# quitedob/yolo-sod

Hardware: AMD Instinct MI355X
Metric: images/sec @640×640 bs=32, 1→8 MI355X; mAP@0.5:0.95 parity vs CPU ref (higher is better)
Workload: dtype f32

## Files before the change

include/yolosod_hip.h:

```cpp
#ifndef YOLOSOD_HIP_H
#define YOLOSOD_HIP_H
#include <stddef.h>
#include <stdint.h>

#ifdef __cplusplus
extern "C" {
#endif

int yolosod_abi_version(void);
const char* yolosod_last_error(void);
int yolosod_init(int device);

size_t yolosod_se_workspace(int B, int C, int H, int W);
int yolosod_se_forward(const float* x, float* y, int B, int C, int H, int W, const float* fc1_w, const float* fc1_b,
                       const float* fc2_w, const float* fc2_b, int hidden, void* workspace, size_t workspace_bytes,
                       void* stream);

size_t yolosod_cbam_workspace(int B, int C, int H, int W);
int yolosod_cbam_forward(const float* x, float* y, int B, int C, int H, int W, const float* fc0_w,
                         const float* fc2_w, int hidden, const float* sa_w, void* workspace, size_t workspace_bytes,
                         void* stream);

size_t yolosod_ca_workspace(int B, int C, int H, int W);
int yolosod_ca_forward(const float* x, float* y, int B, int C, int H, int W, const float* conv1_w,
// ... 69 lines not shown
                              const float* in_bn_var, float in_bn_eps, const float* pw1_w, const float* dw_w,
                              const float* bn_w, const float* bn_b, const float* bn_mean, const float* bn_var,
                              float bn_eps, const float* pw2_w, const float* out_w, const float* out_bn_w,
                              const float* out_bn_b, const float* out_bn_mean, const float* out_bn_var,
                              float out_bn_eps, void* workspace, size_t workspace_bytes, void* stream);

int yolosod_detect_decode(int nl, const float* const* maps, const int* heights, const int* widths,
                          const float* strides, int B, int nc, int reg_max, float* y, void* stream);

int yolosod_detect_head(int nl, const float* const* box_feat, const float* const* cls_feat, int c2, int c3,
                        const float* const* box_w, const float* const* box_b, const float* const* cls_w,
                        const float* const* cls_b, const int* heights, const int* widths, const float* strides, int B,
                        int nc, int reg_max, float* y, void* stream);

size_t yolosod_nms_workspace(int B, int nc, int A, int multi_label);
size_t yolosod_nms_workspace_v2(int B, int nc, int A, int multi_label, int max_det);
int yolosod_nms(float* pred, int B, int nc, int A, float conf_thres, double iou_thres, const int* classes,
                int n_classes, int agnostic, int multi_label, int max_det, int max_nms, float max_wh, int in_place,
                float* out, int* counts, int* out_index, void* workspace, size_t workspace_bytes, void* stream);
int yolosod_nms_merged(float* pred, int B, int nc, int A, float conf_thres, double iou_thres, const int* classes,
                       int n_classes, int agnostic, int multi_label, int max_det, int max_nms, float max_wh,
                       int in_place, float* out, int* counts, int* out_index, int* n_merged, void* workspace,
                       size_t workspace_bytes, void* stream);

int yolosod_letterbox_ingest(const int64_t* desc, int B, void* out, long out_bstride, int out_h, int out_w,
                             int out_bf16, int pad_value, void* stream);
int yolosod_letterbox_ingest_nv12(const int64_t* desc, int B, void* out, long out_bstride, int out_h, int out_w,
                                  int out_bf16, int pad_value, void* stream);
int yolosod_scale_boxes(float* det, const int* counts, int B, int D, const float* geom, void* stream);
int yolosod_tile_merge(const float* y, int n, int nc, int A, const int32_t* desc, int rows, float* merged, int F,
                       int S, float cut_margin, void* stream);
int yolosod_tta_views(const void* x, int B, int C, int H, int W, int bf16, const int64_t* desc, int V, int max_ph,
                      int max_pw, void* stream);
int yolosod_tta_merge(const float* y, int B, int nc, int A, int src_lo, int n, float* cat, int A_tot, int dst,
                      float scale, int flip, float img_w, float img_h, void* stream);
int yolosod_tile_merge_tta(const float* y, int n, int nc, int A, int src_lo, int n_k, const int32_t* desc, int rows,
                           float* merged, int F, int S, int A_tot, int dst, float scale, int flip, float img_w,
                           float img_h, float cut_margin, void* stream);
int yolosod_match_predictions(const float* det, const int* counts, int B, int D, const float* labels,
                              const int* label_off, const float* iouv, int T, uint8_t* tp, void* stream);
int yolosod_confusion_matrix(const float* det, const int* counts, int B, int D, const float* labels,
                             const int* label_off, int nc, float conf_thr, float iou_thr, int32_t* cm, void* stream);

int yolosod_bias_act(const float* y, long y_bstride, float* out, long out_bstride, const float* bias,
                     const float* res, long res_bstride, int B, int C, long HW, int act, void* stream);

int yolosod_bias_act_dual(const float* y, long y_bstride, float* out, long out_bstride, const float* bias,
                          const float* res, long res_bstride, float* out2, long out2_bstride, int c2lo, int B, int C,
                          long HW, int act, void* stream);

size_t yolosod_conv3x3_prep_bytes(int cin);
int yolosod_conv3x3_prepare(const float* w, int cin, void* prep, size_t prep_bytes, void* stream);
int yolosod_conv3x3_silu(const float* x, float* y, int B, int cin, int H, int W, const float* bias, const void* prep,
                         size_t prep_bytes, void* stream);
size_t yolosod_conv3x3_prep_bytes_ex(int cin, int cout);
int yolosod_conv3x3_prepare_ex(const float* w, int cin, int cout, void* prep, size_t prep_bytes, void* stream);
int yolosod_conv3x3_silu_ex(const float* x, float* y, long y_bstride, const float* res, long res_bstride, int B,
                            int cin, int cout, int H, int W, const float* bias, const void* prep, size_t prep_bytes,
                            void* stream);
int yolosod_conv3x3_silu_xs(const float* x, long x_bstride, float* y, long y_bstride, const float* res, long res_bstride,
                            int B, int cin, int cout, int H, int W, const float* bias, const void* prep,
                            size_t prep_bytes, void* stream);
int yolosod_bottleneck3x3_silu_xs(const float* x, long x_bstride, float* y, long y_bstride, const float* res,
                                  long res_bstride, int B, int H, int W, const float* bias1, const void* prep1,
                                  size_t prep1_bytes, const float* bias2, const void* prep2, size_t prep2_bytes,
                                  void* stream);

int yolosod_conv3x3_head_xs(const float* x, long x_bstride, int B, int H, int W, const float* bias, const void* prep,
                            size_t prep_bytes, const void* head_prep, const float* head_bias, int mode, int nc,
                            float stride, float* y, int A, int a_off, void* stream);
size_t yolosod_detect_head_prep_bytes(int rows);
int yolosod_detect_head_prepare(const float* w, int rows, void* prep, size_t prep_bytes, void* stream);

int yolosod_conv1x1_thin(const float* x, long x_bs, const float* w, const float* bias, float* out, long out_bs,
                         const float* res, long res_bs, float* out2, long out2_bs, int c2lo, int B, int Cin, int Cout,
                         long HW, void* stream);

int yolosod_sppf_pool(float* z, long z_bstride, int B, int C, int H, int W, void* stream);

int yolosod_conv1x1_thin_cat(const float* x, long x_bs, const float* x2, long x2_bs, int k1, const float* w,
                             const float* bias, float* out, long out_bs, float* out2, long out2_bs, int c2lo, int B,
                             int Cin, int Cout, long HW, int up_w, void* stream);

int yolosod_conv1x1_thin_stats(const float* x, long x_bs, const float* w, const float* bias, float* out, long out_bs,
                               int B, int Cin, int Cout, long HW, int parts, float* psum, float* pmax, float* tile_ws,
                               void* stream);

int yolosod_conv1x1(const float* x, long x_bs, const float* w, const float* bias, float* out, long out_bs,
                    const float* res, long res_bs, int B, int Cin, int Cout, long HW, int act, void* stream);

int yolosod_gemm_f32(const float* A, long a_bs, int lda, const float* B, long b_bs, int ldb, int b_kcontig, float* C,
                     long c_bs, int ldc, int M, int N, int K, int batch, const float* bias, int bias_mode, int act,
                     const float* res, void* stream);
int yolosod_layernorm(const float* x, float* y, long rows, int C, const float* w, const float* b, float eps,
                      void* stream);
int yolosod_attention(const float* qkv, float* out, long n_seq, int L, int C, int heads, void* stream);

void yolosod_debug_set_swin_fused(int on);
int yolosod_debug_set_swin_x3(int on);
int yolosod_debug_swin_route(int B, int C, int num_heads, int H, int W, int window, int mlp_hidden);
int yolosod_debug_swin_last_route(void);
int yolosod_debug_set_a2_pool_px(int px);
int yolosod_debug_set_head_x2(int on);
int yolosod_debug_set_a2_x2(int on);
int yolosod_debug_set_a2_fused(int on);
int yolosod_debug_set_a2_pool_wide(int on);
int yolosod_se_gate(const float* x, int B, int C, int H, int W, const float* fc1_w, const float* fc1_b,
                    const float* fc2_w, const float* fc2_b, int hidden, const float* psum, float* gate, void* workspace,
                    size_t workspace_bytes, void* stream);
int yolosod_cbam_gates(const float* x, int B, int C, int H, int W, const float* fc0_w, const float* fc2_w, int hidden,
                       const float* sa_w, const float* psum, const float* pmax, float* ca, float* sa, void* workspace,
                       size_t workspace_bytes, void* stream);
size_t yolosod_conv3x3s2_prep_bytes(int cin, int cout);
int yolosod_conv3x3s2_prepare(const float* w, int cin, int cout, void* prep, size_t prep_bytes, void* stream);
int yolosod_conv3x3s2_silu(const float* x, float* y, int B, int cin, int cout, int H, int W, const float* bias,
                           const float* gc, const float* gp, const void* prep, size_t prep_bytes, void* stream);
int yolosod_conv3x3s2_silu_out(const float* x, float* y, long y_bstride, int B, int cin, int cout, int H, int W,
                               const float* bias, const float* gc, const float* gp, const void* prep,
                               size_t prep_bytes, void* stream);
size_t yolosod_conv1x1x2_prep_bytes(int cin, int cout);
int yolosod_conv1x1x2_prepare(const float* w, int cin, int cout, void* prep, size_t prep_bytes, void* stream);
int yolosod_conv1x1x2_silu(const float* x, long x_bstride, float* y, long y_bstride, float* y2, long y2_bstride,
                           int c2lo, int B, int cin, int cout, int HW, const float* bias, const void* prep,
                           size_t prep_bytes, void* stream);
int yolosod_conv1x1x2_silu_cat(const float* x, long x_bstride, const float* x2, long x2_bstride, int k1, float* y,
                               long y_bstride, float* y2, long y2_bstride, int c2lo, int B, int cin, int cout, int HW,
                               const float* bias, const void* prep, size_t prep_bytes, int up_w, void* stream);
int yolosod_conv1x1x2_silu_stats(const float* x, long x_bstride, float* y, long y_bstride, int B, int cin, int cout,
                                 int HW, const float* bias, const void* prep, size_t prep_bytes, int stats, int parts,
                                 float* psum, float* pmax, float* tile_ws, void* stream);
int yolosod_debug_set_conv1x1x2_form(int form);
int yolosod_debug_conv1x1x2_form(int B, int cout, int H, int W);
int yolosod_debug_set_conv3x3s2_form(int form);
int yolosod_debug_conv3x3s2_form(int B, int cout, int H, int W);
int yolosod_debug_set_conv3x3_form(int form);
int yolosod_debug_conv3x3_form(int B, int cout, int H, int W);
int yolosod_debug_conv3x3_form_ex(int B, int cin, int cout, int H, int W);
int yolosod_debug_bottleneck3x3_fused(int B, int H, int W);
int yolosod_debug_set_bottleneck3x3_fuse(int mode);
int yolosod_debug_conv3x3_head_fused(int B, int H, int W);
int yolosod_debug_set_conv3x3_head_fuse(int mode);
void yolosod_debug_set_gemm_x2(int on);
int yolosod_debug_set_swin_tokln(int on);
int yolosod_debug_split_f16(const float* v, uint32_t* h, uint32_t* l, long npair, void* stream);
int yolosod_split_range_flag(int reset, void* stream);

#include <stdint.h>

int yolosod_se_forward_bf16(const uint16_t* x, uint16_t* y, int B, int C, int H, int W, const float* fc1_w,
                            const float* fc1_b, const float* fc2_w, const float* fc2_b, int hidden, const float* psum,
                            void* workspace, size_t workspace_bytes, void* stream);
int yolosod_cbam_forward_bf16(const uint16_t* x, uint16_t* y, int B, int C, int H, int W, const float* fc0_w,
                              const float* fc2_w, int hidden, const float* sa_w, const float* psum, const float* pmax,
                              void* workspace, size_t workspace_bytes, void* stream);
int yolosod_ca_forward_bf16(const uint16_t* x, uint16_t* y, int B, int C, int H, int W, const float* conv1_w,
                            const float* conv1_b, int mip, const float* bn_w, const float* bn_b, const float* bn_mean,
                            const float* bn_var, float bn_eps, const float* convh_w, const float* convh_b,
                            const float* convw_w, const float* convw_b, const float* yin, void* workspace,
                            size_t workspace_bytes, void* stream);
size_t yolosod_swin_workspace_bf16(int B, int C, int H, int W, int num_heads, int window, int mlp_hidden);
int yolosod_swin_forward_bf16(const uint16_t* x, uint16_t* y, int B, int C, int H, int W, int num_heads, int window,
                              const float* dw_w, const float* ln1_w, const float* ln1_b, float ln1_eps,
                              const uint16_t* in_proj_w, const float* in_proj_b, const uint16_t* out_proj_w,
                              const float* out_proj_b, const float* ln2_w, const float* ln2_b, float ln2_eps,
                              const uint16_t* mlp1_w, const float* mlp1_b, int mlp_hidden, const uint16_t* mlp2_w,
                              const float* mlp2_b, const uint16_t* pw_w, const float* bn_w, const float* bn_b,
                              const float* bn_mean, const float* bn_var, float bn_eps, void* workspace,
                              size_t workspace_bytes, void* stream);
size_t yolosod_a2_workspace_bf16(int B, int C, int H, int W, int num_areas);
int yolosod_a2_forward_bf16(const uint16_t* x, uint16_t* y, int B, int C, int H, int W, int num_areas, int num_heads,
                            const uint16_t* proj_w, const float* proj_b, const float* ln_w, const float* ln_b,
                            float ln_eps, const uint16_t* in_proj_w, const float* in_proj_b, const uint16_t* oproj_w,
                            const float* oproj_b, void* workspace, size_t workspace_bytes, void* stream);
int yolosod_detect_head_levels(int nl, int l0, int l1, const void* const* box_feat, const void* const* cls_feat, int c2,
                               int c3, const float* const* box_w, const float* const* box_b, const float* const* cls_w,
                               const float* const* cls_b, const int* heights, const int* widths, const float* strides,
                               int B, int nc, int reg_max, float* y, int bf16, void* stream);
int yolosod_detect_head_bf16(int nl, const uint16_t* const* box_feat, const uint16_t* const* cls_feat, int c2, int c3,
                             const float* const* box_w, const float* const* box_b, const float* const* cls_w,
                             const float* const* cls_b, const int* heights, const int* widths, const float* strides,
                             int B, int nc, int reg_max, float* y, void* stream);
int yolosod_bias_act_bf16(const uint16_t* y, long y_bstride, uint16_t* out, long out_bstride, const float* bias,
                          const uint16_t* res, long res_bstride, uint16_t* out2, long out2_bstride, int c2lo, int B,
                          int C, long HW, int act, void* stream);
int yolosod_bias_act_stats_bf16(const uint16_t* y, long y_bstride, uint16_t* out, long out_bstride, const float* bias,
                                const uint16_t* res, long res_bstride, int B, int C, long HW, int act, int parts,
                                long seg, float* psum, float* pmax, void* stream);
int yolosod_bias_act_capool_bf16(const uint16_t* y, long y_bstride, uint16_t* out, long out_bstride,
                                 const float* bias, const uint16_t* res, long res_bstride, int B, int C, int H, int W,
                                 int act, float* yin, void* stream);
int yolosod_gemm_bf16(const uint16_t* A, long a_bs, int lda, const uint16_t* B, long b_bs, int ldb, int b_kcontig,
                      uint16_t* C, long c_bs, int ldc, int M, int N, int K, int batch, const float* bias,
                      int bias_mode, int act, const uint16_t* res, void* stream);
int yolosod_attention_bf16(const uint16_t* qkv, uint16_t* out, long n_seq, int L, int C, int heads, void* stream);
int yolosod_debug_gemm_bf16_tile(int M, int N, int batch);
int yolosod_debug_gemm_bf16_last_tile(void);
long yolosod_debug_gemm_bf16_launches(int tile);
int yolosod_debug_swin_bf16_route(int B, int C, int num_heads, int H, int W, int window, int mlp_hidden);
int yolosod_debug_swin_bf16_last_route(void);
int yolosod_debug_attention_bf16_form(int L, int C, int heads);
int yolosod_debug_attention_bf16_last_form(void);

#ifdef __cplusplus
}
#endif
#endif
```

yolo-sod_amd/_hip.py:

```python
from __future__ import annotations

import ctypes
import os
from pathlib import Path

import torch

from .utils.metrics import IOU_THRESHOLDS

LIB_PATH = Path(__file__).resolve().parent / "lib" / "libyolosod_hip.so"

_c_float_p = ctypes.c_void_p
_vp = ctypes.c_void_p
_i = ctypes.c_int
_l = ctypes.c_long
_f = ctypes.c_float
_d = ctypes.c_double
_sz = ctypes.c_size_t

SIGNATURES = {
    "yolosod_abi_version": (_i, []),
    "yolosod_last_error": (ctypes.c_char_p, []),
    "yolosod_se_workspace": (_sz, [_i, _i, _i, _i]),
    "yolosod_se_forward": (_i, [_vp, _vp, _i, _i, _i, _i, _vp, _vp, _vp, _vp, _i, _vp, _sz, _vp]),
    "yolosod_cbam_workspace": (_sz, [_i, _i, _i, _i]),
    "yolosod_cbam_forward": (_i, [_vp, _vp, _i, _i, _i, _i, _vp, _vp, _i, _vp, _vp, _sz, _vp]),
    "yolosod_ca_workspace": (_sz, [_i, _i, _i, _i]),
    "yolosod_ca_forward": (_i, [_vp, _vp, _i, _i, _i, _i, _vp, _vp, _i, _vp, _vp, _vp, _vp, _f, _vp, _vp, _vp,
                                _vp, _vp, _sz, _vp]),
    "yolosod_a2_workspace": (_sz, [_i, _i, _i, _i, _i]),
    "yolosod_a2_forward": (_i, [_vp, _vp, _i, _i, _i, _i, _i, _i, _vp, _vp, _vp, _vp, _f, _vp, _vp, _vp, _vp, _vp,
                                _vp, _vp, _sz, _vp]),
    "yolosod_swin_workspace": (_sz, [_i, _i, _i, _i, _i, _i]),
    "yolosod_swin_workspace_v2": (_sz, [_i, _i, _i, _i, _i, _i, _i]),
    "yolosod_swin_forward": (_i, [_vp, _vp, _i, _i, _i, _i, _i, _i, _vp, _vp, _vp, _f, _vp, _vp, _vp, _vp, _vp, _vp,
                                  _f, _vp, _vp, _i, _vp, _vp, _vp, _vp, _vp, _vp, _vp, _f, _vp, _sz, _vp]),
    "yolosod_detect_decode": (_i, [_i, _vp, _vp, _vp, _vp, _i, _i, _i, _vp, _vp]),
    "yolosod_detect_head": (_i, [_i, _vp, _vp, _i, _i, _vp, _vp, _vp, _vp, _vp, _vp, _vp, _i, _i, _i, _vp, _vp]),
    "yolosod_nms_workspace": (_sz, [_i, _i, _i, _i]),
    "yolosod_nms_workspace_v2": (_sz, [_i, _i, _i, _i, _i]),
    "yolosod_nms": (_i, [_vp, _i, _i, _i, _f, _d, _vp, _i, _i, _i, _i, _i, _f, _i, _vp, _vp, _vp, _vp, _sz, _vp]),
    "yolosod_nms_merged": (_i, [_vp, _i, _i, _i, _f, _d, _vp, _i, _i, _i, _i, _i, _f, _i, _vp, _vp, _vp, _vp, _vp, _sz,
                                _vp]),
    "yolosod_gemm_f32": (_i, [_vp, _l, _i, _vp, _l, _i, _i, _vp, _l, _i, _i, _i, _i, _i, _vp, _i, _i, _vp, _vp]),
    "yolosod_layernorm": (_i, [_vp, _vp, _l, _i, _vp, _vp, _f, _vp]),
    "yolosod_attention": (_i, [_vp, _vp, _l, _i, _i, _i, _vp]),
    "yolosod_bias_act": (_i, [_vp, _l, _vp, _l, _vp, _vp, _l, _i, _i, _l, _i, _vp]),
    "yolosod_upsample2x": (_i, [_vp, _vp, _l, _i, _i, _i, _i, _i, _vp]),
    "yolosod_letterbox_ingest": (_i, [_vp, _i, _vp, _l, _i, _i, _i, _i, _vp]),
    "yolosod_letterbox_ingest_nv12": (_i, [_vp, _i, _vp, _l, _i, _i, _i, _i, _vp]),
    "yolosod_scale_boxes": (_i, [_vp, _vp, _i, _i, _vp, _vp]),
    "yolosod_tile_merge": (_i, [_vp, _i, _i, _i, _vp, _i, _vp, _i, _i, _f, _vp]),
    "yolosod_tile_merge_tta": (_i, [_vp, _i, _i, _i, _i, _i, _vp, _i, _vp, _i, _i, _i, _i, _f, _i, _f, _f, _f, _vp]),
    "yolosod_match_predictions": (_i, [_vp, _vp, _i, _i, _vp, _vp, _vp, _i, _vp, _vp]),
    "yolosod_confusion_matrix": (_i, [_vp, _vp, _i, _i, _vp, _vp, _i, _f, _f, _vp, _vp]),
    "yolosod_tta_views": (_i, [_vp, _i, _i, _i, _i, _i, _vp, _i, _i, _i, _vp]),
    "yolosod_tta_merge": (_i, [_vp, _i, _i, _i, _i, _i, _vp, _i, _i, _f, _i, _f, _f, _vp]),
    "yolosod_stem_workspace": (_sz, [_i, _i, _i, _i]),
    "yolosod_stem_conv": (_i, [_vp, _vp, _vp, _vp, _i, _i, _i, _i, _i, _l, _vp, _vp, _sz, _vp]),
    "yolosod_conv1x1_thin_stats": (_i, [_vp, _l, _vp, _vp, _vp, _l, _i, _i, _i, _l, _i, _vp, _vp, _vp, _vp]),
    "yolosod_conv1x1_thin": (_i, [_vp, _l, _vp, _vp, _vp, _l, _vp, _l, _vp, _l, _i, _i, _i, _i, _l, _vp]),
    "yolosod_bias_act_dual": (_i, [_vp, _l, _vp, _l, _vp, _vp, _l, _vp, _l, _i, _i, _i, _l, _i, _vp]),
    "yolosod_bias_act_capool": (_i, [_vp, ctypes.c_long, _vp, ctypes.c_long, _vp, _vp, ctypes.c_long, _i, _i, _i, _i,
                                     _i, _vp, _vp]),
    "yolosod_ca_forward_pre": (_i, [_vp, _vp, _i, _i, _i, _i, _vp, _vp, _i, _vp, _vp, _vp, _vp, _f, _vp, _vp, _vp, _vp,
                                    _vp, _vp, ctypes.c_size_t, _vp]),
    "yolosod_bias_act_stats": (_i, [_vp, _l, _vp, _l, _vp, _vp, _l, _i, _i, _l, _i, _i, _l, _vp, _vp, _vp]),
    "yolosod_plane_parts": (_i, [_l, ctypes.POINTER(ctypes.c_long)]),
    "yolosod_se_forward_pre": (_i, [_vp, _vp, _i, _i, _i, _i, _vp, _vp, _vp, _vp, _i, _vp, _vp, _sz, _vp]),
    "yolosod_cbam_forward_pre": (_i, [_vp, _vp, _i, _i, _i, _i, _vp, _vp, _i, _vp, _vp, _vp, _vp, _sz, _vp]),
    "yolosod_conv1x1": (_i, [_vp, _l, _vp, _vp, _vp, _l, _vp, _l, _i, _i, _i, _l, _i, _vp]),
    "yolosod_conv3x3_prep_bytes": (_sz, [_i]),
    "yolosod_conv3x3_prepare": (_i, [_vp, _i, _vp, _sz, _vp]),
    "yolosod_conv3x3_silu": (_i, [_vp, _vp, _i, _i, _i, _i, _vp, _vp, _sz, _vp]),
    "yolosod_conv1x1x2_prep_bytes": (_sz, [_i, _i]),
    "yolosod_conv1x1x2_prepare": (_i, [_vp, _i, _i, _vp, _sz, _vp]),
    "yolosod_conv1x1x2_silu": (_i, [_vp, _l, _vp, _l, _vp, _l, _i, _i, _i, _i, _i, _vp, _vp, _sz, _vp]),
    "yolosod_conv1x1x2_silu_cat": (_i, [_vp, _l, _vp, _l, _i, _vp, _l, _vp, _l, _i, _i, _i, _i, _i, _vp, _vp, _sz,
                                        _i, _vp]),
    "yolosod_conv1x1x2_silu_stats": (_i, [_vp, _l, _vp, _l, _i, _i, _i, _i, _vp, _vp, _sz, _i, _i, _vp, _vp, _vp, _vp]),
    "yolosod_sppf_pool": (_i, [_vp, _l, _i, _i, _i, _i, _vp]),
    "yolosod_conv1x1_thin_cat": (_i, [_vp, _l, _vp, _l, _i, _vp, _vp, _vp, _l, _vp, _l, _i, _i, _i, _i, _l, _i, _vp]),
    "yolosod_conv3x3_prep_bytes_ex": (_sz, [_i, _i]),
    "yolosod_conv3x3_prepare_ex": (_i, [_vp, _i, _i, _vp, _sz, _vp]),
    "yolosod_conv3x3_silu_ex": (_i, [_vp, _vp, _l, _vp, _l, _i, _i, _i, _i, _i, _vp, _vp, _sz, _vp]),
    "yolosod_conv3x3_silu_xs": (_i, [_vp, _l, _vp, _l, _vp, _l, _i, _i, _i, _i, _i, _vp, _vp, _sz, _vp]),
    "yolosod_debug_set_swin_fused": (None, [_i]),
    "yolosod_debug_set_swin_x3": (_i, [_i]),
    "yolosod_debug_swin_route": (_i, [_i, _i, _i, _i, _i, _i, _i]),
    "yolosod_debug_swin_last_route": (_i, []),
    "yolosod_debug_set_head_x2": (_i, [_i]),
    "yolosod_debug_set_a2_x2": (_i, [_i]),
    "yolosod_debug_set_gemm_x2": (None, [_i]),
    "yolosod_debug_split_f16": (_i, [_vp, _vp, _vp, _l, _vp]),
    "yolosod_swin_prep_bytes": (_sz, [_i, _i, _i]),
    "yolosod_split_range_flag": (_i, [_i, _vp]),
    "yolosod_swin_prepare": (_i, [_i, _i, _i] + [_vp] * 15 + [_f, _vp, _sz, _vp]),
    "yolosod_swin_forward_prepared": (_i, [_vp, _vp, _i, _i, _i, _i, _i, _i, _vp, _f, _vp, _f, _i, _vp, _vp, _sz,
                                           _vp, _sz, _vp]),
    "yolosod_swin_prepared_workspace": (_sz, [_i, _i, _i, _i, _i, _i, _i]),
    "yolosod_a2_prep_bytes": (_sz, [_i, _i, _i, _i]),
    "yolosod_a2_prepare": (_i, [_i, _vp, _vp, _vp, _vp, _vp, _vp, _sz, _vp]),
    "yolosod_a2_forward_prepared": (_i, [_vp, _vp, _i, _i, _i, _i, _i, _i, _vp, _vp, _vp, _vp, _f, _vp, _vp, _vp,
                                         _vp, _vp, _sz, _vp, _sz, _vp]),
    "yolosod_init": (_i, [_i]),
    "yolosod_debug_set_a2_fused": (_i, [_i]),
    "yolosod_debug_set_a2_pool_wide": (_i, [_i]),
    "yolosod_debug_set_conv3x3_form": (_i, [_i]),
    "yolosod_debug_conv3x3_form": (_i, [_i, _i, _i, _i]),
    "yolosod_debug_conv3x3_form_ex": (_i, [_i, _i, _i, _i, _i]),
    "yolosod_bottleneck3x3_silu_xs": (_i, [_vp, _l, _vp, _l, _vp, _l, _i, _i, _i, _vp, _vp, _sz, _vp, _vp, _sz, _vp]),
    "yolosod_conv3x3_head_xs": (_i, [_vp, _l, _i, _i, _i, _vp, _vp, _sz, _vp, _vp, _i, _i, _f, _vp, _i, _i, _vp]),
    "yolosod_detect_head_prep_bytes": (_sz, [_i]),
    "yolosod_detect_head_prepare": (_i, [_vp, _i, _vp, _sz, _vp]),
    "yolosod_debug_conv3x3_head_fused": (_i, [_i, _i, _i]),
    "yolosod_debug_set_conv3x3_head_fuse": (_i, [_i]),
    "yolosod_debug_bottleneck3x3_fused": (_i, [_i, _i, _i]),
    "yolosod_debug_set_bottleneck3x3_fuse": (_i, [_i]),
    "yolosod_debug_set_conv1x1x2_form": (_i, [_i]),
    "yolosod_debug_conv1x1x2_form": (_i, [_i, _i, _i, _i]),
    "yolosod_debug_set_conv3x3s2_form": (_i, [_i]),
    "yolosod_debug_conv3x3s2_form": (_i, [_i, _i, _i, _i]),
    "yolosod_se_gate": (_i, [_vp, _i, _i, _i, _i, _vp, _vp, _vp, _vp, _i, _vp, _vp, _vp, _sz, _vp]),
    "yolosod_cbam_gates": (_i, [_vp, _i, _i, _i, _i, _vp, _vp, _i, _vp, _vp, _vp, _vp, _vp, _vp, _sz, _vp]),
    "yolosod_conv3x3s2_prep_bytes": (_sz, [_i, _i]),
    "yolosod_conv3x3s2_prepare": (_i, [_vp, _i, _i, _vp, _sz, _vp]),
    "yolosod_conv3x3s2_silu": (_i, [_vp, _vp, _i, _i, _i, _i, _i, _vp, _vp, _vp, _vp, _sz, _vp]),
    "yolosod_conv3x3s2_silu_out": (_i, [_vp, _vp, _l, _i, _i, _i, _i, _i, _vp, _vp, _vp, _vp, _sz, _vp]),
    "yolosod_debug_set_swin_tokln": (_i, [_i]),
    "yolosod_debug_set_a2_pool_px": (_i, [_i]),
    "yolosod_mamba_glu_workspace": (_sz, [_i, _i, _i, _i, _i, _i]),
    "yolosod_mamba_glu_forward": (_i, [_vp, _vp, _i, _i, _i, _i, _i, _i, _vp, _vp, _vp, _vp, _vp, _f, _vp, _vp,
                                       _vp, _vp, _vp, _vp, _f, _vp, _vp, _vp, _vp, _vp, _vp, _f, _vp, _sz, _vp]),
    "yolosod_se_forward_bf16": (_i, [_vp, _vp, _i, _i, _i, _i, _vp, _vp, _vp, _vp, _i, _vp, _vp, _sz, _vp]),
    "yolosod_cbam_forward_bf16": (_i, [_vp, _vp, _i, _i, _i, _i, _vp, _vp, _i, _vp, _vp, _vp, _vp, _sz, _vp]),
    "yolosod_ca_forward_bf16": (_i, [_vp, _vp, _i, _i, _i, _i, _vp, _vp, _i, _vp, _vp, _vp, _vp, _f, _vp, _vp, _vp,
                                     _vp, _vp, _vp, _sz, _vp]),
    "yolosod_bias_act_bf16": (_i, [_vp, _l, _vp, _l, _vp, _vp, _l, _vp, _l, _i, _i, _i, _l, _i, _vp]),
    "yolosod_bias_act_stats_bf16": (_i, [_vp, _l, _vp, _l, _vp, _vp, _l, _i, _i, _l, _i, _i, _l, _vp, _vp, _vp]),
    "yolosod_bias_act_capool_bf16": (_i, [_vp, _l, _vp, _l, _vp, _vp, _l, _i, _i, _i, _i, _i, _vp, _vp]),
    "yolosod_swin_workspace_bf16": (_sz, [_i, _i, _i, _i, _i, _i, _i]),
    "yolosod_swin_forward_bf16": (_i, [_vp, _vp, _i, _i, _i, _i, _i, _i, _vp, _vp, _vp, _f, _vp, _vp, _vp, _vp, _vp,
                                       _vp, _f, _vp, _vp, _i, _vp, _vp, _vp, _vp, _vp, _vp, _vp, _f, _vp, _sz, _vp]),
    "yolosod_a2_workspace_bf16": (_sz, [_i, _i, _i, _i, _i]),
    "yolosod_a2_forward_bf16": (_i, [_vp, _vp, _i, _i, _i, _i, _i, _i, _vp, _vp, _vp, _vp, _f, _vp, _vp, _vp, _vp,
                                     _vp, _sz, _vp]),
    "yolosod_detect_head_bf16": (_i, [_i, _vp, _vp, _i, _i, _vp, _vp, _vp, _vp, _vp, _vp, _vp, _i, _i, _i, _vp,
                                      _vp]),
    "yolosod_detect_head_levels": (_i, [_i, _i, _i, _vp, _vp, _i, _i, _vp, _vp, _vp, _vp, _vp, _vp, _vp, _i, _i,
                                        _i, _vp, _i, _vp]),
    "yolosod_gemm_bf16": (_i, [_vp, _l, _i, _vp, _l, _i, _i, _vp, _l, _i, _i, _i, _i, _i, _vp, _i, _i, _vp, _vp]),
    "yolosod_attention_bf16": (_i, [_vp, _vp, _l, _i, _i, _i, _vp]),
    "yolosod_debug_gemm_bf16_tile": (_i, [_i, _i, _i]),
    "yolosod_debug_gemm_bf16_last_tile": (_i, []),
    "yolosod_debug_gemm_bf16_launches": (_l, [_i]),
    "yolosod_debug_swin_bf16_route": (_i, [_i, _i, _i, _i, _i, _i, _i]),
    "yolosod_debug_swin_bf16_last_route": (_i, []),
    "yolosod_debug_attention_bf16_form": (_i, [_i, _i, _i]),
    "yolosod_debug_attention_bf16_last_form": (_i, []),
}

_LIB = None
# ... 141 lines not shown
def _c(t: torch.Tensor) -> torch.Tensor:
    return t.detach().float().contiguous()


class PlaneStats:

    __slots__ = ("psum", "pmax", "parts", "shape")

    def __init__(self, psum, pmax, parts, shape):
        self.psum, self.pmax, self.parts, self.shape = psum, pmax, parts, tuple(shape)


_PARTS = {}


def plane_parts(HW: int):
    if HW not in _PARTS:
        seg = ctypes.c_long(0)
        parts = load_library().yolosod_plane_parts(int(HW), ctypes.byref(seg))
        _PARTS[HW] = (int(parts), int(seg.value))
    return _PARTS[HW]


def _pre_stats(x, need_max):
    st = getattr(x, "_ys_plane_stats", None)
    if st is None or st.shape != tuple(x.shape) or (need_max and st.pmax is None):
        return None
    return st


def _t(t, name):
    if not isinstance(t, torch.Tensor):
        raise TypeError(f"{name}: expected a tensor")
    if t.device.type != "cuda":
        raise RuntimeError(f"{name}: HIP kernel requires a GPU tensor (got device {t.device}); no CPU fallback")
    return t


def se_forward(x, fc1_w, fc1_b, fc2_w, fc2_b):
    bf = _act_dtype(_t(x, "x"))
    hid = fc1_w.shape[0]
    pre = _pre_stats(x, False)
    return _launch(("se", tuple(x.shape), hid) + ((2,) if bf else ()), x.device, ops().se_fwd, x, fc1_w, fc1_b,
                   fc2_w, fc2_b, None if pre is None else pre.psum)


def cbam_forward(x, fc0_w, fc2_w, sa_w):
    bf = _act_dtype(_t(x, "x"))
    hid = fc0_w.shape[0]
    pre = _pre_stats(x, True)
    return _launch(("cbam", tuple(x.shape), hid) + ((2,) if bf else ()), x.device, ops().cbam_fwd, x, fc0_w, fc2_w,
                   sa_w, None if pre is None else pre.psum, None if pre is None else pre.pmax)


def se_gate(x, fc1_w, fc1_b, fc2_w, fc2_b):
    lib = load_library()
    B, C, H, W = x.shape
    hid = int(fc1_w.shape[0])
    pre = _pre_stats(x, False)
    gate = torch.empty((B, C), dtype=torch.float32, device=x.device)
    ws = torch.empty(int(lib.yolosod_se_workspace(B, C, H, W)), dtype=torch.uint8, device=x.device)
    _check(_launch(("se_gate", tuple(x.shape), hid), x.device, lib.yolosod_se_gate, _dev(x, "x"), B, C, H, W,
                   _dev(fc1_w, "fc1_w"), _dev(fc1_b, "fc1_b"), _dev(fc2_w, "fc2_w"), _dev(fc2_b, "fc2_b"), hid,
                   None if pre is None else _dev(pre.psum, "psum"), gate.data_ptr(), ws.data_ptr(), ws.numel(),
                   _stream(x.device)), "se_gate")
    return gate


def cbam_gates(x, fc0_w, fc2_w, sa_w):
    lib = load_library()
    B, C, H, W = x.shape
    hid = int(fc0_w.shape[0])
    pre = _pre_stats(x, True)
    ca = torch.empty((B, C), dtype=torch.float32, device=x.device)
    sa = torch.empty((B, H, W), dtype=torch.float32, device=x.device)
    ws = torch.empty(int(lib.yolosod_cbam_workspace(B, C, H, W)), dtype=torch.uint8, device=x.device)
    _check(_launch(("cbam_gate", tuple(x.shape), hid), x.device, lib.yolosod_cbam_gates, _dev(x, "x"), B, C, H, W,
                   _dev(fc0_w, "fc0_w"), _dev(fc2_w, "fc2_w"), hid, _dev(sa_w, "sa_w"),
                   None if pre is None else _dev(pre.psum, "psum"), None if pre is None else _dev(pre.pmax, "pmax"),
                   ca.data_ptr(), sa.data_ptr(), ws.data_ptr(), ws.numel(), _stream(x.device)), "cbam_gates")
    return ca, sa


def ca_forward(x, conv1_w, conv1_b, bn_w, bn_b, bn_mean, bn_var, bn_eps, convh_w, convh_b, convw_w, convw_b):
    bf = _act_dtype(_t(x, "x"))
    mip = conv1_w.shape[0]
    pre = getattr(x, "_ys_ca_pool", None)
    yin = pre[0] if pre is not None and pre[1] == tuple(x.shape) else None
    return _launch(("ca", tuple(x.shape), mip) + ((2,) if bf else ()), x.device, ops().ca_fwd, x, conv1_w, conv1_b,
                   bn_w, bn_b, bn_mean, bn_var, float(bn_eps), convh_w, convh_b, convw_w, convw_b, yin)


def a2_prep_bytes(C, num_heads, num_areas, W) -> int:
    return int(load_library().yolosod_a2_prep_bytes(int(C), int(num_heads), int(num_areas), int(W)))


def a2_prepare(x, num_areas, num_heads, proj_w, ln_w, ln_b, in_w, in_b):
    return ops().a2_prep(x, int(num_areas), int(num_heads), proj_w, ln_w, ln_b, in_w, in_b)


def a2_forward(x, num_areas, num_heads, proj_w, proj_b, ln_w, ln_b, ln_eps, in_w, in_b, mo_w, mo_b, op_w, op_b,
               prep=None):
    bf = _act_dtype(_t(x, "x"))
    B, C, H, W = x.shape
    if num_areas * W > 320:
        raise RuntimeError(f"A2_Attn: sequence length {num_areas * W} > 320 unsupported")
    if bf and (C // num_heads not in (32, 64, 128) or C % 64):
        raise RuntimeError(f"A2_Attn (bf16): C={C} with head dim {C // num_heads} unsupported")
    use_prep = prep is not None and not bf and mo_w is None and a2_prep_bytes(C, num_heads, num_areas, W) > 0

    def run():
        return ops().a2_fwd(x, int(num_areas), int(num_heads), proj_w, proj_b, ln_w, ln_b, float(ln_eps), in_w, in_b,
                            mo_w, mo_b, op_w, op_b, prep() if use_prep else None)

    return _launch(("a2", tuple(x.shape), (num_areas, num_heads)) + ((2,) if bf else ()), x.device, run)


def swin_forward(x, num_heads, window, dw_w, ln1_w, ln1_b, ln1_eps, in_w, in_b, out_w, out_b, ln2_w, ln2_b,
                 ln2_eps, m1_w, m1_b, m2_w, m2_b, pw_w, bn_w, bn_b, bn_mean, bn_var, bn_eps, prep=None):
    bf = _act_dtype(_t(x, "x"))
    B, C, H, W = x.shape
    hid = m1_w.shape[0]
    wh = H if (H <= window and W <= window) else min(window, H)
    ww = W if (H <= window and W <= window) else min(window, W)
    if wh * ww > 320:
        raise RuntimeError(f"SwinBlock: window of {wh}x{ww} tokens unsupported")
    if C % num_heads or (C // num_heads) not in ((32, 64, 128) if bf else (8, 16, 32, 64, 128)):
        raise RuntimeError(f"SwinBlock: head dim {C}/{num_heads} unsupported")
    key = ("swin", tuple(x.shape), (num_heads, window, hid)) + ((2,) if bf else ())
    if (prep is not None and not bf and wh == 7 and ww == 7 and C * H * W < (1 << 30)
            and swin_prep_bytes(C, num_heads, hid) > 0):
        return _launch(key, x.device, lambda: ops().swin_fwd_prepared(x, prep(), int(num_heads), int(window), dw_w,
                                                                      float(ln1_eps), out_b, float(ln2_eps), int(hid),
                                                                      m2_b))
    return _launch(key, x.device, ops().swin_fwd, x, int(num_heads), int(window), dw_w, ln1_w, ln1_b, float(ln1_eps),
                   in_w, in_b, out_w, out_b, ln2_w, ln2_b, float(ln2_eps), m1_w, m1_b, m2_w, m2_b, pw_w, bn_w, bn_b,
                   bn_mean, bn_var, float(bn_eps))


def split_range_flag(reset: bool = True, device=None) -> bool:
    dev = torch.device("cuda", torch.cuda.current_device()) if device is None else torch.device(device)
    with torch.cuda.device(dev):
        rc = load_library().yolosod_split_range_flag(int(bool(reset)), _stream(dev))
    if rc < 0:
        _check(rc, "split_range_flag")
    return rc == 1


_split_convs_off = 0


def split_convs_enabled() -> bool:
    return _split_convs_off == 0


class exact_fp32_matrix:

    _SWITCHES = ("yolosod_debug_set_swin_x3", "yolosod_debug_set_head_x2", "yolosod_debug_set_a2_x2")

    def __enter__(self):
        global _split_convs_off
        lib = load_library()
        self._prev = [int(getattr(lib, f)(0)) for f in self._SWITCHES]
        _split_convs_off += 1
        return self

# ... 211 lines not shown
            fn = lib.yolosod_bias_act_capool_bf16 if bf else lib.yolosod_bias_act_capool
            _check(_launch(key("capool"), y.device, fn, y.data_ptr(), yb, out.data_ptr(), ob,
                           bp, rp, rb, B, C, H, W, int(act), yin.data_ptr(), _stream(y.device)), "bias_act_capool")
            out._ys_ca_pool = (yin, tuple(out.shape))
            return out
    if stats is not None:
        parts, seg = plane_parts(HW)
        psum = torch.empty(B * C * parts, dtype=torch.float32, device=y.device)
        pmax = torch.empty_like(psum) if stats == "summax" else None
        fn = lib.yolosod_bias_act_stats_bf16 if bf else lib.yolosod_bias_act_stats
        _check(_launch(key(stats), y.device, fn, y.data_ptr(), yb, out.data_ptr(), ob, bp,
                       rp, rb, B, C, HW, int(act), parts, seg, psum.data_ptr(),
                       None if pmax is None else pmax.data_ptr(), _stream(y.device)), "bias_act_stats")
        out._ys_plane_stats = PlaneStats(psum, pmax, parts, out.shape)
        return out
    if bf:
        _check(_launch(key(None), y.device, lib.yolosod_bias_act_bf16, y.data_ptr(), yb,
                       out.data_ptr(), ob, bp, rp, rb, None, 0, 0, B, C, HW, int(act), _stream(y.device)),
               "bias_act_bf16")
        return out
    _check(_launch(key(None), y.device, lib.yolosod_bias_act, y.data_ptr(), yb, out.data_ptr(),
                   ob, bp, rp, rb, B, C, HW, int(act), _stream(y.device)), "bias_act")
    return out


STEM_TILE_ROWS = 8


def stem_ok(x, conv) -> bool:
    if not isinstance(x, torch.Tensor) or x.dim() != 4 or x.device.type != "cuda" or x.dtype != torch.float32:
        return False
    B, Cin, H, W = x.shape
    if (conv.bias is None or Cin != 3 or conv.in_channels != 3 or conv.kernel_size != (3, 3) or conv.stride != (2, 2)
            or conv.padding != (1, 1) or conv.dilation != (1, 1) or conv.groups != 1
            or conv.padding_mode != "zeros" or conv.weight.dtype != torch.float32 or conv.weight.device != x.device):
        return False
    Cout = conv.out_channels
    if Cout % 2 or Cout > 64 or B == 0 or H % 2 or W % 2 or (W // 2) % 4:
        return False
    if not x.is_contiguous() or x.data_ptr() % 16:
        return False
    parts, seg = plane_parts((H // 2) * (W // 2))
    return parts == 1 or STEM_TILE_ROWS * (W // 2) <= seg


def stem_conv(x, weight, bias):
    B, _, H, W = _t(x, "x").shape
    Cout = int(weight.shape[0])
    out, psum = _launch(("stem", tuple(x.shape), (Cout, "sum")), x.device, ops().stem_fwd, x, weight, bias)
    out._ys_plane_stats = PlaneStats(psum, None, plane_parts((H // 2) * (W // 2))[0], out.shape)
    return out


def upsample2x_into(x, out) -> bool:
    B, C, h, w = x.shape
    if (x.device.type != "cuda" or out.device != x.device or out.dtype != x.dtype or x.dtype not in (torch.float32, _BF16)
            or not x.is_contiguous() or tuple(out.shape) != (B, C, 2 * h, 2 * w) or out.stride(3) != 1
            or out.stride(2) != 2 * w or out.stride(1) != 4 * h * w):
        return False
    eb = x.element_size()
    if (w % 4 or x.data_ptr() % 16 or out.data_ptr() % 16 or (out.stride(0) * eb) % 16 or (4 * h * w * eb) % 16
            or B == 0):
        return False
    _check(_launch(("upsample2x", tuple(x.shape), None), x.device, load_library().yolosod_upsample2x, x.data_ptr(),
                   out.data_ptr(), out.stride(0), B, C, h, w, eb, _stream(x.device)), "upsample2x")
    return True


THIN1X1_COUT = (64, 128)
THIN1X1_CIN = (64, 96, 128, 192, 256)


def conv1x1_thin_ok(x, cout) -> bool:
    if isinstance(x, CatView):
        B, Cin, H, W = x.shape
        return (x.device.type == "cuda" and x.dtype == torch.float32 and cout in THIN1X1_COUT and Cin in THIN1X1_CIN
                and (H * W) % 64 == 0 and all(_imgs_contig(t) for t in x.parts) and (not x.up0 or W % 4 == 0))
    B, Cin, H, W = x.shape
    return (x.device.type == "cuda" and x.dtype == torch.float32 and cout in THIN1X1_COUT and Cin in THIN1X1_CIN
            and (H * W) % 64 == 0 and x.stride(3) == 1 and x.stride(2) == W and x.stride(1) == H * W
            and x.stride(0) % 4 == 0 and x.data_ptr() % 16 == 0)


def conv1x1_thin(x, w, bias, out=None, res=None, out2=None, c2lo=0, stats=None):
    lib = load_library()
    B, Cin, H, W = x.shape
    Cout = w.shape[0]
    HW = H * W
    if out is None:
        out = torch.empty((B, Cout, H, W), dtype=torch.float32, device=x.device)

    def bstride(t, name, C):
        if t.device.type != "cuda" or t.dtype != torch.float32:
            raise RuntimeError(f"conv1x1_thin: {name} must be a float32 GPU tensor")
        if tuple(t.shape) != (B, C, H, W) or t.stride(3) != 1 or t.stride(2) != W or t.stride(1) != HW:
            raise RuntimeError(f"conv1x1_thin: {name} must be [B,{C},H,W] with contiguous channels")
        return t.stride(0)

    if isinstance(x, CatView):
        if res is not None or stats is not None:
            raise RuntimeError("conv1x1_thin: a CatView input takes no res / stats")
        x0, x1 = x.parts
        k1 = int(x0.shape[1])
        ob = bstride(out, "out", Cout)
        o2 = bstride(out2, "out2", Cout - c2lo) if out2 is not None else 0
        if x.up0:
            if not _imgs_contig(x0) or W % 4:
                raise RuntimeError("conv1x1_thin: an upsampled CatView part needs contiguous images and W % 4 == 0")
            xb0 = x0.stride(0)
        else:
            xb0 = bstride(x0, "x", k1)
        _check(_launch(("conv1x1_thin", tuple(x.shape), (Cout, False, out2 is not None, "cat")), x.device,
                       lib.yolosod_conv1x1_thin_cat, x0.data_ptr(), xb0, x1.data_ptr(),
                       bstride(x1, "x2", Cin - k1), k1, _dev(w.contiguous(), "weight"), _dev(bias, "bias"),
                       out.data_ptr(), ob, None if out2 is None else out2.data_ptr(), o2, int(c2lo), B, Cin, Cout, HW,
                       W if x.up0 else 0, _stream(x.device)), "conv1x1_thin_cat")
        return out
    xb = bstride(x, "x", Cin)
    ob = bstride(out, "out", Cout)
    rb = bstride(res, "res", Cout) if res is not None else 0
    o2 = bstride(out2, "out2", Cout - c2lo) if out2 is not None else 0
    if stats in ("sum", "summax") and res is None and out2 is None:
        parts, _ = plane_parts(HW)
        psum = torch.empty(B * Cout * parts, dtype=torch.float32, device=x.device)
        pmax = torch.empty_like(psum) if stats == "summax" else None
        tws = torch.empty(2 * B * Cout * (HW // 64), dtype=torch.float32, device=x.device)
        _check(_launch(("conv1x1_thin", tuple(x.shape), (Cout, stats)), x.device, lib.yolosod_conv1x1_thin_stats, x.data_ptr(), xb, _dev(w.contiguous(), "weight"), _dev(bias, "bias"),
                                              out.data_ptr(), ob, B, Cin, Cout, HW, parts, psum.data_ptr(),
                                              None if pmax is None else pmax.data_ptr(), tws.data_ptr(), _stream(x.device)),
               "conv1x1_thin_stats")
        out._ys_plane_stats = PlaneStats(psum, pmax, parts, out.shape)
        return out
    if stats is not None:
        raise RuntimeError(f"conv1x1_thin: stats={stats!r} needs res=None and out2=None")
    _check(_launch(("conv1x1_thin", tuple(x.shape), (Cout, res is not None, out2 is not None)), x.device, lib.yolosod_conv1x1_thin, x.data_ptr(), xb, _dev(w.contiguous(), "weight"), _dev(bias, "bias"),
                                    out.data_ptr(), ob, None if res is None else res.data_ptr(), rb,
                                    None if out2 is None else out2.data_ptr(), o2, int(c2lo), B, Cin, Cout, HW,
                                    _stream(x.device)), "conv1x1_thin")
    return out


def conv1x1(x, w, bias, act, out=None, res=None):
    lib = load_library()
    B, Cin, H, W = x.shape
    Cout = w.shape[0]
    HW = H * W
    if out is None:
        out = torch.empty((B, Cout, H, W), dtype=torch.float32, device=x.device)

    def bstride(t, name, C):
        if t.device.type != "cuda" or t.dtype != torch.float32:
            raise RuntimeError(f"conv1x1: {name} must be a float32 GPU tensor")
        if tuple(t.shape) != (B, C, H, W) or t.stride(3) != 1 or t.stride(2) != W or t.stride(1) != HW:
            raise RuntimeError(f"conv1x1: {name} must be [B,{C},H,W] with contiguous channels")
        return t.stride(0)

    xb = bstride(x, "x", Cin)
    ob = bstride(out, "out", Cout)
    rb = bstride(res, "res", Cout) if res is not None else 0
    _check(_launch(("conv1x1", tuple(x.shape), Cout), x.device, lib.yolosod_conv1x1, x.data_ptr(), xb, _dev(w, "weight"), None if bias is None else _dev(bias, "bias"),
                               out.data_ptr(), ob, None if res is None else res.data_ptr(), rb, B, Cin, Cout, HW,
                               int(act), _stream(x.device)), "conv1x1")
    return out


def conv3x3_ok(x, conv) -> bool:
    return (x.device.type == "cuda" and x.dtype == torch.float32 and x.dim() == 4 and _imgs_contig(x)
            and conv.kernel_size == (3, 3) and conv.stride == (1, 1) and conv.padding == (1, 1)
            and conv.dilation == (1, 1) and conv.groups == 1 and x.shape[1] == conv.in_channels
            and int(load_library().yolosod_conv3x3_prep_bytes_ex(int(conv.in_channels), int(conv.out_channels))) > 0)


def _split_prepare(name, bytes_fn, prepare_fn, w):
# ... 41 lines not shown
                                           0 if res is None else res.stride(0), B, Cin, cout, H, W, _dev(b, "bias"),
                                           blk.data_ptr(), blk.numel(), _stream(x.device))

    _check(_launch((op, tuple(x.shape), cout if res is None else (cout, "res")), x.device, run), "conv3x3")
    return y


def conv3x3_head_fused(B, H, W) -> bool:
    return bool(load_library().yolosod_debug_conv3x3_head_fused(int(B), int(H), int(W)))


def detect_head_prepare(w, rows):
    lib = load_library()
    nbytes = int(lib.yolosod_detect_head_prep_bytes(int(rows)))
    wc = w.detach().float().reshape(w.shape[0], -1).contiguous()
    if nbytes == 0 or tuple(wc.shape) != (rows, 64):
        raise RuntimeError(f"detect_head_prepare: weight {tuple(w.shape)} unsupported ([64 | 1..16, 64])")
    blk = torch.empty(nbytes, dtype=torch.uint8, device=w.device)
    _check(_launch(("head_prep", (rows, 64), None), w.device, lib.yolosod_detect_head_prepare, _dev(wc, "weight"),
                   int(rows), blk.data_ptr(), nbytes, _stream(w.device)), "detect_head_prepare")
    return blk


def conv3x3_head(x, bias, prep, head_prep, head_bias, mode, nc, stride, y, a_off):
    lib = load_library()
    B, Cin, H, W = x.shape
    if Cin != 64:
        raise RuntimeError(f"conv3x3_head: {Cin} channels (64 only)")
    if (y.dtype != torch.float32 or y.device != x.device or not y.is_contiguous() or y.dim() != 3 or y.shape[0] != B
            or y.shape[1] != 4 + nc):
        raise RuntimeError(f"conv3x3_head: y {tuple(y.shape)} is not a contiguous fp32 [{B}, {4 + nc}, A] tensor")
    b = bias.detach().float().contiguous()
    hb = head_bias.detach().float().contiguous()
    if hb.numel() != (64 if mode == 1 else nc):
        raise RuntimeError(f"conv3x3_head: head bias of {hb.numel()} values")

    def run():
        blk, hblk = prep(), head_prep()
        _img_view(x, (B, 64, H, W), "conv3x3_head: x")
        return lib.yolosod_conv3x3_head_xs(x.data_ptr(), x.stride(0), B, H, W, _dev(b, "bias"), blk.data_ptr(),
                                           blk.numel(), hblk.data_ptr(), _dev(hb, "head bias"), int(mode), int(nc),
                                           float(stride), y.data_ptr(), int(y.shape[2]), int(a_off), _stream(x.device))

    _check(_launch(("conv3x3", tuple(x.shape), (64, "head", int(mode))), x.device, run), "conv3x3_head")
    return y


def bottleneck3x3_fused(B, H, W) -> bool:
    return bool(load_library().yolosod_debug_bottleneck3x3_fused(int(B), int(H), int(W)))


def bottleneck3x3_silu(x, bias1, prep1, bias2, prep2, out=None, res=None, op="bottleneck3x3"):
    lib = load_library()
    B, C, H, W = x.shape
    if C != 32:
        raise RuntimeError(f"bottleneck3x3: {C} channels (32 only)")
    if out is None:
        y = torch.empty((B, 32, H, W), dtype=torch.float32, device=x.device)
    else:
        _img_view(out, (B, 32, H, W), "bottleneck3x3: out")
        y = out
    if res is not None:
        _img_view(res, (B, 32, H, W), "bottleneck3x3: res")
    b1 = bias1.detach().float().contiguous()
    b2 = bias2.detach().float().contiguous()

    def run():
        blk1, blk2 = prep1(), prep2()
        _img_view(x, (B, 32, H, W), "bottleneck3x3: x")
        return lib.yolosod_bottleneck3x3_silu_xs(x.data_ptr(), x.stride(0), y.data_ptr(), y.stride(0),
                                                 None if res is None else res.data_ptr(),
                                                 0 if res is None else res.stride(0), B, H, W, _dev(b1, "bias1"),
                                                 blk1.data_ptr(), blk1.numel(), _dev(b2, "bias2"), blk2.data_ptr(),
                                                 blk2.numel(), _stream(x.device))

    _check(_launch((op, tuple(x.shape), 32 if res is None else (32, "res")), x.device, run), "bottleneck3x3")
    return y


class CatView:

    def __init__(self, parts, up0=False):
        a, b = parts
        sp = (2 * a.shape[2], 2 * a.shape[3]) if up0 else tuple(a.shape[2:])
        if a.shape[0] != b.shape[0] or sp != tuple(b.shape[2:]) or a.dtype != b.dtype or a.device != b.device:
            raise ValueError("CatView: parts must agree in batch, spatial size, dtype and device")
        self.parts = (a, b)
        self.up0 = bool(up0)
        self.shape = torch.Size((a.shape[0], a.shape[1] + b.shape[1], b.shape[2], b.shape[3]))
        self.device, self.dtype = a.device, a.dtype

    def dim(self):
        return 4

    def materialize(self):
        a, b = self.parts
        if self.up0:
            a = torch.nn.functional.interpolate(a, scale_factor=2, mode="nearest")
        return torch.cat((a, b), 1)


def sppf_pool(z, c):
    B, C4, H, W = z.shape
    if (C4 != 4 * c or z.dtype != torch.float32 or z.device.type != "cuda"
            or z.stride()[1:] != (H * W, W, 1)):
        raise RuntimeError("sppf_pool: z must be a [B, 4c, H, W] fp32 GPU tensor with contiguous images")
    lib = load_library()
    _check(_launch(("sppf_pool", (B, c, H, W), None), z.device, lib.yolosod_sppf_pool, z.data_ptr(), z.stride(0), B,
                   int(c), H, W, _stream(z.device)), "sppf_pool")
    return z


def _imgs_contig(t) -> bool:
    B, C, H, W = t.shape
    return t.stride()[1:] == (H * W, W, 1) and t.stride(0) % 4 == 0 and t.data_ptr() % 16 == 0


def conv1x1x2_ok(x, conv) -> bool:
    if isinstance(x, CatView):
        if not (all(_imgs_contig(t) for t in x.parts) and x.parts[0].shape[1] % 128 == 0):
            return False
    elif not (x.dim() == 4 and _imgs_contig(x)):
        return False
    return (x.device.type == "cuda" and x.dtype == torch.float32
            and conv.kernel_size == (1, 1) and conv.stride == (1, 1) and conv.padding == (0, 0) and conv.groups == 1
            and x.shape[1] == conv.in_channels and (x.shape[2] * x.shape[3]) % 4 == 0
            and int(load_library().yolosod_conv1x1x2_prep_bytes(int(conv.in_channels), int(conv.out_channels))) > 0)


def conv1x1x2_prepare(w):
    lib = load_library()
    return _split_prepare("conv1x1x2", lib.yolosod_conv1x1x2_prep_bytes, lib.yolosod_conv1x1x2_prepare,
                          w.reshape(int(w.shape[0]), int(w.shape[1])))


def conv1x1x2_silu(x, bias, prep, cout, out=None, out2=None, c2lo=0, op="conv1x1x2", stats=None):
    lib = load_library()
    B, Cin, H, W = x.shape
    if stats is not None and (stats not in ("sum", "summax", "capool") or out2 is not None or isinstance(x, CatView)):
        raise RuntimeError(f"conv1x1x2: stats={stats!r} takes one input tensor, no out2")
    if out is None:
        y = torch.empty((B, cout, H, W), dtype=torch.float32, device=x.device)
    else:
        _img_view(out, (B, cout, H, W), "conv1x1x2: out")
        y = out
    if out2 is not None:
        _img_view(out2, (B, cout - c2lo, H, W), "conv1x1x2: out2")
    b = bias.detach().float().contiguous()
    if stats in ("sum", "summax"):
        HW = H * W
        parts, _ = plane_parts(HW)
        psum = torch.empty(B * cout * parts, dtype=torch.float32, device=x.device)
        pmax = torch.empty_like(psum) if stats == "summax" else None
        tws = torch.empty(2 * B * cout * ((HW + 63) // 64), dtype=torch.float32, device=x.device)

        def run_stats():
            blk = prep()
            return lib.yolosod_conv1x1x2_silu_stats(x.data_ptr(), x.stride(0), y.data_ptr(), y.stride(0), B, Cin, cout,
                                                    HW, _dev(b, "bias"), blk.data_ptr(), blk.numel(),
                                                    2 if stats == "summax" else 1, parts, psum.data_ptr(),
                                                    None if pmax is None else pmax.data_ptr(), tws.data_ptr(),
                                                    _stream(x.device))

        _check(_launch(("conv1x1x2_stats", tuple(x.shape), (cout, stats)), x.device, run_stats), "conv1x1x2_stats")
        y._ys_plane_stats = PlaneStats(psum, pmax, parts, y.shape)
        return y

    x0, x1 = x.parts if isinstance(x, CatView) else (x, None)

    def run():
        blk = prep()
        return lib.yolosod_conv1x1x2_silu_cat(x0.data_ptr(), x0.stride(0), None if x1 is None else x1.data_ptr(),
                                              0 if x1 is None else x1.stride(0), int(x0.shape[1]), y.data_ptr(),
                                              y.stride(0), None if out2 is None else out2.data_ptr(),
                                              0 if out2 is None else out2.stride(0), int(c2lo), B, Cin, cout, H * W,
                                              _dev(b, "bias"), blk.data_ptr(), blk.numel(),
                                              W if x1 is not None and x.up0 else 0, _stream(x.device))

    extra = (cout, out2 is not None) + (("cat",) if x1 is not None else ())
    if stats == "capool":
        op, extra = "conv1x1x2_stats", (cout, stats)
    _check(_launch((op, tuple(x.shape), extra), x.device, run), "conv1x1x2")
    return y


def conv3x3s2_ok(x, conv) -> bool:
    return (x.device.type == "cuda" and x.dtype == torch.float32 and x.is_contiguous() and x.dim() == 4
            and conv.kernel_size == (3, 3) and conv.stride == (2, 2) and conv.padding == (1, 1)
            and conv.dilation == (1, 1) and conv.groups == 1
            and (conv.out_channels == 64 or (conv.out_channels % 128 == 0 and conv.out_channels <= 512))
            and conv.in_channels % 32 == 0 and x.shape[1] == conv.in_channels and ((x.shape[3] + 1) // 2) % 4 == 0
            and x.numel() * 4 < 2 ** 32
            and int(load_library().yolosod_conv3x3s2_prep_bytes(int(conv.in_channels), int(conv.out_channels))) > 0)


def conv3x3s2_prepare(w):
    lib = load_library()
    return _split_prepare("conv3x3s2", lib.yolosod_conv3x3s2_prep_bytes, lib.yolosod_conv3x3s2_prepare, w)


def conv3x3s2_silu(x, bias, prep, cout, gate_c=None, gate_p=None, key=None, out=None):
    lib = load_library()
    B, Cin, H, W = x.shape
    Ho, Wo = (H + 1) // 2, (W + 1) // 2
    if out is None:
        y = torch.empty((B, cout, Ho, Wo), dtype=torch.float32, device=x.device)
    else:
        y = out
        if (tuple(y.shape) != (B, cout, Ho, Wo) or y.dtype != torch.float32 or y.device != x.device
                or y.stride()[1:] != (Ho * Wo, Wo, 1) or y.data_ptr() % 16 or y.stride(0) % 4):
            raise RuntimeError(f"conv3x3s2: out {tuple(y.shape)} / {y.stride()} is not a [{B}, {cout}, {Ho}, {Wo}] "
                               "fp32 view with contiguous 16-byte aligned images")
    b = bias.detach().float().contiguous()
    gc = None if gate_c is None else gate_c.float().contiguous()
    gp = None if gate_p is None else gate_p.float().contiguous()
    if gc is not None and (tuple(gc.shape) != (B, Cin) or gc.data_ptr() % 16):
        raise RuntimeError(f"conv3x3s2: channel gate {tuple(gc.shape)} (16-byte aligned [{B}, {Cin}] expected)")
    if gp is not None and gp.numel() != B * H * W:
        raise RuntimeError(f"conv3x3s2: spatial gate of {gp.numel()} values ({B * H * W} expected)")

    def run():
        blk = prep()
        return lib.yolosod_conv3x3s2_silu_out(_dev(x, "x"), y.data_ptr(), y.stride(0), B, Cin, cout, H, W,
                                              _dev(b, "bias"), None if gc is None else _dev(gc, "gate_c"),
                                              None if gp is None else _dev(gp, "gate_p"), blk.data_ptr(), blk.numel(),
                                              _stream(x.device))

    if key is None:
        key = ("conv3x3s2", tuple(x.shape), (cout, gc is not None, gp is not None))
    _check(_launch(key, x.device, run), "conv3x3s2")
    return y


INGEST_MAX_DIM = 16384


def letterbox_ingest(images, out_shape, geoms, dtype=torch.float32, out=None, pad_value=114):
    lib = load_library()
    B = len(images)
    out_h, out_w = int(out_shape[0]), int(out_shape[1])
    if B < 1 or len(geoms) != B:
        raise RuntimeError(f"letterbox_ingest: {B} frames with {len(geoms)} geometries")
    if dtype not in (torch.float32, _BF16):
        raise RuntimeError(f"letterbox_ingest: output dtype must be float32 or bfloat16, got {dtype}")
    if out_w % 4 or not (0 < out_h <= INGEST_MAX_DIM and 0 < out_w <= INGEST_MAX_DIM):
        raise RuntimeError(f"letterbox_ingest: canvas {out_h}x{out_w} unsupported (width % 4 == 0, <= {INGEST_MAX_DIM})")
    rows = []
    dev = None
    for i, (t, g) in enumerate(zip(images, geoms)):
        if not isinstance(t, torch.Tensor):
            raise TypeError(f"letterbox_ingest: frame {i}: expected a tensor")
        if t.dtype != torch.uint8:
            raise RuntimeError(f"letterbox_ingest: frame {i}: expected uint8, got {t.dtype}")
        if t.dim() != 3 or t.shape[2] != 3:
            raise RuntimeError(f"letterbox_ingest: frame {i}: expected [h, w, 3] (BGR), got {tuple(t.shape)}")
        h, w = int(t.shape[0]), int(t.shape[1])
        if not (0 < h <= INGEST_MAX_DIM and 0 < w <= INGEST_MAX_DIM):
            raise RuntimeError(f"letterbox_ingest: frame {i}: {h}x{w} outside 1..{INGEST_MAX_DIM}")
        if t.stride(2) != 1:
            raise RuntimeError(f"letterbox_ingest: frame {i}: channel stride {t.stride(2)} (1 expected)")
        if w > 1 and t.stride(1) != 3:
            raise RuntimeError(f"letterbox_ingest: frame {i}: pixel stride {t.stride(1)} (3 expected)")
        pitch = int(t.stride(0)) if h > 1 else 3 * w
        if pitch < 3 * w:
# ... 538 lines not shown
```

yolo-sod_amd/csrc/channel_attention.hip:

```cpp
#include "common.h"
#include <stdlib.h>
#include <math.h>

namespace ys {

constexpr int kMaxParts = 64;

struct PartPlan {
  int parts;
  long seg;
};
static PartPlan part_plan(long HW) {
  long p = HW / 8192;
  if (p > kMaxParts) p = kMaxParts;
  if (p < 1) p = 1;
  long seg = (HW + p - 1) / p;
  if ((HW & 3) == 0) seg = (seg + 3) & ~3L;
  p = (HW + seg - 1) / seg;
  return {(int)p, seg};
}

template <bool WITH_MAX, class T>
__global__ __launch_bounds__(256) void plane_part_stats_kernel(const T* __restrict__ x, long HW, int parts,
                                                               long seg, float* __restrict__ psum,
// ... 669 lines not shown
template <class T>
static int cbam_forward_impl(const T* x, T* y, int B, int C, int H, int W, const float* fc0_w, const float* fc2_w,
                             int hidden, const float* sa_w, const float* psum_pre, const float* pmax_pre,
                             void* workspace, size_t workspace_bytes, void* stream, float* ca_out = nullptr,
                             float* sa_out = nullptr) {
  YS_CHECK_ARG(x && (y || (ca_out && sa_out)) && fc0_w && fc2_w && sa_w, "cbam: null pointer");
  YS_CHECK_ARG(B >= 0 && C > 0 && C <= 16384 && H > 0 && W > 0, "cbam: bad shape");
  YS_CHECK_ARG(hidden > 0 && hidden <= 64, "cbam: hidden=%d unsupported (1..64)", hidden);
  if (B == 0) return 0;
  const long HW = (long)H * W;
  const int V = (HW % 4 == 0) ? 4 : 1;
  const long pxb = (HW + 256 * V - 1) / (256 * V);
  const int G = (C + kCbamGroup - 1) / kCbamGroup;
  Carver cv(workspace, workspace_bytes);
  float* psum = cv.take<float>((size_t)B * C * part_plan((long)H * W).parts);
  float* pmax = cv.take<float>((size_t)B * C * part_plan((long)H * W).parts);
  float* ca = cv.take<float>((size_t)B * C);
  float* mpart = cv.take<float>((size_t)B * G * 2 * HW);
  float* sa = cv.take<float>((size_t)B * HW);
  YS_CHECK_ARG(sa, "cbam: workspace too small (%zu)", workspace_bytes);
  if (!y) {
    ca = ca_out;
    sa = sa_out;
  }
  hipStream_t st = (hipStream_t)stream;
  const PartPlan pp = part_plan(HW);
  const size_t lds = sizeof(float) * (3 * (size_t)C + 128);
  const bool fused = V == 4 && lds <= 64 * 1024;
  YS_CHECK_ARG(lds <= 64 * 1024, "cbam: C=%d too large for the gate kernel", C);
  const float* ps = psum_pre ? psum_pre : psum;
  const float* pm = pmax_pre ? pmax_pre : pmax;
  if (!psum_pre)
    hipLaunchKernelGGL((plane_part_stats_kernel<true, T>), dim3((unsigned)(B * C * pp.parts)), dim3(256), 0, st, x, HW,
                       pp.parts, pp.seg, psum, pmax);
  dim3 gs((unsigned)pxb, G, B);
  if (fused) {
    hipLaunchKernelGGL((cbam_pixel_stats_kernel<4, T, true>), gs, dim3(256), lds, st, x, ca, C, kCbamGroup, HW, mpart,
                       ps, pm, pp.parts, 1.0f / (float)HW, fc0_w, fc2_w, hidden);
  } else {
    hipLaunchKernelGGL((channel_gate_kernel<true>), dim3(B), dim3(256), lds, st, ps, pm, pp.parts, C, 1.0f / (float)HW,
                       fc0_w, nullptr, fc2_w, nullptr, hidden, ca);
    if (V == 4)
      hipLaunchKernelGGL((cbam_pixel_stats_kernel<4, T, false>), gs, dim3(256), 0, st, x, ca, C, kCbamGroup, HW, mpart,
                         nullptr, nullptr, 0, 0.f, nullptr, nullptr, 0);
    else
      hipLaunchKernelGGL((cbam_pixel_stats_kernel<1, T, false>), gs, dim3(256), 0, st, x, ca, C, kCbamGroup, HW, mpart,
                         nullptr, nullptr, 0, 0.f, nullptr, nullptr, 0);
  }
  hipLaunchKernelGGL(cbam_sa_kernel, dim3((W + kSaTW - 1) / kSaTW, (H + kSaTH - 1) / kSaTH, B), dim3(256), 0, st, mpart, G, C, H, W, sa_w,
                     sa);
  if (y) {
    dim3 ga((unsigned)pxb, (C + 7) / 8, B);
    if (V == 4)
      hipLaunchKernelGGL((cbam_apply_kernel<4, T>), ga, dim3(256), 0, st, x, y, ca, sa, C, HW);
    else
      hipLaunchKernelGGL((cbam_apply_kernel<1, T>), ga, dim3(256), 0, st, x, y, ca, sa, C, HW);
  }
  YS_CHECK_LAUNCH("cbam");
  return 0;
}

YS_EXPORT int yolosod_cbam_forward(const float* x, float* y, int B, int C, int H, int W, const float* fc0_w,
                                   const float* fc2_w, int hidden, const float* sa_w, void* workspace,
                                   size_t workspace_bytes, void* stream) {
  return cbam_forward_impl(x, y, B, C, H, W, fc0_w, fc2_w, hidden, sa_w, (const float*)nullptr, nullptr, workspace,
                           workspace_bytes, stream);
}

YS_EXPORT int yolosod_cbam_forward_pre(const float* x, float* y, int B, int C, int H, int W, const float* fc0_w,
                                       const float* fc2_w, int hidden, const float* sa_w, const float* psum,
                                       const float* pmax, void* workspace, size_t workspace_bytes, void* stream) {
  YS_CHECK_ARG(psum && pmax, "cbam_pre: null partials");
  return cbam_forward_impl(x, y, B, C, H, W, fc0_w, fc2_w, hidden, sa_w, psum, pmax, workspace, workspace_bytes,
                           stream);
}

YS_EXPORT int yolosod_cbam_gates(const float* x, int B, int C, int H, int W, const float* fc0_w, const float* fc2_w,
                                 int hidden, const float* sa_w, const float* psum, const float* pmax, float* ca,
                                 float* sa, void* workspace, size_t workspace_bytes, void* stream) {
  YS_CHECK_ARG((psum == nullptr) == (pmax == nullptr), "cbam_gates: give both partials or neither");
  YS_CHECK_ARG(ca && sa, "cbam_gates: null output");
  return cbam_forward_impl<float>(x, nullptr, B, C, H, W, fc0_w, fc2_w, hidden, sa_w, psum, pmax, workspace,
                                  workspace_bytes, stream, ca, sa);
}

YS_EXPORT int yolosod_cbam_forward_bf16(const bf16_t* x, bf16_t* y, int B, int C, int H, int W, const float* fc0_w,
                                        const float* fc2_w, int hidden, const float* sa_w, const float* psum,
                                        const float* pmax, void* workspace, size_t workspace_bytes, void* stream) {
  YS_CHECK_ARG((psum == nullptr) == (pmax == nullptr), "cbam_bf16: give both partials or neither");
  return cbam_forward_impl(x, y, B, C, H, W, fc0_w, fc2_w, hidden, sa_w, psum, pmax, workspace, workspace_bytes,
                           stream);
}

YS_EXPORT size_t yolosod_ca_workspace(int B, int C, int H, int W) {
  Sizer s;
  s.take<float>((size_t)B * C * (H + W));
  s.take<float>((size_t)B * C * (H + W));
  return s.off;
}

template <class T>
static int ca_forward_impl(const T* x, T* y, int B, int C, int H, int W, const float* conv1_w, const float* conv1_b,
                           int mip, const float* bn_w, const float* bn_b, const float* bn_mean, const float* bn_var,
                           float bn_eps, const float* convh_w, const float* convh_b, const float* convw_w,
                           const float* convw_b, const float* yin_pre, void* workspace, size_t workspace_bytes,
                           void* stream) {
  YS_CHECK_ARG(x && y && conv1_w && conv1_b && bn_w && bn_b && bn_mean && bn_var && convh_w && convh_b && convw_w &&
                   convw_b,
               "ca: null pointer");
  YS_CHECK_ARG(B >= 0 && C > 0 && H > 0 && W > 0 && W <= 1024, "ca: bad shape (W <= 1024 supported)");
  YS_CHECK_ARG(mip > 0 && mip <= 64, "ca: mip=%d unsupported (1..64)", mip);
  const size_t gate_lds = ca_gate_lds_bytes(C, mip);
  YS_CHECK_ARG(gate_lds <= 64 * 1024, "ca: C=%d mip=%d exceed the gate kernel's LDS budget", C, mip);
  if (B == 0) return 0;
  Carver cv(workspace, workspace_bytes);
  float* yin = cv.take<float>((size_t)B * C * (H + W));
  float* gate = cv.take<float>((size_t)B * C * (H + W));
  YS_CHECK_ARG(gate, "ca: workspace too small (%zu)", workspace_bytes);
  hipStream_t st = (hipStream_t)stream;
  const long HW = (long)H * W;
  int RB = 8192 / W;
  if (RB < 1) RB = 1;
  if (RB > H) RB = H;
  const size_t pool_lds = sizeof(float) * (size_t)RB * W;
  const int V = (W % 4 == 0) ? 4 : 1;
  const int VA = (sizeof(T) == 2 && W % 8 == 0) ? 8 : V;
  const unsigned apply_y = (unsigned)((HW + 256 * VA - 1) / (256 * VA));
  if (!yin_pre)
    hipLaunchKernelGGL((ca_pool_kernel<T>), dim3(B * C), dim3(256), pool_lds, st, x, H, W, RB, yin);
  hipLaunchKernelGGL(ca_gate_kernel, dim3((H + W + 15) / 16, B), dim3(256), gate_lds, st, yin_pre ? yin_pre : yin, C,
                     H, W, mip, conv1_w, conv1_b, bn_w, bn_b, bn_mean, bn_var, bn_eps, convh_w, convh_b, convw_w,
                     convw_b, gate);
  if (VA == 8)
    hipLaunchKernelGGL((ca_apply_kernel<8, T>), dim3(B * C, apply_y), dim3(256), 0, st, x, y, gate, H, W);
  else if (V == 4)
    hipLaunchKernelGGL((ca_apply_kernel<4, T>), dim3(B * C, apply_y), dim3(256), 0, st, x, y, gate, H, W);
  else
    hipLaunchKernelGGL((ca_apply_kernel<1, T>), dim3(B * C, apply_y), dim3(256), 0, st, x, y, gate, H, W);
  YS_CHECK_LAUNCH("ca");
  return 0;
}

YS_EXPORT int yolosod_ca_forward(const float* x, float* y, int B, int C, int H, int W, const float* conv1_w,
                                 const float* conv1_b, int mip, const float* bn_w, const float* bn_b,
                                 const float* bn_mean, const float* bn_var, float bn_eps, const float* convh_w,
                                 const float* convh_b, const float* convw_w, const float* convw_b, void* workspace,
                                 size_t workspace_bytes, void* stream) {
  return ca_forward_impl(x, y, B, C, H, W, conv1_w, conv1_b, mip, bn_w, bn_b, bn_mean, bn_var, bn_eps, convh_w,
                         convh_b, convw_w, convw_b, (const float*)nullptr, workspace, workspace_bytes, stream);
}

YS_EXPORT int yolosod_ca_forward_pre(const float* x, float* y, int B, int C, int H, int W, const float* conv1_w,
                                     const float* conv1_b, int mip, const float* bn_w, const float* bn_b,
                                     const float* bn_mean, const float* bn_var, float bn_eps, const float* convh_w,
                                     const float* convh_b, const float* convw_w, const float* convw_b,
                                     const float* yin, void* workspace, size_t workspace_bytes, void* stream) {
  YS_CHECK_ARG(yin, "ca_pre: null pooled means");
  return ca_forward_impl(x, y, B, C, H, W, conv1_w, conv1_b, mip, bn_w, bn_b, bn_mean, bn_var, bn_eps, convh_w,
                         convh_b, convw_w, convw_b, yin, workspace, workspace_bytes, stream);
}

YS_EXPORT int yolosod_ca_forward_bf16(const bf16_t* x, bf16_t* y, int B, int C, int H, int W, const float* conv1_w,
                                      const float* conv1_b, int mip, const float* bn_w, const float* bn_b,
                                      const float* bn_mean, const float* bn_var, float bn_eps, const float* convh_w,
                                      const float* convh_b, const float* convw_w, const float* convw_b,
                                      const float* yin, void* workspace, size_t workspace_bytes, void* stream) {
// ... 4 lines not shown
```

yolo-sod_amd/csrc/conv1x1x2.hip:

```cpp
#include "split_conv.h"

namespace ys {
namespace c1 {

constexpr float WSC = SPLIT_WSC;
constexpr int KS = 128;
constexpr int PS = KS + 8;
constexpr int NT = 256;

struct Args {
  const float* x;
  long xbs;
  const h16_t* wp;
  const float* bias;
  float* y;
  long ybs;
  float* y2;
  long y2bs;
  int c2lo, cin, cout, HW, ntile;
  unsigned* range_flag;
  const unsigned* prep_flag;
  const float* x2;
  long x2bs;
  int k1;
  int up_w;
};

#include "conv1x1x2_kernel.h"
#define YS_C1_STATS_FORMS
#include "conv1x1x2_kernel.h"
#undef YS_C1_STATS_FORMS

}
}

using namespace ys;

static int c1_pad(int cin) { return (cin + c1::KS - 1) / c1::KS * c1::KS; }
static size_t c1_halves(int cin, int cout) { return (size_t)2 * cout * c1_pad(cin); }

static int g_c1_form = 0;
YS_EXPORT int yolosod_debug_set_conv1x1x2_form(int form) {
  const int old = g_c1_form;
  if (form >= 0 && form < 12 && (form & 3) != 3) g_c1_form = form;
  return old;
}

static int c1_form(int B, int cout, int HW) {
  if (cout == 64) return 1 + 4 * 1;
  const int fgrp = g_c1_form & 3, fbuf = g_c1_form >> 2;
  const bool g256 = fgrp ? fgrp == 2
                         : cout == 512 && HW <= 400 && (long)B * ((HW + 63) / 64) * (cout / 128) > 2L * cu_count();
  return (g256 && cout % 256 == 0 ? 2 : 1) + 4 * (fbuf ? fbuf : 1);
}

YS_EXPORT int yolosod_debug_conv1x1x2_form(int B, int cout, int H, int W) {
  if (B <= 0 || H <= 0 || W <= 0 || ((long)H * W) % 4 || cout <= 0 || (cout != 64 && cout % 128) || cout > 1024)
    return 0;
  return c1_form(B, cout, H * W);
}

template <int CPW, bool DB>
static void c1_launch(bool dual, unsigned nwg, hipStream_t st, const c1::Args& a) {
  if (dual) hipLaunchKernelGGL((c1::conv1x1_x2_kernel<true, 64, CPW, DB>), dim3(nwg), dim3(c1::NT), 0, st, a);
  else hipLaunchKernelGGL((c1::conv1x1_x2_kernel<false, 64, CPW, DB>), dim3(nwg), dim3(c1::NT), 0, st, a);
}

YS_EXPORT size_t yolosod_conv1x1x2_prep_bytes(int cin, int cout) {
  if (cin <= 0 || cin % 32 || cin > 4096 || cout <= 0 || (cout != 64 && cout % 128) || cout > 1024) return 0;
  return split_prep_bytes(c1_halves(cin, cout));
}

YS_EXPORT int yolosod_conv1x1x2_prepare(const float* w, int cin, int cout, void* prep, size_t prep_bytes,
                                        void* stream) {
  YS_CHECK_ARG(yolosod_conv1x1x2_prep_bytes(cin, cout) > 0, "conv1x1x2_prepare: (cin=%d, cout=%d) unsupported", cin,
               cout);
  return split_prepare<1>("conv1x1x2_prepare", w, cin, c1_pad(cin), cout, prep, prep_bytes, stream);
}

YS_EXPORT int yolosod_conv1x1x2_silu_cat(const float* x, long x_bstride, const float* x2, long x2_bstride, int k1,
                                         float* y, long y_bstride, float* y2, long y2_bstride, int c2lo, int B, int cin,
                                         int cout, int HW, const float* bias, const void* prep, size_t prep_bytes,
                                         int up_w, void* stream) {
  YS_CHECK_ARG(x && y && bias && prep, "conv1x1x2: null pointer");
  if (!x2) k1 = cin;
  YS_CHECK_ARG(up_w == 0 || (x2 && up_w > 0 && up_w % 2 == 0 && HW % up_w == 0 && (HW / up_w) % 2 == 0),
               "conv1x1x2: an upsampled first part needs a second part and even H, W (W=%d, HW=%d)", up_w, HW);
  YS_CHECK_ARG(k1 > 0 && k1 <= cin && (!x2 || (k1 % c1::KS == 0 && k1 < cin && x2_bstride >= (long)(cin - k1) * HW)),
               "conv1x1x2: concat split k1=%d (Cin %d) must be a multiple of %d", k1, cin, c1::KS);
  YS_CHECK_ARG(B >= 0 && HW > 0 && HW % 4 == 0 && yolosod_conv1x1x2_prep_bytes(cin, cout) > 0, "conv1x1x2: bad shape");
  YS_CHECK_ARG(x_bstride >= (long)k1 * (up_w ? HW / 4 : HW) && y_bstride >= (long)cout * HW,
               "conv1x1x2: batch strides too small");
  YS_CHECK_ARG((long)c1_pad(cin) * HW * 4 < (1L << 32), "conv1x1x2: image too large for 32-bit buffer offsets");
  YS_CHECK_ARG((((uintptr_t)y | (uintptr_t)(y2 ? y2 : y)) & 15) == 0 && y_bstride % 4 == 0 && y2_bstride % 4 == 0,
               "conv1x1x2: outputs must be 16-byte aligned");
  YS_CHECK_ARG(!y2 || (c2lo >= 0 && c2lo < cout && y2_bstride >= (long)(cout - c2lo) * HW), "conv1x1x2: c2lo=%d",
               c2lo);
  if (B == 0) return 0;
  SplitPrep sp;
  YS_CHECK_ARG(split_prep_carve(prep, prep_bytes, c1_halves(cin, cout), &sp),
               "conv1x1x2: prepared block too small");
  constexpr int NPx = 64;
  const int ntile = (HW + NPx - 1) / NPx;
  c1::Args a{x, x_bstride, sp.wp, bias, y, y_bstride, y2, y2_bstride, c2lo, cin, cout, HW, ntile, range_flag_dev(),
             sp.flag, x2, x2_bstride, k1, up_w};
  const int form = c1_form(B, cout, HW);
  const bool g256 = (form & 3) == 2, db = (form >> 2) == 2;
  const long nwg = (long)B * ntile * (cout == 64 ? 1 : cout / (g256 ? 256 : 128));
  YS_CHECK_ARG(nwg < (1L << 31), "conv1x1x2: too many tiles");
  hipStream_t st = (hipStream_t)stream;
  if (cout == 64) c1_launch<1, false>(y2 != nullptr, (unsigned)nwg, st, a);
  else if (g256 && db) c1_launch<4, true>(y2 != nullptr, (unsigned)nwg, st, a);
  else if (g256) c1_launch<4, false>(y2 != nullptr, (unsigned)nwg, st, a);
  else if (db) c1_launch<2, true>(y2 != nullptr, (unsigned)nwg, st, a);
  else c1_launch<2, false>(y2 != nullptr, (unsigned)nwg, st, a);
  YS_CHECK_LAUNCH("conv1x1x2");
  return 0;
}

YS_EXPORT int yolosod_conv1x1x2_silu(const float* x, long x_bstride, float* y, long y_bstride, float* y2,
                                     long y2_bstride, int c2lo, int B, int cin, int cout, int HW, const float* bias,
                                     const void* prep, size_t prep_bytes, void* stream) {
  return yolosod_conv1x1x2_silu_cat(x, x_bstride, nullptr, 0, cin, y, y_bstride, y2, y2_bstride, c2lo, B, cin, cout, HW,
                                    bias, prep, prep_bytes, 0, stream);
}

template <int CPW>
static void c1_launch_stats(int stats, unsigned nwg, hipStream_t st, const c1::Args& a) {
  if (stats == 2)
    hipLaunchKernelGGL((c1::conv1x1_x2s_kernel<CPW, 2>), dim3(nwg), dim3(c1::NT), 0, st, a);
  else
    hipLaunchKernelGGL((c1::conv1x1_x2s_kernel<CPW, 1>), dim3(nwg), dim3(c1::NT), 0, st, a);
}

YS_EXPORT int yolosod_conv1x1x2_silu_stats(const float* x, long x_bstride, float* y, long y_bstride, int B, int cin,
                                           int cout, int HW, const float* bias, const void* prep, size_t prep_bytes,
                                           int stats, int parts, float* psum, float* pmax, float* tile_ws,
                                           void* stream) {
  YS_CHECK_ARG(x && y && bias && prep && psum && tile_ws, "conv1x1x2_stats: null pointer");
  YS_CHECK_ARG((stats == 1 || stats == 2) && (stats == 1 || pmax) && parts >= 1, "conv1x1x2_stats: stats=%d parts=%d",
               stats, parts);
  YS_CHECK_ARG(B >= 0 && HW > 0 && HW % 4 == 0 && cout % 128 == 0 && yolosod_conv1x1x2_prep_bytes(cin, cout) > 0,
               "conv1x1x2_stats: bad shape");
  YS_CHECK_ARG(x_bstride >= (long)cin * HW && y_bstride >= (long)cout * HW, "conv1x1x2_stats: batch strides too small");
  YS_CHECK_ARG((long)c1_pad(cin) * HW * 4 < (1L << 32), "conv1x1x2_stats: image too large for 32-bit buffer offsets");
  YS_CHECK_ARG(((uintptr_t)y & 15) == 0 && y_bstride % 4 == 0, "conv1x1x2_stats: output must be 16-byte aligned");
  if (B == 0) return 0;
  SplitPrep sp;
  YS_CHECK_ARG(split_prep_carve(prep, prep_bytes, c1_halves(cin, cout), &sp),
               "conv1x1x2_stats: prepared block too small");
  const int ntile = (HW + 63) / 64;
  float* tsum = tile_ws;
  float* tmax = tile_ws + (long)B * cout * ntile;
  c1::Args a{x, x_bstride, sp.wp, bias, y, y_bstride, tsum, tmax - tsum, 0, cin, cout, HW, ntile, range_flag_dev(),
             sp.flag, nullptr, 0, cin, 0};
  const bool g256 = (c1_form(B, cout, HW) & 3) == 2;
  const long nwg = (long)B * ntile * (cout / (g256 ? 256 : 128));
  YS_CHECK_ARG(nwg < (1L << 31), "conv1x1x2_stats: too many tiles");
  hipStream_t st = (hipStream_t)stream;
  if (g256) c1_launch_stats<4>(stats, (unsigned)nwg, st, a);
  else c1_launch_stats<2>(stats, (unsigned)nwg, st, a);
  thin_stats_reduce_launch(tsum, stats == 2 ? tmax : nullptr, (long)B * cout, ntile, parts, psum,
                           stats == 2 ? pmax : nullptr, st);
  YS_CHECK_LAUNCH("conv1x1x2_stats");
  return 0;
}
```

yolo-sod_amd/csrc/conv1x1x2_kernel.h:

```cpp

#ifdef YS_C1_STATS_FORMS
template <int CPW, int STATS>
__global__ __launch_bounds__(NT, 2) void conv1x1_x2s_kernel(Args p) {
  constexpr bool DUAL = false, DB = false;
  constexpr int NP = 64;
  static_assert(STATS == 1 || STATS == 2, "STATS");
#else
template <bool DUAL, int NP, int CPW = 2, bool DB = false>
__global__ __launch_bounds__(NT, 2) void conv1x1_x2_kernel(Args p) {
  constexpr int STATS = 0;
#endif
  constexpr int PL = NP * PS;
  constexpr int NITEM = (KS / 4) * NP;
  constexpr int NIT = NITEM / NT;
  constexpr int NPB = NP / 16;
  static_assert(NITEM % NT == 0, "items");
  __shared__ __attribute__((aligned(16))) h16_t Pl[(DB ? 4 : 2) * PL];
  const int tid = threadIdx.x, lane = tid & 63, wid = __builtin_amdgcn_readfirstlane(tid >> 6);
  const int l15 = lane & 15, g = lane >> 4;
  const int ngrp = p.cout / (64 * CPW);
  const int grp = blockIdx.x % ngrp, tile = (blockIdx.x / ngrp) % p.ntile, b = blockIdx.x / (ngrp * p.ntile);
  const int HW = p.HW, p0 = tile * NP, nst = (p.cin + KS - 1) / KS, nks = nst * (KS / 32);
  float rng = 0.f;

  auto rsrc = [&](const void* base, unsigned bytes) {
    const unsigned long long a = (unsigned long long)base;
    return __builtin_amdgcn_make_buffer_rsrc(
        (void*)(((unsigned long long)__builtin_amdgcn_readfirstlane((unsigned)(a >> 32)) << 32) |
                (unsigned)__builtin_amdgcn_readfirstlane((unsigned)a)),
        (short)0, __builtin_amdgcn_readfirstlane(bytes), 0x00020000);
  };
  const float* xb1 = p.x + (long)b * p.xbs;
  const float* xb2 = p.x2 ? p.x2 + (long)b * p.x2bs : xb1;
  const int HW1 = p.up_w ? HW >> 2 : HW;
  const unsigned nb1 = (unsigned)((long)p.k1 * HW1 * 4), nb2 = (unsigned)((long)(p.cin - p.k1) * HW * 4);
  const __amdgpu_buffer_rsrc_t rw = rsrc(p.wp, (unsigned)((long)nks * (p.cout >> 4) * 2 * 1024));

  static_assert(NT % NP == 0, "a thread stages one pixel");
  const int q0 = tid / NP;
  const int pc = min(p0 + tid % NP, HW - 1);
  int pc1 = pc;
  if (p.up_w) {
    const int yy = pc / p.up_w, xx = pc - yy * p.up_w;
    pc1 = (yy >> 1) * (p.up_w >> 1) + (xx >> 1);
  }
  f32x4 sv[NIT];
  auto load_part = [&](int st, int k0, int k1, bool live) __attribute__((always_inline)) {
    const bool second = KS * st >= p.k1;
    const int chs = second ? HW : HW1;
    const unsigned sx = (unsigned)((second ? KS * st - p.k1 : KS * st) * chs * 4);
    const unsigned vo = (unsigned)((4 * q0 * chs + (second ? pc : pc1)) * 4);
    const __amdgpu_buffer_rsrc_t r = rsrc(second ? xb2 : xb1, live ? (second ? nb2 : nb1) : 0u);
#pragma unroll
    for (int k = 0; k < 4 * NIT; ++k)
      if (k >= k0 && k < k1)
        sv[k >> 2][k & 3] = __builtin_bit_cast(
            float, __builtin_amdgcn_raw_buffer_load_b32(
                       r, vo + sx + (unsigned)((4 * (NT / NP) * (k >> 2) + (k & 3)) * chs * 4), 0, 0));
  };
  const int cb0 = grp * 4 * CPW + CPW * wid;
  auto wfrag = [&](int s, int u, int pl) __attribute__((always_inline)) {
    const int st = __builtin_amdgcn_readfirstlane((s * (p.cout >> 4) * 2) * 1024);
    return __builtin_bit_cast(f16x8_t, __builtin_amdgcn_raw_buffer_load_b128(
                                           rw, (unsigned)((((cb0 + u) * 2 + pl) * 64 + lane) * 16), st, 0));
  };
  f32x4 acc[CPW][NPB];
#pragma unroll
  for (int u = 0; u < CPW; ++u)
#pragma unroll
    for (int k = 0; k < NPB; ++k) acc[u][k] = f32x4{0.f, 0.f, 0.f, 0.f};
  float bo[CPW];
#pragma unroll
  for (int u = 0; u < CPW; ++u) bo[u] = p.bias[16 * (cb0 + u) + l15];

  auto stage_store = [&](h16_t* pl) __attribute__((always_inline)) {
#pragma unroll
    for (int i = 0; i < NIT; ++i) {
      const int e = tid + NT * i, quad = e / NP, px = e - quad * NP;
      uint2 hh, ll;
      split4x(sv[i], hh, ll);
      rng = range_acc(rng, sv[i]);
      h16_t* d = pl + px * PS + 4 * quad;
      *reinterpret_cast<uint2*>(d) = hh;
      *reinterpret_cast<uint2*>(d + PL) = ll;
    }
  };
  load_part(0, 0, 4 * NIT, true);
  if (DB) {
    stage_store(Pl);
    __syncthreads();
  }
  for (int st = 0; st < nst; ++st) {
    const h16_t* cur = DB ? Pl + (st & 1) * 2 * PL : Pl;
    if (!DB) {
      __syncthreads();
      stage_store(Pl);
      __syncthreads();
    }
    const bool nlive = st + 1 < nst;
    const int stn = nlive ? st + 1 : st;
    f16x8_t wa[CPW][2], wn[CPW][2];
#pragma unroll
    for (int u = 0; u < CPW; ++u) {
      wa[u][0] = wfrag(4 * st, u, 0);
      wa[u][1] = wfrag(4 * st, u, 1);
    }
    __builtin_amdgcn_sched_barrier(0);
#pragma unroll
    for (int kk = 0; kk < KS / 32; ++kk) {
      const int sn = kk + 1 < KS / 32 ? 4 * st + kk + 1 : 4 * st + kk;
#pragma unroll
      for (int u = 0; u < CPW; ++u) {
        wn[u][0] = wfrag(sn, u, 0);
        wn[u][1] = wfrag(sn, u, 1);
      }
      load_part(stn, NIT * kk, NIT * kk + NIT, nlive);
      __builtin_amdgcn_sched_barrier(0);
#pragma unroll
      for (int k = 0; k < NPB; ++k) {
        const h16_t* src = cur + (16 * k + l15) * PS + 32 * kk + 8 * g;
        const f16x8_t xh = *reinterpret_cast<const f16x8_t*>(src);
        const f16x8_t xl = *reinterpret_cast<const f16x8_t*>(src + PL);
#pragma unroll
        for (int u = 0; u < CPW; ++u) {
          f32x4 c = __builtin_amdgcn_mfma_f32_16x16x32_f16(xh, wa[u][1], acc[u][k], 0, 0, 0);
          c = __builtin_amdgcn_mfma_f32_16x16x32_f16(xl, wa[u][0], c, 0, 0, 0);
          acc[u][k] = __builtin_amdgcn_mfma_f32_16x16x32_f16(xh, wa[u][0], c, 0, 0, 0);
        }
      }
#pragma unroll
      for (int u = 0; u < CPW; ++u) {
        wa[u][0] = wn[u][0];
        wa[u][1] = wn[u][1];
      }
    }
    if (DB && nlive) {
      stage_store(Pl + ((st + 1) & 1) * 2 * PL);
      __syncthreads();
    }
  }
  float* yb = p.y + (long)b * p.ybs;
#pragma unroll
  for (int u = 0; u < CPW; ++u) {
    const int o = 16 * (cb0 + u) + l15;
    float ts = 0.f, tm = -INFINITY;
#pragma unroll
    for (int k = 0; k < NPB; ++k) {
      const int px = p0 + 16 * k + 4 * g;
      f32x4 v;
#pragma unroll
      for (int j = 0; j < 4; ++j) v[j] = silu_fast_(acc[u][k][j] * (1.0f / WSC) + bo[u]);
      if (px < HW) {
        __builtin_nontemporal_store(v, reinterpret_cast<f32x4*>(yb + (long)o * HW + px));
        if (DUAL && o >= p.c2lo)
          __builtin_nontemporal_store(
              v, reinterpret_cast<f32x4*>(p.y2 + (long)b * p.y2bs + (long)(o - p.c2lo) * HW + px));
        if (STATS) {
          ts += (v[0] + v[1]) + (v[2] + v[3]);
          if (STATS == 2) tm = nmax_(tm, nmax4_(v[0], v[1], v[2], v[3]));
        }
      }
    }
// ... 18 lines not shown
```

yolo-sod_amd/csrc/conv_epilogue.hip:

```cpp
#include "common.h"
#include <math.h>

namespace ys {


template <int ACT, bool RES, bool DUAL = false, class T = float>
__global__ __launch_bounds__(256) void bias_act_kernel(const T* __restrict__ y, T* __restrict__ out,
                                                       const float* __restrict__ bias, const T* __restrict__ res,
                                                       int C, long HW4, long y_bs4, long o_bs4, long r_bs4,
                                                       long total4, int rev, T* __restrict__ out2 = nullptr,
                                                       int c2lo = 0, long o2_bs4 = 0) {
  for (long i0 = (long)blockIdx.x * 256 + threadIdx.x; i0 < total4; i0 += (long)gridDim.x * 256) {
    const long i = rev ? total4 - 1 - i0 : i0;
    const long b = i / ((long)C * HW4);
    const long rem = i - b * (long)C * HW4;
    const int c = (int)(rem / HW4);
    const float bc = bias[c];
    f32x4 v = ld4(y + 4 * (b * y_bs4 + rem));
    v += bc;
    if (ACT == 1) {
      v.x = silu_st<T>(v.x); v.y = silu_st<T>(v.y); v.z = silu_st<T>(v.z); v.w = silu_st<T>(v.w);
    }
    if (RES) v += ld4(res + 4 * (b * r_bs4 + rem));
    st4(out + 4 * (b * o_bs4 + rem), v);
// ... 121 lines not shown
  }
  __syncthreads();
  if (tid == 0) {
    psum[bx] = (ss[0] + ss[1]) + (ss[2] + ss[3]);
    if (MAX) pmax[bx] = nmax4_(sm[0], sm[1], sm[2], sm[3]);
  }
}

template <int ACT, bool RES, class T = float>
__global__ __launch_bounds__(256) void bias_act_capool_kernel(const T* __restrict__ y, T* __restrict__ out,
                                                              const float* __restrict__ bias,
                                                              const T* __restrict__ res, int C, int H, int W,
                                                              int RB, long y_bs, long o_bs, long r_bs,
                                                              float* __restrict__ yin) {
  extern __shared__ __attribute__((aligned(16))) float band[];
  const long plane = blockIdx.x;
  const long b = plane / C;
  const int c = (int)(plane - b * C);
  const long HW = (long)H * W;
  const T* yp = y + b * y_bs + (long)c * HW;
  T* op = out + b * o_bs + (long)c * HW;
  const T* rp = RES ? res + b * r_bs + (long)c * HW : nullptr;
  float* o = yin + plane * (long)(H + W);
  const float bc = bias[c];
  const int tid = threadIdx.x;
  const int W4 = W >> 2, NG = 256 / W4;
  const int cq = tid % W4, rg = tid / W4;
  f32x4* band4 = reinterpret_cast<f32x4*>(band);
  f32x4 col = f32x4{0.f, 0.f, 0.f, 0.f};
  const float invW = 1.0f / (float)W;
  for (int h0 = 0; h0 < H; h0 += RB) {
    const int rb = (H - h0 < RB) ? H - h0 : RB;
    const int n4 = rb * W4;
    const long base = (long)h0 * W;
    f32x4 v[8], r[8];
#pragma unroll
    for (int u = 0; u < 8; ++u) {
      const int i = tid + 256 * u < n4 ? tid + 256 * u : n4 - 1;
      v[u] = ld4(yp + base + 4 * i);
      if (RES) r[u] = ld4(rp + base + 4 * i);
    }
#pragma unroll
    for (int u = 0; u < 8; ++u) {
      f32x4 t = v[u] + bc;
      if (ACT == 1) {
        t.x = silu_st<T>(t.x); t.y = silu_st<T>(t.y); t.z = silu_st<T>(t.z); t.w = silu_st<T>(t.w);
      }
      if (RES) t += r[u];
      v[u] = t;
    }
#pragma unroll
    for (int u = 0; u < 8; ++u) {
      const int i = tid + 256 * u;
      if (i < n4) {
        f32x4 t = v[u];
        st4(op + base + 4 * i, t);
        if (sizeof(T) == 2) t = round_bf16(t);
        band4[i] = t;
      }
    }
    __syncthreads();
    for (int rr = tid >> 2; rr < rb; rr += 64) {
      f32x4 s4 = f32x4{0.f, 0.f, 0.f, 0.f};
      for (int q = tid & 3; q < W4; q += 4) s4 += band4[rr * W4 + q];
      const float sm = quad_sum((s4.x + s4.y) + (s4.z + s4.w));
      if ((tid & 3) == 0) o[h0 + rr] = sm * invW;
    }
    if (rg < NG)
      for (int rr = rg; rr < rb; rr += NG) col += band4[rr * W4 + cq];
    __syncthreads();
  }
  float* cpart = band + (long)RB * W;
  if (rg < NG) reinterpret_cast<f32x4*>(cpart)[rg * W4 + cq] = col;
  __syncthreads();
  const float invH = 1.0f / (float)H;
  for (int w = tid; w < W; w += 256) {
    float s = 0.f;
    for (int g = 0; g < NG; ++g) s += cpart[g * W + w];
    o[H + w] = s * invH;
  }
}


template <int M, int K, bool RES, bool DUAL, bool STATS = false, bool UP = false>
__global__ __launch_bounds__(256, 2) void conv1x1_thin_kernel(const float* __restrict__ x, long x_bs,
                                                              const float* __restrict__ w,
                                                              const float* __restrict__ bias, float* __restrict__ out,
                                                              long o_bs, const float* __restrict__ res, long r_bs,
                                                              float* __restrict__ out2, long o2_bs, int c2lo, int HW,
                                                              int ntile, int rev, float* __restrict__ tsum = nullptr,
                                                              float* __restrict__ tmax = nullptr,
                                                              const float* __restrict__ x2 = nullptr, long x2_bs = 0,
                                                              int k1 = K, int up_w = 0) {
  constexpr int RB = M / 64;
  constexpr int KQ = K / 4;
  constexpr int XS = 68;
  __shared__ __attribute__((aligned(16))) float xs[K * XS];
  const int tid = threadIdx.x, lane = tid & 63, wid = tid >> 6;
  const int l15 = lane & 15, g = lane >> 4;
  const int b = rev ? gridDim.y - 1 - blockIdx.y : blockIdx.y;
  const float* xb = x + (long)b * x_bs;
  const float* xb2 = x2 ? x2 + (long)b * x2_bs - (long)k1 * HW : xb;
  float4 a[RB][KQ / 4];
#pragma unroll
  for (int rb = 0; rb < RB; ++rb) {
    const float* wr = w + (long)(wid * (M / 4) + rb * 16 + l15) * K + g * KQ;
#pragma unroll
    for (int t = 0; t < KQ / 4; ++t) a[rb][t] = *reinterpret_cast<const float4*>(wr + 4 * t);
  }
  float bv[RB][4];
#pragma unroll
  for (int rb = 0; rb < RB; ++rb)
#pragma unroll
    for (int r = 0; r < 4; ++r) bv[rb][r] = bias[wid * (M / 4) + rb * 16 + 4 * g + r];
  for (int tile = blockIdx.x; tile < ntile; tile += gridDim.x) {
    const int p0 = tile * 64;
    __syncthreads();
    if (UP) {
      const int pp = p0 + 4 * (tid & 15), yy = pp / up_w, xx = pp - yy * up_w;
      const float* xu = xb + (yy >> 1) * (up_w >> 1) + (xx >> 1);
      const int hw1 = HW >> 2;
#pragma unroll 4
      for (int e = tid; e < k1 * 16; e += 256) {
        const int row = e >> 4, c4 = e & 15;
        const float2 s2 = *reinterpret_cast<const float2*>(xu + (long)row * hw1);
        *reinterpret_cast<float4*>(xs + row * XS + 4 * c4) = make_float4(s2.x, s2.x, s2.y, s2.y);
      }
#pragma unroll 4
      for (int e = k1 * 16 + tid; e < K * 16; e += 256) {
        const int row = e >> 4, c4 = e & 15;
        *reinterpret_cast<float4*>(xs + row * XS + 4 * c4) =
            *reinterpret_cast<const float4*>(xb2 + (long)row * HW + p0 + 4 * c4);
      }
    } else {
#pragma unroll 4
      for (int e = tid; e < K * 16; e += 256) {
        const int row = e >> 4, c4 = e & 15;
        *reinterpret_cast<float4*>(xs + row * XS + 4 * c4) =
            *reinterpret_cast<const float4*>((row < k1 ? xb : xb2) + (long)row * HW + p0 + 4 * c4);
      }
    }
    __syncthreads();
    f32x4 acc[RB][4];
#pragma unroll
    for (int rb = 0; rb < RB; ++rb)
#pragma unroll
      for (int pb = 0; pb < 4; ++pb) acc[rb][pb] = f32x4{0.f, 0.f, 0.f, 0.f};
#pragma unroll
    for (int t4 = 0; t4 < KQ / 4; ++t4)
#pragma unroll
      for (int c = 0; c < 4; ++c) {
        const float* xr = xs + (g * KQ + 4 * t4 + c) * XS + l15;
        float bx[4];
#pragma unroll
        for (int pb = 0; pb < 4; ++pb) bx[pb] = xr[16 * pb];
#pragma unroll
        for (int rb = 0; rb < RB; ++rb) {
          const float av = c == 0 ? a[rb][t4].x : c == 1 ? a[rb][t4].y : c == 2 ? a[rb][t4].z : a[rb][t4].w;
#pragma unroll
          for (int pb = 0; pb < 4; ++pb) acc[rb][pb] = __builtin_amdgcn_mfma_f32_16x16x4f32(av, bx[pb], acc[rb][pb], 0, 0, 0);
        }
      }
#pragma unroll
    for (int rb = 0; rb < RB; ++rb)
#pragma unroll
      for (int r = 0; r < 4; ++r) {
        const int row = wid * (M / 4) + rb * 16 + 4 * g + r;
        float ts = 0.f, tm = -INFINITY;
#pragma unroll
        for (int pb = 0; pb < 4; ++pb) {
          const int p = p0 + pb * 16 + l15;
          float v = siluf_(acc[rb][pb][r] + bv[rb][r]);
          if (RES) v += res[(long)b * r_bs + (long)row * HW + p];
          out[(long)b * o_bs + (long)row * HW + p] = v;
          if (DUAL && row >= c2lo) out2[(long)b * o2_bs + (long)(row - c2lo) * HW + p] = v;
          if (STATS) {
            ts += v;
            tm = nmax_(tm, v);
          }
        }
        if (STATS) {
#pragma unroll
          for (int o = 1; o < 16; o <<= 1) {
            ts += __shfl_xor(ts, o, 64);
            tm = nmax_(tm, __shfl_xor(tm, o, 64));
          }
          if (l15 == 0) {
            const long ti = ((long)b * M + row) * ntile + tile;
            tsum[ti] = ts;
            tmax[ti] = tm;
          }
        }
      }
  }
}

__global__ __launch_bounds__(256) void thin_stats_reduce_kernel(const float* __restrict__ tsum,
                                                                const float* __restrict__ tmax, long planes, int ntile,
                                                                int parts, float* __restrict__ psum,
                                                                float* __restrict__ pmax) {
  const long plane = (long)blockIdx.x * 4 + (threadIdx.x >> 6);
  const int lane = threadIdx.x & 63;
  if (plane >= planes) return;
  float s = 0.f, m = -INFINITY;
  for (int t = lane; t < ntile; t += 64) {
    s += tsum[plane * ntile + t];
    if (tmax) m = nmax_(m, tmax[plane * ntile + t]);
  }
  s = wave_sum(s);
  m = wave_nmax(m);
  for (int k = lane; k < parts; k += 64) {
    psum[plane * parts + k] = k == 0 ? s : 0.f;
    if (pmax) pmax[plane * parts + k] = k == 0 ? m : -INFINITY;
  }
}

void thin_stats_reduce_launch(const float* tsum, const float* tmax, long planes, int ntile, int parts, float* psum,
                              float* pmax, hipStream_t st) {
  hipLaunchKernelGGL(thin_stats_reduce_kernel, dim3((unsigned)((planes + 3) / 4)), dim3(256), 0, st, tsum, tmax, planes,
                     ntile, parts, psum, pmax);
}

template <class E>
__global__ __launch_bounds__(256) void upsample2x_kernel(const E* __restrict__ x, E* __restrict__ out, long ob, int C,
                                                         int h, int w, long quads) {
  const int wq = w >> 2;
  for (long q = (long)blockIdx.x * 256 + threadIdx.x; q < quads; q += (long)gridDim.x * 256) {
    const long row = q / wq;
    const int j = (int)(q - row * wq) * 4;
    const long plane = row / h;
    const int i = (int)(row - plane * h);
    const int b = (int)(plane / C), c = (int)(plane - (long)b * C);
    E* o = out + (long)b * ob + ((long)c * 2 * h + 2 * i) * (2L * w) + 2 * j;
    if (sizeof(E) == 4) {
      const uint4 v = *reinterpret_cast<const uint4*>(x + row * w + j);
      const uint4 lo = make_uint4(v.x, v.x, v.y, v.y), hi = make_uint4(v.z, v.z, v.w, v.w);
      uint4* o0 = reinterpret_cast<uint4*>(o);
      uint4* o1 = reinterpret_cast<uint4*>(o + 2L * w);
      o0[0] = lo; o0[1] = hi; o1[0] = lo; o1[1] = hi;
    } else {
      const uint2 v = *reinterpret_cast<const uint2*>(x + row * w + j);
      const uint32_t e0 = v.x & 0xffffu, e1 = v.x >> 16, e2 = v.y & 0xffffu, e3 = v.y >> 16;
      const uint4 d = make_uint4(e0 | (e0 << 16), e1 | (e1 << 16), e2 | (e2 << 16), e3 | (e3 << 16));
      *reinterpret_cast<uint4*>(o) = d;
      *reinterpret_cast<uint4*>(o + 2L * w) = d;
    }
  }
}

}

using namespace ys;

YS_EXPORT int yolosod_upsample2x(const void* x, void* out, long out_bstride, int B, int C, int h, int w, int elem_bytes,
                                 void* stream) {
  YS_CHECK_ARG(x && out, "upsample2x: null pointer");
  YS_CHECK_ARG(B >= 0 && C > 0 && h > 0 && w > 0 && (elem_bytes == 4 || elem_bytes == 2), "upsample2x: bad shape");
  YS_CHECK_ARG(w % 4 == 0 && ((uintptr_t)x & 15) == 0 && ((uintptr_t)out & 15) == 0 &&
                   (out_bstride * elem_bytes) % 16 == 0 && (4L * h * w * elem_bytes) % 16 == 0 &&
                   out_bstride >= 4L * C * h * w,
               "upsample2x: w %% 4, 16-byte alignment and a batch stride >= C*4*h*w required");
  if (B == 0) return 0;
  const long quads = (long)B * C * h * (w / 4);
  const unsigned grid = (unsigned)((quads + 255) / 256 < 8192 ? (quads + 255) / 256 : 8192);
  hipStream_t st = (hipStream_t)stream;
  if (elem_bytes == 4)
    hipLaunchKernelGGL(upsample2x_kernel<uint32_t>, dim3(grid), dim3(256), 0, st, (const uint32_t*)x, (uint32_t*)out,
                       out_bstride, C, h, w, quads);
  else
    hipLaunchKernelGGL(upsample2x_kernel<uint16_t>, dim3(grid), dim3(256), 0, st, (const uint16_t*)x, (uint16_t*)out,
                       out_bstride, C, h, w, quads);
  YS_CHECK_LAUNCH("upsample2x");
  return 0;
}

template <class T>
static int bias_act_stats_impl(const T* y, long y_bstride, T* out, long out_bstride, const float* bias, const T* res,
                               long res_bstride, int B, int C, long HW, int act, int parts, long seg, float* psum,
// ... 121 lines not shown
#undef YS_BAC
  YS_CHECK_LAUNCH("bias_act_capool");
  return 0;
}

YS_EXPORT int yolosod_bias_act_stats(const float* y, long y_bstride, float* out, long out_bstride, const float* bias,
                                     const float* res, long res_bstride, int B, int C, long HW, int act, int parts,
                                     long seg, float* psum, float* pmax, void* stream) {
  return bias_act_stats_impl(y, y_bstride, out, out_bstride, bias, res, res_bstride, B, C, HW, act, parts, seg, psum,
                             pmax, stream);
}

YS_EXPORT int yolosod_bias_act(const float* y, long y_bstride, float* out, long out_bstride, const float* bias,
                               const float* res, long res_bstride, int B, int C, long HW, int act, void* stream) {
  return bias_act_impl(y, y_bstride, out, out_bstride, bias, res, res_bstride, (float*)nullptr, 0L, 0, B, C, HW, act,
                       stream);
}

YS_EXPORT int yolosod_bias_act_dual(const float* y, long y_bstride, float* out, long out_bstride, const float* bias,
                                    const float* res, long res_bstride, float* out2, long out2_bstride, int c2lo,
                                    int B, int C, long HW, int act, void* stream) {
  YS_CHECK_ARG(out2, "bias_act_dual: null pointer");
  return bias_act_impl(y, y_bstride, out, out_bstride, bias, res, res_bstride, out2, out2_bstride, c2lo, B, C, HW, act,
                       stream);
}

YS_EXPORT int yolosod_bias_act_capool(const float* y, long y_bstride, float* out, long out_bstride, const float* bias,
                                      const float* res, long res_bstride, int B, int C, int H, int W, int act,
                                      float* yin, void* stream) {
  return bias_act_capool_impl(y, y_bstride, out, out_bstride, bias, res, res_bstride, B, C, H, W, act, yin, stream);
}

YS_EXPORT int yolosod_bias_act_bf16(const bf16_t* y, long y_bstride, bf16_t* out, long out_bstride, const float* bias,
                                    const bf16_t* res, long res_bstride, bf16_t* out2, long out2_bstride, int c2lo,
                                    int B, int C, long HW, int act, void* stream) {
  return bias_act_impl(y, y_bstride, out, out_bstride, bias, res, res_bstride, out2, out2_bstride, c2lo, B, C, HW, act,
                       stream);
}
YS_EXPORT int yolosod_bias_act_stats_bf16(const bf16_t* y, long y_bstride, bf16_t* out, long out_bstride,
                                          const float* bias, const bf16_t* res, long res_bstride, int B, int C,
                                          long HW, int act, int parts, long seg, float* psum, float* pmax,
                                          void* stream) {
  return bias_act_stats_impl(y, y_bstride, out, out_bstride, bias, res, res_bstride, B, C, HW, act, parts, seg, psum,
                             pmax, stream);
}
YS_EXPORT int yolosod_bias_act_capool_bf16(const bf16_t* y, long y_bstride, bf16_t* out, long out_bstride,
                                           const float* bias, const bf16_t* res, long res_bstride, int B, int C, int H,
                                           int W, int act, float* yin, void* stream) {
  return bias_act_capool_impl(y, y_bstride, out, out_bstride, bias, res, res_bstride, B, C, H, W, act, yin, stream);
}

YS_EXPORT int yolosod_conv1x1_thin(const float* x, long x_bs, const float* w, const float* bias, float* out, long out_bs,
                                   const float* res, long res_bs, float* out2, long out2_bs, int c2lo, int B, int Cin,
                                   int Cout, long HW, void* stream) {
  YS_CHECK_ARG(x && w && bias && out, "conv1x1_thin: null pointer");
  YS_CHECK_ARG(HW % 64 == 0 && HW < (1L << 30), "conv1x1_thin: HW=%ld must be a multiple of 64", HW);
  YS_CHECK_ARG(Cout == 64 || Cout == 128, "conv1x1_thin: Cout=%d unsupported", Cout);
  YS_CHECK_ARG(x_bs % 4 == 0 && out_bs % 4 == 0 && (!res || res_bs % 4 == 0) && (!out2 || out2_bs % 4 == 0),
               "conv1x1_thin: batch strides must be multiples of 4");
  YS_CHECK_ARG((((uintptr_t)x | (uintptr_t)w | (uintptr_t)out) & 15) == 0, "conv1x1_thin: pointers must be 16-byte aligned");
  YS_CHECK_ARG(!out2 || (c2lo >= 0 && c2lo < Cout), "conv1x1_thin: c2lo=%d", c2lo);
  if (B == 0) return 0;
  const int ntile = (int)(HW / 64);
  const int gx = ntile < 4 ? ntile : (ntile + 3) / 4;
  hipStream_t st = (hipStream_t)stream;
  const dim3 grid((unsigned)gx, (unsigned)B);
  bool ok = false;
#define YS_THIN(M_, K_)                                                                                            \
  if (Cout == M_ && Cin == K_) {                                                                                   \
    ok = true;                                                                                                     \
    if (res && out2) hipLaunchKernelGGL((conv1x1_thin_kernel<M_, K_, true, true>), grid, dim3(256), 0, st, x, x_bs, w, bias, out, out_bs, res, res_bs, out2, out2_bs, c2lo, (int)HW, ntile, mall_reverse()); \
    else if (res) hipLaunchKernelGGL((conv1x1_thin_kernel<M_, K_, true, false>), grid, dim3(256), 0, st, x, x_bs, w, bias, out, out_bs, res, res_bs, out2, out2_bs, c2lo, (int)HW, ntile, mall_reverse()); \
    else if (out2) hipLaunchKernelGGL((conv1x1_thin_kernel<M_, K_, false, true>), grid, dim3(256), 0, st, x, x_bs, w, bias, out, out_bs, res, res_bs, out2, out2_bs, c2lo, (int)HW, ntile, mall_reverse()); \
    else hipLaunchKernelGGL((conv1x1_thin_kernel<M_, K_, false, false>), grid, dim3(256), 0, st, x, x_bs, w, bias, out, out_bs, res, res_bs, out2, out2_bs, c2lo, (int)HW, ntile, mall_reverse()); \
  }
  YS_THIN(64, 64) YS_THIN(64, 96) YS_THIN(64, 128) YS_THIN(64, 192) YS_THIN(64, 256)
  YS_THIN(128, 64) YS_THIN(128, 96) YS_THIN(128, 128) YS_THIN(128, 192) YS_THIN(128, 256)
#undef YS_THIN
  YS_CHECK_ARG(ok, "conv1x1_thin: Cin=%d unsupported", Cin);
  YS_CHECK_LAUNCH("conv1x1_thin");
  return 0;
}

YS_EXPORT int yolosod_conv1x1_thin_cat(const float* x, long x_bs, const float* x2, long x2_bs, int k1, const float* w,
                                       const float* bias, float* out, long out_bs, float* out2, long out2_bs, int c2lo,
                                       int B, int Cin, int Cout, long HW, int up_w, void* stream) {
  YS_CHECK_ARG(x && x2 && w && bias && out, "conv1x1_thin_cat: null pointer");
  YS_CHECK_ARG(k1 > 0 && k1 < Cin, "conv1x1_thin_cat: k1=%d (Cin %d)", k1, Cin);
  YS_CHECK_ARG(HW % 64 == 0 && HW < (1L << 30), "conv1x1_thin_cat: HW=%ld must be a multiple of 64", HW);
  YS_CHECK_ARG(Cout == 64 || Cout == 128, "conv1x1_thin_cat: Cout=%d unsupported", Cout);
  YS_CHECK_ARG(x_bs % 4 == 0 && x2_bs % 4 == 0 && out_bs % 4 == 0 && (!out2 || out2_bs % 4 == 0),
               "conv1x1_thin_cat: batch strides must be multiples of 4");
  YS_CHECK_ARG((((uintptr_t)x | (uintptr_t)x2 | (uintptr_t)w | (uintptr_t)out) & 15) == 0,
               "conv1x1_thin_cat: pointers must be 16-byte aligned");
  YS_CHECK_ARG(!out2 || (c2lo >= 0 && c2lo < Cout), "conv1x1_thin_cat: c2lo=%d", c2lo);
  YS_CHECK_ARG(up_w == 0 || (up_w > 0 && up_w % 4 == 0 && HW % up_w == 0 && (HW / up_w) % 2 == 0 &&
                             x_bs >= (long)k1 * (HW / 4)),
               "conv1x1_thin_cat: upsampled part needs W %% 4 == 0 and an even H (W=%d, HW=%ld)", up_w, HW);
  if (B == 0) return 0;
  const int ntile = (int)(HW / 64);
  const int gx = ntile < 4 ? ntile : (ntile + 3) / 4;
  hipStream_t st = (hipStream_t)stream;
  const dim3 grid((unsigned)gx, (unsigned)B);
  bool ok = false;
#define YS_THINC(M_, K_)                                                                                          \
  if (Cout == M_ && Cin == K_) {                                                                                  \
    ok = true;                                                                                                    \
    if (out2 && up_w) hipLaunchKernelGGL((conv1x1_thin_kernel<M_, K_, false, true, false, true>), grid, dim3(256), 0, st, x, x_bs, w, \
                                 bias, out, out_bs, nullptr, 0L, out2, out2_bs, c2lo, (int)HW, ntile, mall_reverse(), \
                                 nullptr, nullptr, x2, x2_bs, k1, up_w);                                           \
    else if (up_w) hipLaunchKernelGGL((conv1x1_thin_kernel<M_, K_, false, false, false, true>), grid, dim3(256), 0, st, x, x_bs, w, bias, \
                            out, out_bs, nullptr, 0L, nullptr, 0L, 0, (int)HW, ntile, mall_reverse(), nullptr, nullptr, \
                            x2, x2_bs, k1, up_w);                                                                  \
    else if (out2) hipLaunchKernelGGL((conv1x1_thin_kernel<M_, K_, false, true>), grid, dim3(256), 0, st, x, x_bs, w, \
                                 bias, out, out_bs, nullptr, 0L, out2, out2_bs, c2lo, (int)HW, ntile, mall_reverse(), \
                                 nullptr, nullptr, x2, x2_bs, k1);                                                 \
    else hipLaunchKernelGGL((conv1x1_thin_kernel<M_, K_, false, false>), grid, dim3(256), 0, st, x, x_bs, w, bias,  \
                            out, out_bs, nullptr, 0L, nullptr, 0L, 0, (int)HW, ntile, mall_reverse(), nullptr, nullptr, \
                            x2, x2_bs, k1);                                                                        \
  }
  YS_THINC(64, 64) YS_THINC(64, 96) YS_THINC(64, 128) YS_THINC(64, 192) YS_THINC(64, 256)
  YS_THINC(128, 64) YS_THINC(128, 96) YS_THINC(128, 128) YS_THINC(128, 192) YS_THINC(128, 256)
#undef YS_THINC
  YS_CHECK_ARG(ok, "conv1x1_thin_cat: Cin=%d unsupported", Cin);
  YS_CHECK_LAUNCH("conv1x1_thin_cat");
  return 0;
}

YS_EXPORT int yolosod_conv1x1_thin_stats(const float* x, long x_bs, const float* w, const float* bias, float* out,
                                         long out_bs, int B, int Cin, int Cout, long HW, int parts, float* psum,
                                         float* pmax, float* tile_ws, void* stream) {
  YS_CHECK_ARG(x && w && bias && out && psum && tile_ws, "conv1x1_thin_stats: null pointer");
  YS_CHECK_ARG(HW % 64 == 0 && HW < (1L << 30), "conv1x1_thin_stats: HW=%ld must be a multiple of 64", HW);
  YS_CHECK_ARG(Cout == 64 || Cout == 128, "conv1x1_thin_stats: Cout=%d unsupported", Cout);
  YS_CHECK_ARG(parts >= 1, "conv1x1_thin_stats: parts=%d", parts);
  YS_CHECK_ARG(x_bs % 4 == 0 && out_bs % 4 == 0, "conv1x1_thin_stats: batch strides must be multiples of 4");
  YS_CHECK_ARG((((uintptr_t)x | (uintptr_t)w | (uintptr_t)out) & 15) == 0,
               "conv1x1_thin_stats: pointers must be 16-byte aligned");
  if (B == 0) return 0;
  const int ntile = (int)(HW / 64);
  const int gx = ntile < 4 ? ntile : (ntile + 3) / 4;
  hipStream_t st = (hipStream_t)stream;
  const dim3 grid((unsigned)gx, (unsigned)B);
  float* tsum = tile_ws;
  float* tmax = tile_ws + (long)B * Cout * ntile;
  bool ok = false;
#define YS_THINS(M_, K_)                                                                                          \
  if (Cout == M_ && Cin == K_) {                                                                                  \
    ok = true;                                                                                                    \
    hipLaunchKernelGGL((conv1x1_thin_kernel<M_, K_, false, false, true>), grid, dim3(256), 0, st, x, x_bs, w, bias, \
                       out, out_bs, nullptr, 0L, nullptr, 0L, 0, (int)HW, ntile, mall_reverse(), tsum, tmax);                   \
  }
  YS_THINS(64, 64) YS_THINS(64, 96) YS_THINS(64, 128) YS_THINS(64, 192) YS_THINS(64, 256)
  YS_THINS(128, 64) YS_THINS(128, 96) YS_THINS(128, 128) YS_THINS(128, 192) YS_THINS(128, 256)
#undef YS_THINS
  YS_CHECK_ARG(ok, "conv1x1_thin_stats: Cin=%d unsupported", Cin);
  const long planes = (long)B * Cout;
  hipLaunchKernelGGL(thin_stats_reduce_kernel, dim3((unsigned)((planes + 3) / 4)), dim3(256), 0, st, tsum, tmax, planes,
                     ntile, parts, psum, pmax);
  YS_CHECK_LAUNCH("conv1x1_thin_stats");
  return 0;
}
```

yolo-sod_amd/nn/modules.py:

```python
from __future__ import annotations

import contextlib
import math
import os
from collections.abc import Sequence

import torch
import torch.nn as nn
import torch.nn.functional as F

from .. import _hip

__all__ = (
    "Conv", "DWConv", "Concat", "Bottleneck", "C2f", "SPPF", "DFL", "SE", "SE_Block", "CBAM_Block",
    "ChannelAttention", "SpatialAttention", "CA_Block", "h_sigmoid", "A2_Attn", "WindowAttention", "SwinBlock",
    "Conv1x1BN", "GLUBlock", "MambaBlock", "Detect",
)


def autopad(k, p=None, d=1):
    if d > 1:
        k = d * (k - 1) + 1 if isinstance(k, int) else [d * (x - 1) + 1 for x in k]
    if p is None:
        p = k // 2 if isinstance(k, int) else [x // 2 for x in k]
# ... 29 lines not shown
    if isinstance(v, (tuple, list)):
        for t in v:
            d = _cuda_device(t)
            if d is not None:
                return d
    return None


def _record_stream(v, stream):
    if isinstance(v, torch.Tensor):
        if v.is_cuda:
            v.record_stream(stream)
    elif isinstance(v, (tuple, list)):
        for t in v:
            _record_stream(t, stream)


def _f32(mod: nn.Module, tag: str, *ts):
    if all(t.dtype == torch.float32 and t.is_contiguous() for t in ts):
        return tuple(t.detach() for t in ts)
    return _cached(mod, tag, ts, lambda: tuple(t.detach().float().contiguous() for t in ts))


def _as(mod: nn.Module, tag: str, dtype, *ts):
    if all(t.dtype == dtype and t.is_contiguous() for t in ts):
        return tuple(t.detach() for t in ts)
    return _cached(mod, tag, ts, lambda: tuple(t.detach().to(dtype).contiguous() for t in ts))


def _act_code(act):
    if isinstance(act, nn.SiLU):
        return 1
    if isinstance(act, nn.Identity):
        return 0
    return None


THIN1X1 = os.environ.get("YOLOSOD_THIN1X1", "1") == "1"
CONV3X3 = os.environ.get("YOLOSOD_CONV3X3", "1")
S2_NECK = os.environ.get("YOLOSOD_S2_NECK", "1") != "0"
S1_BACKBONE_DEFAULT, S2_BACKBONE_DEFAULT = "1", "10"
S2_BACKBONE_LAYERS = (7, 10)


def _backbone_switch(value: str, layers=()):
    v = value.strip()
    if v in ("0", "1"):
        return v == "1"
    try:
        picked = frozenset(int(t) for t in v.split(","))
    except ValueError:
        picked = frozenset()
    if not picked or not picked <= frozenset(layers):
        raise ValueError(f"backbone switch {value!r}: expected 0, 1"
                         + (f" or layers out of {tuple(layers)}" if layers else ""))
    return True if picked == frozenset(layers) else picked


S2_BACKBONE = _backbone_switch(os.environ.get("YOLOSOD_S2_BACKBONE", S2_BACKBONE_DEFAULT), S2_BACKBONE_LAYERS)
S1_BACKBONE = _backbone_switch(os.environ.get("YOLOSOD_S1_BACKBONE", S1_BACKBONE_DEFAULT))
S1_NECK = os.environ.get("YOLOSOD_S1_NECK", "1") != "0"
N1_NECK = os.environ.get("YOLOSOD_N1_NECK", "1") != "0"
N1_BACKBONE_DEFAULT = "8,11,13"
N1_BACKBONE_LAYERS = (6, 8, 11, 13)
N1_BACKBONE = _backbone_switch(os.environ.get("YOLOSOD_N1_BACKBONE", N1_BACKBONE_DEFAULT), N1_BACKBONE_LAYERS)
N1_STATS_DEFAULT = "17,22,31"
N1_STATS_LAYERS = (17, 22, 31)
N1_STATS = _backbone_switch(os.environ.get("YOLOSOD_N1_STATS", N1_STATS_DEFAULT), N1_STATS_LAYERS)
C2F_SLICES = os.environ.get("YOLOSOD_C2F_SLICES", "1") != "0"
SPPF_HIP = os.environ.get("YOLOSOD_SPPF_HIP", "1") != "0"
STEM_HIP = os.environ.get("YOLOSOD_STEM_HIP", "1") != "0"


def _onoff_switch(name: str, value: str) -> bool:
    v = value.strip()
    if v not in ("0", "1"):
        raise ValueError(f"{name}={value!r}: expected 0 or 1")
    return v == "1"


BOTTLENECK_FUSE = _onoff_switch("YOLOSOD_BOTTLENECK_FUSE", os.environ.get("YOLOSOD_BOTTLENECK_FUSE", "1"))
HEAD_FUSE_DEFAULT = "1"
HEAD_FUSE = _onoff_switch("YOLOSOD_HEAD_FUSE", os.environ.get("YOLOSOD_HEAD_FUSE", HEAD_FUSE_DEFAULT))


def _s2_on(s2, layer=None):
    if not s2:
        return False
    if s2 != "backbone":
        return S2_NECK
    if layer is None or isinstance(S2_BACKBONE, bool):
        return S2_BACKBONE
    return layer in S2_BACKBONE


def _s1_on(s1) -> bool:
    return bool(s1) and (S1_BACKBONE if s1 == "backbone" else S1_NECK)


def _n1_on(n1, layer=None):
    if not n1:
        return False
    if n1 != "backbone":
        return N1_NECK
    if layer is None or isinstance(N1_BACKBONE, bool):
        return bool(N1_BACKBONE)
    return layer in N1_BACKBONE


def _n1_stats_on(stats_layer) -> bool:
    if stats_layer is None:
        return False
    if isinstance(N1_STATS, bool):
        return N1_STATS
    return stats_layer in N1_STATS


def _n1_run(conv, x, out, out2, c2lo, n1, stats=None):
    prep = _prep(conv, "c1prep", _hip.conv1x1x2_prepare)
    return _hip.conv1x1x2_silu(x, conv.bias, prep, conv.out_channels, out=out, out2=out2, c2lo=c2lo,
                               op="conv1x1x2_backbone" if n1 == "backbone" else "conv1x1x2", stats=stats)


def conv_epilogue(conv: nn.Conv2d, act_code, x, out=None, res=None, stats=None, out2=None, c2lo=0, tower=False,
                  s2=False, s1=False, n1=False, layer=None, stats_layer=None):
    if x.device.type != "cuda" or conv.bias is None or act_code is None or x.dtype not in (torch.float32,
                                                                                           torch.bfloat16):
        return None
    split = _hip.split_convs_enabled()
    if isinstance(x, _hip.CatView):
        if act_code == 1 and res is None and stats is None and conv.kernel_size == (1, 1):
            if split and _n1_on(n1, layer) and _hip.conv1x1x2_ok(x, conv) and (
                    out is None or _hip._imgs_contig(out)) and (out2 is None or _hip._imgs_contig(out2)):
                return _n1_run(conv, x, out, out2, c2lo, n1)
            if (THIN1X1 and conv.out_channels == 64 and conv.stride == (1, 1) and conv.groups == 1
                    and conv.padding == (0, 0) and _hip.conv1x1_thin_ok(x, conv.out_channels)
                    and (out is None or out.data_ptr() % 16 == 0)):
                return _hip.conv1x1_thin(x, conv.weight.detach().reshape(conv.out_channels, -1), conv.bias.detach(),
                                         out=out, out2=out2, c2lo=c2lo)
        x = x.materialize()
    if (split and act_code == 1 and out is None and res is None and stats is None and out2 is None and CONV3X3 != "0"
            and (CONV3X3 == "all" or tower) and _hip.conv3x3_ok(x, conv)):
        prep = _prep(conv, "c3prep", _hip.conv3x3_prepare)
        return _hip.conv3x3_silu(x, conv.bias, prep, conv.out_channels)
    if (split and _n1_on(n1, layer) and act_code == 1 and res is None
            and (stats is None or (n1 is True and out2 is None and stats in ("sum", "summax", "capool")
                                   and _n1_stats_on(stats_layer)))
            and _hip.conv1x1x2_ok(x, conv) and (out is None or _hip._imgs_contig(out))
            and (out2 is None or _hip._imgs_contig(out2))):
        return _n1_run(conv, x, out, out2, c2lo, n1, stats)
    if (split and _s1_on(s1) and act_code == 1 and stats is None and out2 is None and _hip.conv3x3_ok(x, conv)
            and x.shape[3] % 4 == 0 and (res is None or _hip._imgs_contig(res))):
        prep = _prep(conv, "c3prep", _hip.conv3x3_prepare)
        return _hip.conv3x3_silu(x, conv.bias, prep, conv.out_channels, out=out, res=res,
                                 op="conv3x3_backbone" if s1 == "backbone" else "conv3x3")
    if (split and _s2_on(s2, layer) and act_code == 1 and res is None and stats is None and out2 is None
            and _hip.conv3x3s2_ok(x, conv)):
        prep = _prep(conv, "c3s2prep", _hip.conv3x3s2_prepare)
        key = ("conv3x3s2_backbone", tuple(x.shape), (conv.out_channels, False, False)) if s2 == "backbone" else None
        return _hip.conv3x3s2_silu(x, conv.bias, prep, conv.out_channels, key=key, out=out)
    if (THIN1X1 and act_code == 1 and (stats is None or (stats in ("sum", "summax") and res is None and out2 is None))
            and conv.out_channels == 64 and conv.kernel_size == (1, 1) and conv.stride == (1, 1)
            and conv.groups == 1 and conv.padding == (0, 0) and _hip.conv1x1_thin_ok(x, conv.out_channels)
            and (out is None or out.data_ptr() % 16 == 0) and (res is None or res.data_ptr() % 16 == 0)):
        return _hip.conv1x1_thin(x, conv.weight.detach().reshape(conv.out_channels, -1), conv.bias.detach(),
                                 out=out, res=res, out2=out2, c2lo=c2lo, stats=stats)
    y = F.conv2d(x, conv.weight, None, conv.stride, conv.padding, conv.dilation, conv.groups)
    if (y.shape[2] * y.shape[3]) % 4 or y.dtype != x.dtype:
        y = y + conv.bias.view(1, -1, 1, 1)
        y = F.silu(y) if act_code == 1 else y
        if res is not None:
            y = y + res
        if out2 is not None:
            out2.copy_(y[:, c2lo:])
        if out is not None:
            out.copy_(y)
            return out
        return y
    (bias,) = _f32(conv, "bias", conv.bias)
    return _hip.bias_act(y, bias, act_code, out=out, res=res, stats=stats, out2=out2, c2lo=c2lo)


def catview_route(cv, c0, c1, H, W, dtype) -> bool:
    conv = cv.conv
    if (dtype != torch.float32 or not cv.is_fused() or conv.bias is None or _act_code(cv.act) != 1
            or cv.emit_stats is not None or conv.kernel_size != (1, 1) or conv.stride != (1, 1) or conv.groups != 1
            or conv.padding != (0, 0) or conv.in_channels != c0 + c1):
        return False
    if cv.n1 and N1_NECK and _hip.split_convs_enabled() and c0 % 128 == 0 and c1 % 32 == 0 and (H * W) % 4 == 0 and int(
            _hip.load_library().yolosod_conv1x1x2_prep_bytes(c0 + c1, conv.out_channels)) > 0:
        return True
    return (THIN1X1 and conv.out_channels == 64 and c0 + c1 in _hip.THIN1X1_CIN and (H * W) % 64 == 0
            and c0 % 4 == 0 and c1 % 4 == 0)


class Conv(nn.Module):

    default_act = nn.SiLU()
    emit_stats = None
    tower = False
    s2 = False
    s2_backbone = False
    layer = None
    s1 = False
    s1_backbone = False
    n1 = False
    n1_backbone = False
    n1_layer = None
    n1_stats_layer = None
    stem = False

    def __init__(self, c1, c2, k=1, s=1, p=None, g=1, d=1, act=True):
        super().__init__()
        self.conv = nn.Conv2d(c1, c2, k, s, autopad(k, p, d), groups=g, dilation=d, bias=False)
        self.bn = nn.BatchNorm2d(c2)
        self.act = self.default_act if act is True else act if isinstance(act, nn.Module) else nn.Identity()

    def forward(self, x):
        return self.act(self.bn(self.conv(x)))

    def gated_ok(self, x) -> bool:
        return (not hasattr(self, "bn") and self.conv.bias is not None and isinstance(self.act, nn.SiLU)
                and _hip.split_convs_enabled() and _hip.conv3x3s2_ok(x, self.conv))

    def forward_gated(self, x, gate_c, gate_p, key):
        cv = self.conv
        prep = _prep(cv, "c3s2prep", _hip.conv3x3s2_prepare)
        return _hip.conv3x3s2_silu(x, cv.bias, prep, cv.out_channels, gate_c, gate_p, key=key)

    def forward_fuse(self, x, out=None, res=None, out2=None, c2lo=0):
        if (self.stem and STEM_HIP and self.emit_stats == "sum" and out is None and res is None and out2 is None
                and isinstance(self.act, nn.SiLU) and _hip.stem_ok(x, self.conv)):
            return _hip.stem_conv(x, self.conv.weight.detach(), self.conv.bias.detach())
        y = conv_epilogue(self.conv, _act_code(self.act), x, out, res, self.emit_stats, out2, c2lo, self.tower,
                          "backbone" if self.s2_backbone else self.s2, self.s1_mark(),
                          "backbone" if self.n1_backbone else self.n1,
                          self.n1_layer if self.n1_backbone else self.layer, self.n1_stats_layer)
        if y is not None:
            return y
        if isinstance(x, _hip.CatView):
            x = x.materialize()
        y = self.act(self.conv(x))
        if res is not None:
            y = y + res
        if out2 is not None:
            out2.copy_(y[:, c2lo:])
        if out is not None:
            out.copy_(y)
            return out
        return y

    def is_fused(self):
        return not hasattr(self, "bn")

    def s1_mark(self):
        return "backbone" if self.s1_backbone else self.s1


class DWConv(Conv):

    def __init__(self, c1, c2, k=1, s=1, d=1, act=True):
        super().__init__(c1, c2, k, s, g=math.gcd(c1, c2), d=d, act=act)


class Concat(nn.Module):
    def __init__(self, dimension=1):
        super().__init__()
        self.d = dimension

    def forward(self, x):
        return torch.cat(x, self.d)


class Bottleneck(nn.Module):
    def __init__(self, c1, c2, shortcut=True, g=1, k=(3, 3), e=0.5):
        super().__init__()
        c_ = int(c2 * e)
        self.cv1 = Conv(c1, c_, k[0], 1)
        self.cv2 = Conv(c_, c2, k[1], 1, g=g)
        self.add = shortcut and c1 == c2

    def _one_launch(self, x, out, out2) -> bool:
        if not (BOTTLENECK_FUSE and out2 is None and x.device.type == "cuda" and x.dtype == torch.float32
                and _hip.split_convs_enabled() and x.dim() == 4 and x.shape[1] == 32 and x.shape[3] % 4 == 0):
            return False
        for cv in (self.cv1, self.cv2):
            c = cv.conv
            if not (cv.is_fused() and c.bias is not None and _act_code(cv.act) == 1 and cv.emit_stats is None
                    and _s1_on(cv.s1_mark()) and c.in_channels == 32 and c.out_channels == 32
                    and _hip.conv3x3_ok(x, c)):
                return False
        if not _hip._imgs_contig(x) or (out is not None and not _hip._imgs_contig(out)):
            return False
        return _hip.bottleneck3x3_fused(x.shape[0], x.shape[2], x.shape[3])

    def forward(self, x, out=None, out2=None):
        if self._one_launch(x, out, out2):
            c1, c2 = self.cv1.conv, self.cv2.conv
            prep1 = _prep(c1, "c3prep", _hip.conv3x3_prepare)
            prep2 = _prep(c2, "c3prep", _hip.conv3x3_prepare)
            backbone = self.cv2.s1_mark() == "backbone"
            return _hip.bottleneck3x3_silu(x, c1.bias, prep1, c2.bias, prep2, out=out, res=x if self.add else None,
                                           op="bottleneck3x3_backbone" if backbone else "bottleneck3x3")
        if self.cv2.is_fused():
            return self.cv2.forward_fuse(self.cv1(x), out=out, res=x if self.add else None, out2=out2)
        y = x + self.cv2(self.cv1(x)) if self.add else self.cv2(self.cv1(x))
        if out2 is not None:
            out2.copy_(y)
        if out is not None:
            out.copy_(y)
            return out
        return y

# ... 558 lines not shown
```

yolo-sod_amd/nn/tasks.py:

```python
from __future__ import annotations

import ast
import contextlib
import copy
import hashlib
import math
import os
import re
from pathlib import Path

import numpy as np
import torch
import torch.nn as nn
import yaml

from .. import _hip
from . import modules as M

CFG_DIR = Path(__file__).resolve().parent.parent / "cfg"

_STREAMS_ENV = os.environ.get("YOLOSOD_STREAMS")
STREAMS = int(_STREAMS_ENV) if _STREAMS_ENV is not None else 1
SIDE_STREAMS = max(1, int(os.environ.get("YOLOSOD_SIDE_STREAMS", "2")))
GATE_FUSE = os.environ.get("YOLOSOD_GATE_FUSE", "1") != "0"
# ... 103 lines not shown
            ch = []
        ch.append(c2)
    return nn.Sequential(*layers), sorted(save)


def initialize_weights(model: nn.Module) -> None:
    for m in model.modules():
        t = type(m)
        if t is nn.BatchNorm2d:
            m.eps = 1e-3
            m.momentum = 0.03
        elif t in {nn.Hardswish, nn.LeakyReLU, nn.ReLU, nn.ReLU6, nn.SiLU}:
            m.inplace = True


def state_dict_sha256(model: nn.Module) -> str:
    h = hashlib.sha256()
    for k, v in model.state_dict().items():
        h.update(k.encode())
        h.update(v.detach().cpu().contiguous().numpy().tobytes())
    return h.hexdigest()


class BaseModel(nn.Module):
    def forward(self, x, *args, **kwargs):
        return self.predict(x, *args, **kwargs)

    def predict(self, x, profile=False, visualize=False, augment=False, embed=None):
        if augment:
            return self._predict_augment(x)
        return self._predict_once(x)

    def _predict_augment(self, x):
        raise NotImplementedError(f"{type(self).__name__} does not support augment=True")

    def _predict_once(self, x):
        if x.device.type == "cuda" and getattr(self, "_fused", False):
            return self._predict_once_planned(x)
        y = []
        for m in self.model:
            if m.f != -1:
                x = y[m.f] if isinstance(m.f, int) else [x if j == -1 else y[j] for j in m.f]
            x = m(x)
            y.append(x if m.i in self.save else None)
        return x

    def _concat_producers(self):
        plan = getattr(self, "_cplan", None)
        if plan is not None:
            return plan
        plan = {}
        for c, m in enumerate(self.model):
            if not isinstance(m, M.Concat) or m.d != 1 or not isinstance(m.f, (list, tuple)) or -1 not in m.f:
                continue
            p = c - 1
            prod = self.model[p]
            if p in self.save or sum(1 for j in m.f if j in (-1, p)) != 1:
                continue
            if (isinstance(prod, M.Conv) and prod.is_fused() and prod.emit_stats is None) or (
                    isinstance(prod, nn.Upsample) and prod.mode == "nearest" and prod.size is None
                    and prod.scale_factor in (2, 2.0, (2, 2), (2.0, 2.0))):
                plan[p] = c
        self._cplan = plan
        return plan

    def _gate_consumers(self):
        plan = getattr(self, "_gplan", None)
        if plan is not None:
            return plan
        plan = {}
        det = self.model[-1]
        busy = set(self._concat_producers()) | (set(det.f) if isinstance(det, M.Detect) and isinstance(
            det.f, (list, tuple)) else set())
        for k in range(len(self.model) - 1):
            m, nxt = self.model[k], self.model[k + 1]
            if (isinstance(m, (M.SE, M.CBAM_Block)) and k not in self.save and k + 1 not in busy
                    and isinstance(nxt, M.Conv)
                    and not isinstance(nxt, M.DWConv) and nxt.f == -1 and nxt.conv.kernel_size == (3, 3)
                    and nxt.conv.stride == (2, 2) and nxt.conv.groups == 1 and nxt.conv.out_channels in (64, 128)):
                plan[k] = nxt
        self._gplan = plan
        return plan

    def _predict_once_planned(self, x):
        plan = self._concat_producers()
        det = self.model[-1]
        towers = lvl = main = side = None
        img_hw = tuple(x.shape[2:])
        streams = STREAMS
        if _STREAMS_ENV is None and x.dtype == torch.bfloat16:
            streams = 2
        if (streams > 0 and isinstance(det, M.Detect) and isinstance(det.f, (list, tuple)) and len(set(det.f)) == len(det.f)
                and det._fused_ok([x])):
            lvl = {j: k for k, j in enumerate(det.f)}
            towers = {}
            ready = []
            last_mafn = max((k for k, mm in enumerate(self.model)
                             if isinstance(mm, (M.SE, M.CBAM_Block, M.CA_Block, M.A2_Attn, M.SwinBlock))), default=-1)
            main = torch.cuda.current_stream(x.device)
            side = getattr(self, "_side_streams", None)
            if side is None or len(side) != SIDE_STREAMS or side[0].device != x.device:
                side = self._side_streams = [torch.cuda.Stream(device=x.device) for _ in range(SIDE_STREAMS)]
            rr = 0
            head_y = None
            lvl_in = {}
            head_hw = [_level_hw(img_hw, float(s)) for s in det.stride]
        y = []
        pend = {}
        cvpend = {}
        elided = 0
        gplan = self._gate_consumers() if GATE_FUSE else {}
        gated = None
        for m in self.model:
            if gated is not None:
                xg, gc, gp, key = gated
                gated = None
                x = m.forward_gated(xg, gc, gp, key)
                y.append(x if m.i in self.save else None)
                continue
            inp = x
            if m.f != -1:
                inp = y[m.f] if isinstance(m.f, int) else [x if j == -1 else y[j] for j in m.f]
            cons = gplan.get(m.i)
            if cons is not None and isinstance(inp, torch.Tensor) and cons.gated_ok(inp):
                if isinstance(m, M.SE):
                    gc, gp = m.gate(inp), None
                    key = ("se_conv", tuple(inp.shape), (cons.conv.out_channels, m.fc1.out_channels))
                else:
                    gc, gp = m.gates(inp)
                    key = ("cbam_conv", tuple(inp.shape),
                           (cons.conv.out_channels, m.channel_attention.fc[0].out_channels))
                gated = (inp, gc, gp, key)
                x = None
                y.append(None)
                continue
            c = plan.get(m.i)
            if c is not None and isinstance(inp, torch.Tensor) and inp.dim() == 4:
                cat = self.model[c]
                B, _, H, W = inp.shape
                if isinstance(m, nn.Upsample):
                    H, W = 2 * H, 2 * W
                    cp = inp.shape[1]
                else:
                    cv = m.conv
                    cp = cv.out_channels
                    H, W = ((n + 2 * p - d * (k - 1) - 1) // s + 1 for n, p, d, k, s in
                            zip((H, W), cv.padding, cv.dilation, cv.kernel_size, cv.stride))
                srcs = [None if j == -1 else y[j] for j in cat.f]
                chans = [cp if s is None else s.shape[1] for s in srcs]
                nxt = self.model[c + 1] if c + 1 < len(self.model) else None
                if (CATVIEW and len(srcs) == 2 and c not in self.save and isinstance(nxt, M.C2f) and nxt.f == -1
                        and all(s is None or (s.shape[0], s.shape[2], s.shape[3]) == (B, H, W) for s in srcs)
                        and M.catview_route(nxt.cv1, chans[0], chans[1], H, W, inp.dtype)):
                    up0 = False
                    if isinstance(m, nn.Upsample):
                        if (UPVIEW and cat.f[0] == -1 and inp.dtype == torch.float32 and inp.is_contiguous()
                                and inp.data_ptr() % 16 == 0 and W % 4 == 0):
                            x, up0 = inp, True
                        else:
                            x = torch.empty((B, cp, H, W), dtype=inp.dtype, device=inp.device)
                            if not (UPSAMPLE_HIP and _hip.upsample2x_into(inp, x)):
                                x = m(inp)
                    else:
                        x = m(inp)
                    cvpend[c] = (up0,)
                    y.append(None)
                    continue
                if all(s is None or (s.shape[0], s.shape[2], s.shape[3]) == (B, H, W) for s in srcs):
                    buf = torch.empty((B, sum(chans), H, W), dtype=inp.dtype, device=inp.device)
                    offs = [sum(chans[:i]) for i in range(len(chans))]
                    k = [j for j in cat.f].index(-1)
                    out = buf[:, offs[k]:offs[k] + cp]
                    if isinstance(m, nn.Upsample):
                        h, w = inp.shape[2], inp.shape[3]
                        if not (UPSAMPLE_HIP and _hip.upsample2x_into(inp, out)):
                            out.view(B, cp, h, 2, w, 2).copy_(inp[:, :, :, None, :, None].expand(B, cp, h, 2, w, 2))
                    else:
                        m.forward_fuse(inp, out=out)
                    pend[c] = (buf, offs, chans)
                    x = out
                    y.append(None)
                    continue
            cvp = cvpend.pop(m.i, None)
            if cvp is not None:
                x = _hip.CatView([x if j == -1 else y[j] for j in m.f], up0=cvp[0])
                elided += 1
            elif m.i in pend:
                buf, offs, chans = pend.pop(m.i)
                elided += 1
                for j, o, n in zip(m.f, offs, chans):
                    if j != -1:
                        buf[:, o:o + n].copy_(y[j])
                x = buf
            elif m is det and towers is not None and len(towers) == det.nl:
                feats = [towers[k] for k in range(det.nl)]
                for sd in side:
                    main.wait_stream(sd)
                if head_y is None:
                    x = det.forward_towers(feats)
                else:
                    ins = [lvl_in[k] for k in range(det.nl)]
                    if [tuple(t.shape[2:]) for t in ins] == head_hw:
                        x = det.forward_levels(head_y, feats, ins)
                    else:
                        x = det.forward_towers([f if f is not None else det.tower_features(k, ins[k])
                                                for k, f in enumerate(feats)])
            else:
                x = m(inp)
            if towers is not None and m is not det:
                if m.i in lvl:
                    ready.append((lvl[m.i], x))
                if ready and (streams != 2 or m.i >= last_mafn):
                    for k, xk in ready:
                        lvl_in[k] = xk
                        if (None not in head_hw and tuple(xk.shape[2:]) == head_hw[k]
                                and det.head_fuse_level(k, xk)):
                            if head_y is None:
                                head_off = [sum(h * w for h, w in head_hw[:j]) for j in range(det.nl + 1)]
                                head_y = torch.empty((xk.shape[0], 4 + det.nc, head_off[-1]), dtype=torch.float32,
                                                     device=xk.device)
                            for mode in (1, 2):
                                sd = side[rr % len(side)]
                                rr += 1
                                sd.wait_stream(main)
                                xk.record_stream(sd)
                                head_y.record_stream(sd)
                                with torch.cuda.stream(sd):
                                    det.tower_into(head_y, k, mode, xk, head_off[k])
                            towers[k] = None
                            continue
                        feats = []
                        for tower in (det.cv2[k], det.cv3[k]):
                            sd = side[rr % len(side)]
                            rr += 1
                            sd.wait_stream(main)
                            xk.record_stream(sd)
                            with torch.cuda.stream(sd):
                                f = tower[:-1](xk).contiguous()
                            f.record_stream(main)
                            feats.append(f)
                        towers[k] = tuple(feats)
                    ready = []
            y.append(x if m.i in self.save else None)
        self._last_elided = elided
        return x

    def is_fused(self, thresh=10):
        bn = tuple(v for k, v in nn.__dict__.items() if "Norm" in k)
        return sum(isinstance(v, bn) for v in self.modules()) < thresh

    def fuse(self, verbose=False):
        if not self.is_fused():
            for m in self.model.modules():
                if isinstance(m, M.Conv) and hasattr(m, "bn"):
                    m.conv = _fuse_conv_and_bn(m.conv, m.bn)
                    delattr(m, "bn")
                    m.forward = m.forward_fuse
        self._fused = True
        self._cplan = None
        return self


def _level_hw(img_hw, stride):
    h, w = img_hw
    n = int(round(math.log2(stride))) if stride >= 1 else -1
    if n < 0 or 2.0 ** n != stride:
        return None
    for _ in range(n):
        h, w = (h + 1) // 2, (w + 1) // 2
    return h, w


def _fuse_conv_and_bn(conv: nn.Conv2d, bn: nn.BatchNorm2d) -> nn.Conv2d:
    fused = nn.Conv2d(conv.in_channels, conv.out_channels, kernel_size=conv.kernel_size, stride=conv.stride,
                      padding=conv.padding, dilation=conv.dilation, groups=conv.groups,
                      bias=True).requires_grad_(False).to(conv.weight.device)
    with torch.no_grad():
        w, b = M.fold_conv_bn(conv, bn)
        fused.weight.copy_(w)
        fused.bias.copy_(b)
    return fused


def probe_manifest_path(yaml_file) -> Path:
    return CFG_DIR / (Path(yaml_file).stem + ".probe.npz")


class DetectionModel(BaseModel):

    def __init__(self, cfg="yolov12-sod-fusion-v5-simple.yaml", ch=3, nc=None, verbose=False, registry=None,
                 probe_stats: bool = True):
        super().__init__()
        self.yaml = cfg if isinstance(cfg, dict) else yaml_model_load(cfg)
        ch = self.yaml["ch"] = self.yaml.get("ch", ch)
        if nc and nc != self.yaml["nc"]:
            self.yaml["nc"] = nc
        self.model, self.save = parse_model(copy.deepcopy(self.yaml), ch=ch, verbose=verbose, registry=registry)
        self.names = {i: f"{i}" for i in range(self.yaml["nc"])}
        self.inplace = self.yaml.get("inplace", True)

        for i, m in enumerate(self.model):
            if i and m.f == -1 and isinstance(m, (M.SE, M.CBAM_Block, M.CA_Block)):
                prod = self.model[i - 1]
                conv = prod if isinstance(prod, M.Conv) else getattr(prod, "cv2", None)
                if isinstance(conv, M.Conv):
                    conv.emit_stats = ("summax" if isinstance(m, M.CBAM_Block) else
                                       "capool" if isinstance(m, M.CA_Block) else "sum")

        m0 = self.model[0]
        if (isinstance(m0, M.Conv) and not isinstance(m0, M.DWConv) and m0.emit_stats == "sum"
                and m0.conv.in_channels == 3 and m0.conv.kernel_size == (3, 3) and m0.conv.stride == (2, 2)
                and m0.conv.groups == 1):
            m0.stem = True

        n_backbone = len(self.yaml.get("backbone", []))
        for i, m in enumerate(self.model):
            if (isinstance(m, M.Conv) and not isinstance(m, M.DWConv)
                    and m.conv.kernel_size == (3, 3) and m.conv.stride == (2, 2) and m.conv.groups == 1):
                if i >= n_backbone:
                    m.s2 = True
                elif i and m.f == -1 and not isinstance(self.model[i - 1], (M.SE, M.CBAM_Block)):
                    m.s2_backbone = True
                    m.layer = i
            if isinstance(m, M.C2f):
                for bt in m.m:
                    for cv in (bt.cv1, bt.cv2):
                        if cv.conv.kernel_size == (3, 3) and cv.conv.stride == (1, 1) and cv.conv.groups == 1:
                            if i >= n_backbone:
                                cv.s1 = True
                            else:
                                cv.s1_backbone = True
            if i >= n_backbone:
                for cv in ([m] if isinstance(m, M.Conv) and not isinstance(m, M.DWConv) else
                           [m.cv1, m.cv2] if isinstance(m, M.C2f) else []):
                    if cv.conv.kernel_size == (1, 1) and cv.conv.groups == 1 and cv.conv.out_channels % 128 == 0:
                        cv.n1 = True
                        if cv.emit_stats is not None:
                            cv.n1_stats_layer = i
            elif isinstance(m, (M.C2f, M.SPPF)):
                for cv in (m.cv1, m.cv2):
                    if cv.conv.kernel_size == (1, 1) and cv.conv.groups == 1 and cv.conv.out_channels % 128 == 0:
                        cv.n1_backbone = True
# ... 92 lines not shown
```

yolo-sod_amd/perf.py:

```python
from __future__ import annotations

import os

F32 = 4

PEAK_HBM_GBS = 8000.0
PEAK_FP32_MFMA_TFLOPS = 157.3
PEAK_BF16_MFMA_TFLOPS = 2516.6


def elem_size(key) -> int:
    return key[3] if len(key) > 3 else F32


def peak_tflops(key) -> float:
    return PEAK_BF16_MFMA_TFLOPS if elem_size(key) == 2 else PEAK_FP32_MFMA_TFLOPS


def _on(name: str) -> bool:
    return os.environ.get(name, "1") != "0"


def method_peak_tflops(key) -> float:
    if elem_size(key) == 4:
        op = key[0]
        split = ((op == "swin" and key[1][1] in (64, 256) and _on("YOLOSOD_SWIN_X3"))
                 or (op == "a2" and _on("YOLOSOD_A2_X2")) or (op == "head" and _on("YOLOSOD_HEAD_X2"))
                 or op in FUSED_CONV)
        if split:
            return PEAK_BF16_MFMA_TFLOPS / 3
    return peak_tflops(key)


FUSED_CONV = {"se_conv": "se", "cbam_conv": "cbam"}
GATE_ONLY = {"se_gate": "se_conv", "cbam_gate": "cbam_conv"}
PATH_OPS = frozenset({"se", "cbam", "ca", "a2", "swin", "mamba", "decode", "head", "nms", *FUSED_CONV})


def swin_geom(H, W, ws=7):
    if H <= ws and W <= ws:
        return H, W, H, W
    wh, ww = min(ws, H), min(ws, W)
    return wh, ww, H + (wh - H % wh) % wh, W + (ww - W % ww) % ww


def op_cost(key):
    b, f = _op_cost(key[:3], elem_size(key))
    return b, f


def _op_cost(key, E):
    op, shape, extra = key
    if op in FUSED_CONV:
        B, C, H, W = shape
        cout, hid = extra
        Ho, Wo = (H + 1) // 2, (W + 1) // 2
        act = B * C * H * W * E + B * cout * Ho * Wo * E + (B * H * W * F32 if op == "cbam_conv" else 0)
        w = (cout * C * 9 + cout + 2 * C * hid + C + hid + (98 if op == "cbam_conv" else 0)) * F32
        flops = 2 * B * Ho * Wo * cout * C * 9 + B * C * H * W * (1 if op == "se_conv" else 2)
        return act + w, flops
    if op in ("se", "cbam", "ca"):
        B, C, H, W = shape
        hid = extra
        act = 2 * B * C * H * W * E
        w = (2 * C * hid + C + hid) * F32
        flops = B * C * H * W * (2 if op == "se" else 6)
        return act + w, flops
    if op == "a2":
        B, C, H, W = shape
        A, heads = extra
        L = A * W
        act = 2 * B * C * H * W * E
        w = (2 * (C * C + C) + 4 * C * C + 4 * C + 2 * C) * F32
        conv = 2 * 2 * C * C * H * W
        mha = 2 * L * C * 3 * C + 2 * L * C * C + 2 * 2 * L * L * C
        return act + w, B * (conv + mha)
    if op == "swin":
        B, C, H, W = shape
        heads, ws, hid = extra
        wh, ww, Hp, Wp = swin_geom(H, W, ws)
        L = wh * ww
        tok_p = Hp * Wp
        act = 2 * B * C * H * W * E
        w = (9 * C + 4 * C * C + 3 * C + C + 2 * C * hid + hid + C + C * C + 6 * C) * F32
        dense = tok_p * (2 * C * 3 * C + 2 * C * C + 2 * 2 * C * hid) + H * W * 2 * C * C
        attn = tok_p * 2 * 2 * L * C
        dw = H * W * 2 * 9 * C
        return act + w, B * (dense + attn + dw)
    if op == "mamba":
        B, C, H, W = shape
        ch, r = extra
        hd = 2 * ch
        hw, hwh = H * W, (H // r) * (W // r)
        act = 2 * B * C * hw * E
        w = (ch * C + 2 * hd * ch + 9 * hd + ch * hd + C * ch + 4 * (ch + hd + C)) * F32
        flops = 2 * ch * C * hw + hwh * (2 * 2 * hd * ch + 2 * 9 * hd + 2 * ch * hd + 2 * C * ch)
        return act + w, B * flops
    if op == "decode":
        B, A = shape
        nc = extra
        return B * A * ((64 + nc) + (4 + nc)) * F32, B * A * (64 * 4 + nc * 4)
    if op == "head":
        B, A = shape
        nc, c2, c3 = extra
        return (B * A * ((c2 + c3) * E + (4 + nc) * F32) + (64 * c2 + nc * c3 + 64 + nc) * F32,
                B * A * (2 * (64 * c2 + nc * c3) + 64 * 4 + nc * 4))
    if op == "nms":
        B, nc, A = shape
        return B * A * (4 + nc) * F32, 0
    raise KeyError(op)


def bound_of(key, method: bool = True) -> str:
    nbytes, flops = op_cost(key)
    peak = method_peak_tflops(key) if method else peak_tflops(key)
    return "mfma" if flops / (peak * 1e12) > nbytes / (PEAK_HBM_GBS * 1e9) else "hbm"


def t_min_ms(key, method: bool = False) -> float:
    nbytes, flops = op_cost(key)
    peak = method_peak_tflops(key) if method else peak_tflops(key)
    return max(nbytes / (PEAK_HBM_GBS * 1e9), flops / (peak * 1e12)) * 1e3



PRODUCER_GATE = {"sum": "se", "summax": "cbam", "capool": "ca"}


def _numel(shape) -> int:
    n = 1
    for d in shape:
        n *= d
    return n


def producer_of(key):
    op, shape, extra = key[:3]
    tail, E = tuple(key[3:]), elem_size(key)
    if op == "bias_act" and isinstance(extra, str) and extra.split("+")[0] in PRODUCER_GATE:
        st, res = extra.split("+")[0], extra.endswith("+res")
        plain = ("bias_act", tuple(shape), "res" if res else None) + tail
        return PRODUCER_GATE[st], tuple(shape), plain, _numel(shape) * E * (3 if res else 2)
    if op == "conv1x1_thin" and isinstance(extra, tuple) and len(extra) == 2 and extra[1] in ("sum", "summax"):
        B, cin, H, W = shape
        cout = extra[0]
        plain = ("conv1x1_thin", tuple(shape), (cout, False, False)) + tail
        return PRODUCER_GATE[extra[1]], (B, cout, H, W), plain, B * H * W * (cin + cout) * E
    if op == "conv1x1x2_stats" and isinstance(extra, tuple) and len(extra) == 2 and extra[1] in PRODUCER_GATE:
        B, cin, H, W = shape
        cout = extra[0]
        plain = ("conv1x1x2", tuple(shape), (cout, False)) + tail
        return PRODUCER_GATE[extra[1]], (B, cout, H, W), plain, B * H * W * (cin + cout) * E
    if op == "stem" and isinstance(extra, tuple) and len(extra) == 2 and extra[1] in PRODUCER_GATE:
        B, cin, H, W = shape
        cout = extra[0]
        plain = ("stem", tuple(shape), (cout, None)) + tail
        nbytes = B * (cin * H * W + cout * (H // 2) * (W // 2)) * E
        return PRODUCER_GATE[extra[1]], (B, cout, H // 2, W // 2), plain, nbytes
    return None


class PathSelect:

    def __init__(self):
        self.plain = set()

    def __call__(self, key):
        if key[0] in PATH_OPS or key[0] in GATE_ONLY:
            return True
        p = producer_of(key)
        if p is not None:
            self.plain.add(p[2])
            return True
        return key in self.plain


def aggregate(calls):
    agg = {}
    for key, ms in calls:
        a = agg.setdefault(key, [0.0, 0])
        a[0] += ms
        a[1] += 1
    return agg


def producer_billing(agg):
    out = {}
    for key, (tot, n) in agg.items():
        p = producer_of(key)
        if p is None:
            continue
        gate, gshape, plain, pbytes = p
        t_st = tot / n
        if plain in agg:
            t_pl = agg[plain][0] / agg[plain][1]
            basis = f"its in-model plain variant, {agg[plain][1]} launches"
        else:
            t_pl = pbytes / (PEAK_HBM_GBS * 1e9) * 1e3
            basis = "plain pass at the HBM roof (no plain variant of this shape in the model)"
        out[(gate, gshape)] = (max(0.0, t_st - t_pl),
                               f"{key[0]}{tuple(key[1])} {key[2]}: {t_st:.4f} ms in-model vs {t_pl:.4f} ms ({basis})")
    return out


def summarize(calls, steps):
    agg = aggregate(calls)
    billed = producer_billing(agg)
    gate_ms = {}
    for key, (tot, n) in agg.items():
        if key[0] in GATE_ONLY:
            k2 = (GATE_ONLY[key[0]], tuple(key[1]))
            gate_ms[k2] = gate_ms.get(k2, 0.0) + tot
    ops, backbone = [], []
    for key, (tot, n) in agg.items():
        if key[0] in GATE_ONLY:
            continue
        if key[0] not in PATH_OPS:
            backbone.append({"op": key[0], "shape": list(key[1]), "extra": str(key[2]), "launches": n,
                             "total_ms_per_step": round(tot / steps, 4)})
            continue
        nbytes, flops = op_cost(key)
        kern = tot / n + gate_ms.get((key[0], tuple(key[1])), 0.0) / n
        ext, src = billed.get((FUSED_CONV.get(key[0], key[0]), tuple(key[1])), (0.0, None))
        avg = kern + ext
        bound = bound_of(key)
        tm, tm_d = t_min_ms(key, method=True), t_min_ms(key)
        o = {"op": key[0], "shape": list(key[1]), "dtype": "bf16" if elem_size(key) == 2 else "f32",
             "launches": n, "avg_ms": round(avg, 4), "kernels_ms": round(kern, 4),
             "total_ms_per_step": round(avg * n / steps, 4),
             "GBps": round(nbytes / (avg * 1e-3) / 1e9, 1), "TFLOPs": round(flops / (avg * 1e-3) / 1e12, 2),
             "bound": bound, "peak": method_peak_tflops(key) if bound == "mfma" else PEAK_HBM_GBS,
             "t_min_ms": round(tm, 4), "frac": round(tm / avg, 3), "frac_vs_dtype_peak": round(tm_d / avg, 3),
             "bytes": nbytes, "flops": flops, "key": key}
        if src:
            o["producer_extra_ms"] = round(ext, 4)
            o["producer"] = src
        ops.append(o)
    ops.sort(key=lambda o: -o["total_ms_per_step"])
    t_meas = sum(o["total_ms_per_step"] for o in ops)
    t_min = sum(t_min_ms(o["key"], method=True) * o["launches"] / steps for o in ops)
    t_min_d = sum(t_min_ms(o["key"]) * o["launches"] / steps for o in ops)
    path = {"t_min_ms": round(t_min, 4), "t_meas_ms": round(t_meas, 4),
            "frac": round(t_min / t_meas, 4) if t_meas else None,
            "definition": "sum over hot-path ops of max(bytes / 8 TB/s, flops / matrix ceiling of the method the op "
                          "computes with: fp16 peak / 3 = 838.9 TF/s for the fp32 ops on fp16 two-term splits, 2516.6 "
                          "for bf16, 157.3 for exact fp32 MFMA) / measured; a producing epilogue's extra time for a "
                          "gate's statistics (in-model producer minus its in-model plain variant of the same shape) is "
                          "billed to the gate",
            "frac_vs_dtype_peak": round(t_min_d / t_meas, 4) if t_meas else None}
    path["mafn"] = mafn_path(ops, steps)
    return ops, sorted(backbone, key=lambda o: -o["total_ms_per_step"]), path



def _split_fused(key):
    op, shape, extra = key[:3]
    B, C, H, W = shape
    cout, hid = extra
    E = elem_size(key)
    Ho, Wo = (H + 1) // 2, (W + 1) // 2
    conv_b = (B * C * H * W + B * cout * Ho * Wo) * E + (cout * C * 9 + cout) * F32
    conv_f = 2 * B * Ho * Wo * cout * C * 9
    t_conv = max(conv_b / (PEAK_HBM_GBS * 1e9), conv_f / (PEAK_BF16_MFMA_TFLOPS / 3 * 1e12)) * 1e3
    return (FUSED_CONV[op], tuple(shape), hid) + tuple(key[3:]), t_conv


def mafn_path(ops, steps):
    t_min = t_meas = 0.0
    nbytes = 0
    parts = []
    for o in ops:
        key, n = o["key"], o["launches"]
        if key[0] in FUSED_CONV:
            k8, t_conv = _split_fused(key)
            meas = max(o["avg_ms"] - t_conv, 0.0)
        elif key[0] == "head":
            B, A = key[1]
            nc = key[2][0]
            k8, meas = ("decode", (B, A), nc) + tuple(key[3:]), o["avg_ms"]
        else:
            k8, meas = key, o["avg_ms"]
        b, _ = op_cost(k8)
        tm = t_min_ms(k8, method=True)
        nbytes += b * n / steps
        t_min += tm * n / steps
        t_meas += meas * n / steps
        parts.append(f"{k8[0]}{tuple(k8[1])}: {meas:.4f} ms")
    floor = nbytes / (PEAK_HBM_GBS * 1e9) * 1e3
    return {"bytes_per_step": int(nbytes), "t_hbm_floor_ms": round(floor, 4), "t_min_ms": round(t_min, 4),
            "t_meas_ms": round(t_meas, 4), "frac": round(t_min / t_meas, 4) if t_meas else None,
            "frac_vs_hbm_floor": round(floor / t_meas, 4) if t_meas else None,
            "definition": "SURVEY 8(d): MAFN instances + decode + NMS scan; gate-fused SE/CBAM billed without their "
                          "consumer conv (its t_min subtracted, its FLOPs excluded)", "instances": parts}



CSV_FIELDS = ("config", "steps", "seq", "op", "shape", "extra", "esize", "ms")


def calls_to_rows(config, steps, calls):
    return [{"config": config, "steps": steps, "seq": i, "op": k[0], "shape": "x".join(map(str, k[1])),
             "extra": repr(k[2]), "esize": k[3] if len(k) > 3 else "", "ms": f"{ms:.6f}"}
            for i, (k, ms) in enumerate(calls)]


def rows_to_calls(rows):
    import ast
    out = []
    for r in rows:
        key = (r["op"], tuple(int(d) for d in r["shape"].split("x")), ast.literal_eval(r["extra"]))
        if r["esize"] != "":
            key = key + (int(r["esize"]),)
        out.append((key, float(r["ms"])))
    return out
```

Before: 4623.

## Fuse neck SE/CBAM gate application into following 1x1 conv input loads

Adds a lazy GatedMap wrapper so neck SE/CBAM blocks only compute their gates. The gated map is never written out; the channel and spatial gates are applied while the next 1x1 conv (thin or split-fp16 form, including concat-view consumers) loads its input tile. A gate_apply kernel materializes the map only for readers that cannot take a gate. This is meant to remove a full activation write and re-read per neck attention block, at the cost of new kernel variants, planning logic and perf-accounting changes.

```diff
diff --git a/include/yolosod_hip.h b/include/yolosod_hip.h
--- a/include/yolosod_hip.h
+++ b/include/yolosod_hip.h
@@ -175,6 +175,10 @@
                              const float* bias, float* out, long out_bs, float* out2, long out2_bs, int c2lo, int B,
                              int Cin, int Cout, long HW, int up_w, void* stream);
 
+int yolosod_conv1x1_thin_gated(const float* x, long x_bs, const float* gate_c, const float* w, const float* bias,
+                               float* out, long out_bs, float* out2, long out2_bs, int c2lo, int B, int Cin, int Cout,
+                               long HW, void* stream);
+
 int yolosod_conv1x1_thin_stats(const float* x, long x_bs, const float* w, const float* bias, float* out, long out_bs,
                                int B, int Cin, int Cout, long HW, int parts, float* psum, float* pmax, float* tile_ws,
                                void* stream);
@@ -204,6 +208,8 @@
 int yolosod_cbam_gates(const float* x, int B, int C, int H, int W, const float* fc0_w, const float* fc2_w, int hidden,
                        const float* sa_w, const float* psum, const float* pmax, float* ca, float* sa, void* workspace,
                        size_t workspace_bytes, void* stream);
+int yolosod_gate_apply(const float* x, float* y, int B, int C, int H, int W, const float* gate_c, const float* gate_p,
+                       void* stream);
 size_t yolosod_conv3x3s2_prep_bytes(int cin, int cout);
 int yolosod_conv3x3s2_prepare(const float* w, int cin, int cout, void* prep, size_t prep_bytes, void* stream);
 int yolosod_conv3x3s2_silu(const float* x, float* y, int B, int cin, int cout, int H, int W, const float* bias,
@@ -219,6 +225,10 @@
 int yolosod_conv1x1x2_silu_cat(const float* x, long x_bstride, const float* x2, long x2_bstride, int k1, float* y,
                                long y_bstride, float* y2, long y2_bstride, int c2lo, int B, int cin, int cout, int HW,
                                const float* bias, const void* prep, size_t prep_bytes, int up_w, void* stream);
+int yolosod_conv1x1x2_silu_cat_gated(const float* x, long x_bstride, const float* x2, long x2_bstride, int k1,
+                                     const float* gate_c, const float* gate_p, float* y, long y_bstride, float* y2,
+                                     long y2_bstride, int c2lo, int B, int cin, int cout, int HW, const float* bias,
+                                     const void* prep, size_t prep_bytes, int up_w, void* stream);
 int yolosod_conv1x1x2_silu_stats(const float* x, long x_bstride, float* y, long y_bstride, int B, int cin, int cout,
                                  int HW, const float* bias, const void* prep, size_t prep_bytes, int stats, int parts,
                                  float* psum, float* pmax, float* tile_ws, void* stream);
diff --git a/yolo-sod_amd/_hip.py b/yolo-sod_amd/_hip.py
--- a/yolo-sod_amd/_hip.py
+++ b/yolo-sod_amd/_hip.py
@@ -78,6 +78,10 @@
     "yolosod_conv1x1x2_silu": (_i, [_vp, _l, _vp, _l, _vp, _l, _i, _i, _i, _i, _i, _vp, _vp, _sz, _vp]),
     "yolosod_conv1x1x2_silu_cat": (_i, [_vp, _l, _vp, _l, _i, _vp, _l, _vp, _l, _i, _i, _i, _i, _i, _vp, _vp, _sz,
                                         _i, _vp]),
+    "yolosod_conv1x1x2_silu_cat_gated": (_i, [_vp, _l, _vp, _l, _i, _vp, _vp, _vp, _l, _vp, _l, _i, _i, _i, _i, _i, _vp,
+                                              _vp, _sz, _i, _vp]),
+    "yolosod_conv1x1_thin_gated": (_i, [_vp, _l, _vp, _vp, _vp, _vp, _l, _vp, _l, _i, _i, _i, _i, _l, _vp]),
+    "yolosod_gate_apply": (_i, [_vp, _vp, _i, _i, _i, _i, _vp, _vp, _vp]),
     "yolosod_conv1x1x2_silu_stats": (_i, [_vp, _l, _vp, _l, _i, _i, _i, _i, _vp, _vp, _sz, _i, _i, _vp, _vp, _vp, _vp]),
     "yolosod_sppf_pool": (_i, [_vp, _l, _i, _i, _i, _i, _vp]),
     "yolosod_conv1x1_thin_cat": (_i, [_vp, _l, _vp, _l, _i, _vp, _vp, _vp, _l, _vp, _l, _i, _i, _i, _i, _l, _i, _vp]),
@@ -385,6 +389,36 @@
     return ca, sa
 
 
+def gate_apply(x, gate_c, gate_p=None):
+    lib = load_library()
+    B, C, H, W = x.shape
+    if tuple(gate_c.shape) != (B, C) or (gate_p is not None and gate_p.numel() != B * H * W):
+        raise RuntimeError(f"gate_apply: gates {tuple(gate_c.shape)} / "
+                           f"{None if gate_p is None else tuple(gate_p.shape)} do not fit x {tuple(x.shape)}")
+    y = torch.empty_like(x)
+    _check(_launch(("gate_apply", tuple(x.shape), "se" if gate_p is None else "cbam"), x.device, lib.yolosod_gate_apply,
+                   _dev(x, "x"), y.data_ptr(), B, C, H, W, _dev(gate_c, "gate_c"),
+                   None if gate_p is None else _dev(gate_p, "gate_p"), _stream(x.device)), "gate_apply")
+    return y
+
+
+class GatedMap:
+
+    def __init__(self, x, gc, gp, hid):
+        self.x, self.gc, self.gp, self.hid = x, gc, gp, int(hid)
+        self.shape, self.device, self.dtype = x.shape, x.device, x.dtype
+        self.kind = "se" if gp is None else "cbam"
+        self._y = None
+
+    def dim(self):
+        return 4
+
+    def materialize(self):
+        if self._y is None:
+            self._y = gate_apply(self.x, self.gc, self.gp)
+        return self._y
+
+
 def ca_forward(x, conv1_w, conv1_b, bn_w, bn_b, bn_mean, bn_var, bn_eps, convh_w, convh_b, convw_w, convw_b):
     bf = _act_dtype(_t(x, "x"))
     mip = conv1_w.shape[0]
@@ -762,13 +796,30 @@
             and x.stride(0) % 4 == 0 and x.data_ptr() % 16 == 0)
 
 
-def conv1x1_thin(x, w, bias, out=None, res=None, out2=None, c2lo=0, stats=None):
+def conv1x1_thin(x, w, bias, out=None, res=None, out2=None, c2lo=0, stats=None, gate=None, key=None):
     lib = load_library()
     B, Cin, H, W = x.shape
     Cout = w.shape[0]
     HW = H * W
     if out is None:
         out = torch.empty((B, Cout, H, W), dtype=torch.float32, device=x.device)
+    if gate is not None:
+        if isinstance(x, CatView) or res is not None or stats is not None:
+            raise RuntimeError("conv1x1_thin: a gate takes one input tensor, no res / stats")
+        if (tuple(gate.shape) != (B, Cin) or tuple(w.shape) != (Cout, Cin) or bias.numel() != Cout or Cout != 64
+                or not conv1x1_thin_ok(x, Cout)):
+            raise RuntimeError(f"conv1x1_thin: gate {tuple(gate.shape)} / input {tuple(x.shape)} unsupported")
+        for t, C in ((out, Cout),) + (((out2, Cout - c2lo),) if out2 is not None else ()):
+            if (t.device != x.device or t.dtype != torch.float32 or tuple(t.shape) != (B, C, H, W)
+                    or t.stride()[1:] != (HW, W, 1)):
+                raise RuntimeError(f"conv1x1_thin: output must be a [B,{C},H,W] fp32 GPU tensor with contiguous channels")
+        if key is None:
+            key = ("conv1x1_thin", tuple(x.shape), (Cout, False, out2 is not None, "gated"))
+        _check(_launch(key, x.device, lib.yolosod_conv1x1_thin_gated, x.data_ptr(), x.stride(0), _dev(gate, "gate"),
+                       _dev(w.contiguous(), "weight"), _dev(bias, "bias"), out.data_ptr(), out.stride(0),
+                       None if out2 is None else out2.data_ptr(), 0 if out2 is None else out2.stride(0), int(c2lo), B,
+                       Cin, Cout, HW, _stream(x.device)), "conv1x1_thin_gated")
+        return out
 
     def bstride(t, name, C):
         if t.device.type != "cuda" or t.dtype != torch.float32:
@@ -976,6 +1027,9 @@
 
     def __init__(self, parts, up0=False):
         a, b = parts
+        self.gate = None
+        if isinstance(b, GatedMap):
+            self.gate, b = b, b.x
         sp = (2 * a.shape[2], 2 * a.shape[3]) if up0 else tuple(a.shape[2:])
         if a.shape[0] != b.shape[0] or sp != tuple(b.shape[2:]) or a.dtype != b.dtype or a.device != b.device:
             raise ValueError("CatView: parts must agree in batch, spatial size, dtype and device")
@@ -987,8 +1041,13 @@
     def dim(self):
         return 4
 
+    def ungated(self):
+        if self.gate is None:
+            return self
+        return CatView((self.parts[0], self.gate.materialize()), up0=self.up0)
+
     def materialize(self):
-        a, b = self.parts
+        a, b = self.ungated().parts
         if self.up0:
             a = torch.nn.functional.interpolate(a, scale_factor=2, mode="nearest")
         return torch.cat((a, b), 1)
@@ -1028,9 +1087,18 @@
                           w.reshape(int(w.shape[0]), int(w.shape[1])))
 
 
-def conv1x1x2_silu(x, bias, prep, cout, out=None, out2=None, c2lo=0, op="conv1x1x2", stats=None):
+def conv1x1x2_silu(x, bias, prep, cout, out=None, out2=None, c2lo=0, op="conv1x1x2", stats=None, gate_c=None,
+                   gate_p=None, key=None):
     lib = load_library()
     B, Cin, H, W = x.shape
+    if gate_c is None and gate_p is not None:
+        raise RuntimeError("conv1x1x2: a spatial gate comes with a channel gate")
+    if gate_c is not None:
+        ng = int(x.parts[1].shape[1]) if isinstance(x, CatView) else Cin
+        if stats is not None or tuple(gate_c.shape) != (B, ng) or (gate_p is not None and gate_p.numel() != B * H * W):
+            raise RuntimeError(f"conv1x1x2: gates {tuple(gate_c.shape)} / "
+                               f"{None if gate_p is None else tuple(gate_p.shape)} do not fit the {ng} gated channels "
+                               f"of input {tuple(x.shape)} (no statistics form takes a gate)")
     if stats is not None and (stats not in ("sum", "summax", "capool") or out2 is not None or isinstance(x, CatView)):
         raise RuntimeError(f"conv1x1x2: stats={stats!r} takes one input tensor, no out2")
     if out is None:
@@ -1074,6 +1142,20 @@
     extra = (cout, out2 is not None) + (("cat",) if x1 is not None else ())
     if stats == "capool":
         op, extra = "conv1x1x2_stats", (cout, stats)
+    if gate_c is not None:
+        def run_gated():
+            blk = prep()
+            return lib.yolosod_conv1x1x2_silu_cat_gated(
+                x0.data_ptr(), x0.stride(0), None if x1 is None else x1.data_ptr(), 0 if x1 is None else x1.stride(0),
+                int(x0.shape[1]), _dev(gate_c, "gate_c"), None if gate_p is None else _dev(gate_p, "gate_p"),
+                y.data_ptr(), y.stride(0), None if out2 is None else out2.data_ptr(),
+                0 if out2 is None else out2.stride(0), int(c2lo), B, Cin, cout, H * W, _dev(b, "bias"), blk.data_ptr(),
+                blk.numel(), W if x1 is not None and x.up0 else 0, _stream(x.device))
+
+        if key is None:
+            key = (op, tuple(x.shape), extra + ("se" if gate_p is None else "cbam",))
+        _check(_launch(key, x.device, run_gated), "conv1x1x2_gated")
+        return y
     _check(_launch((op, tuple(x.shape), extra), x.device, run), "conv1x1x2")
     return y
 
diff --git a/yolo-sod_amd/csrc/channel_attention.hip b/yolo-sod_amd/csrc/channel_attention.hip
--- a/yolo-sod_amd/csrc/channel_attention.hip
+++ b/yolo-sod_amd/csrc/channel_attention.hip
@@ -775,6 +775,31 @@
   YS_CHECK_ARG(ca && sa, "cbam_gates: null output");
   return cbam_forward_impl<float>(x, nullptr, B, C, H, W, fc0_w, fc2_w, hidden, sa_w, psum, pmax, workspace,
                                   workspace_bytes, stream, ca, sa);
+}
+
+YS_EXPORT int yolosod_gate_apply(const float* x, float* y, int B, int C, int H, int W, const float* gate_c,
+                                 const float* gate_p, void* stream) {
+  YS_CHECK_ARG(x && y && gate_c, "gate_apply: null pointer");
+  YS_CHECK_ARG(B >= 0 && C > 0 && C <= 16384 && H > 0 && W > 0, "gate_apply: bad shape");
+  if (B == 0) return 0;
+  hipStream_t st = (hipStream_t)stream;
+  const long HW = (long)H * W;
+  if (!gate_p) {
+    const long xchunks = (HW % 4 == 0) ? (HW + 1023) / 1024 : (HW + 255) / 256;
+    const dim3 grid((unsigned)xchunks, (unsigned)((C + 7) / 8), (unsigned)B);
+    hipLaunchKernelGGL((plane_scale_kernel<float, false>), grid, dim3(256), 0, st, x, y, gate_c, C, HW, mall_reverse(),
+                       0, nullptr, 0, 0.f, nullptr, nullptr, nullptr, nullptr, 0);
+  } else {
+    const int V = (HW % 4 == 0) ? 4 : 1;
+    const long pxb = (HW + 256 * V - 1) / (256 * V);
+    const dim3 ga((unsigned)pxb, (unsigned)((C + 7) / 8), (unsigned)B);
+    if (V == 4)
+      hipLaunchKernelGGL((cbam_apply_kernel<4, float>), ga, dim3(256), 0, st, x, y, gate_c, gate_p, C, HW);
+    else
+      hipLaunchKernelGGL((cbam_apply_kernel<1, float>), ga, dim3(256), 0, st, x, y, gate_c, gate_p, C, HW);
+  }
+  YS_CHECK_LAUNCH("gate_apply");
+  return 0;
 }
 
 YS_EXPORT int yolosod_cbam_forward_bf16(const bf16_t* x, bf16_t* y, int B, int C, int H, int W, const float* fc0_w,
diff --git a/yolo-sod_amd/csrc/conv1x1_thin_kernel.h b/yolo-sod_amd/csrc/conv1x1_thin_kernel.h
--- /dev/null
+++ b/yolo-sod_amd/csrc/conv1x1_thin_kernel.h
@@ -0,0 +1,143 @@
+#ifdef YS_THIN_GATE_FORM
+template <int M, int K, bool DUAL>
+__global__ __launch_bounds__(256, K <= 128 ? 4 : 2) void conv1x1_thin_gate_kernel(const float* __restrict__ x, long x_bs,
+                                                                   const float* __restrict__ w,
+                                                                   const float* __restrict__ bias,
+                                                                   float* __restrict__ out, long o_bs,
+                                                                   float* __restrict__ out2, long o2_bs, int c2lo,
+                                                                   int HW, int ntile, int rev,
+                                                                   const float* __restrict__ gc) {
+  constexpr bool RES = false, STATS = false;
+  constexpr int k1 = K;
+  constexpr long r_bs = 0, x2_bs = 0;
+  const float* const res = nullptr;
+  const float* const x2 = nullptr;
+  float* const tsum = nullptr;
+  float* const tmax = nullptr;
+#else
+template <int M, int K, bool RES, bool DUAL, bool STATS = false, bool UP = false>
+__global__ __launch_bounds__(256, 2) void conv1x1_thin_kernel(const float* __restrict__ x, long x_bs,
+                                                              const float* __restrict__ w,
+                                                              const float* __restrict__ bias, float* __restrict__ out,
+                                                              long o_bs, const float* __restrict__ res, long r_bs,
+                                                              float* __restrict__ out2, long o2_bs, int c2lo, int HW,
+                                                              int ntile, int rev, float* __restrict__ tsum = nullptr,
+                                                              float* __restrict__ tmax = nullptr,
+                                                              const float* __restrict__ x2 = nullptr, long x2_bs = 0,
+                                                              int k1 = K, int up_w = 0) {
+#endif
+  constexpr int RB = M / 64;
+  constexpr int KQ = K / 4;
+  constexpr int XS = 68;
+  __shared__ __attribute__((aligned(16))) float xs[K * XS];
+  const int tid = threadIdx.x, lane = tid & 63, wid = tid >> 6;
+  const int l15 = lane & 15, g = lane >> 4;
+  const int b = rev ? gridDim.y - 1 - blockIdx.y : blockIdx.y;
+  const float* xb = x + (long)b * x_bs;
+  const float* xb2 = x2 ? x2 + (long)b * x2_bs - (long)k1 * HW : xb;
+  float4 a[RB][KQ / 4];
+#pragma unroll
+  for (int rb = 0; rb < RB; ++rb) {
+    const float* wr = w + (long)(wid * (M / 4) + rb * 16 + l15) * K + g * KQ;
+#pragma unroll
+    for (int t = 0; t < KQ / 4; ++t) a[rb][t] = *reinterpret_cast<const float4*>(wr + 4 * t);
+  }
+  float bv[RB][4];
+#pragma unroll
+  for (int rb = 0; rb < RB; ++rb)
+#pragma unroll
+    for (int r = 0; r < 4; ++r) bv[rb][r] = bias[wid * (M / 4) + rb * 16 + 4 * g + r];
+  for (int tile = blockIdx.x; tile < ntile; tile += gridDim.x) {
+    const int p0 = tile * 64;
+    __syncthreads();
+#ifdef YS_THIN_GATE_FORM
+    {
+      const float* gcb = gc + (long)b * K;
+#pragma unroll 4
+      for (int e = tid; e < K * 16; e += 256) {
+        const int row = e >> 4, c4 = e & 15;
+        const float4 v = *reinterpret_cast<const float4*>(xb + (long)row * HW + p0 + 4 * c4);
+        const float a = gcb[row];
+        *reinterpret_cast<float4*>(xs + row * XS + 4 * c4) = make_float4(v.x * a, v.y * a, v.z * a, v.w * a);
+      }
+    }
+#else
+    if (UP) {
+      const int pp = p0 + 4 * (tid & 15), yy = pp / up_w, xx = pp - yy * up_w;
+      const float* xu = xb + (yy >> 1) * (up_w >> 1) + (xx >> 1);
+      const int hw1 = HW >> 2;
+#pragma unroll 4
+      for (int e = tid; e < k1 * 16; e += 256) {
+        const int row = e >> 4, c4 = e & 15;
+        const float2 s2 = *reinterpret_cast<const float2*>(xu + (long)row * hw1);
+        *reinterpret_cast<float4*>(xs + row * XS + 4 * c4) = make_float4(s2.x, s2.x, s2.y, s2.y);
+      }
+#pragma unroll 4
+      for (int e = k1 * 16 + tid; e < K * 16; e += 256) {
+        const int row = e >> 4, c4 = e & 15;
+        *reinterpret_cast<float4*>(xs + row * XS + 4 * c4) =
+            *reinterpret_cast<const float4*>(xb2 + (long)row * HW + p0 + 4 * c4);
+      }
+    } else {
+#pragma unroll 4
+      for (int e = tid; e < K * 16; e += 256) {
+        const int row = e >> 4, c4 = e & 15;
+        *reinterpret_cast<float4*>(xs + row * XS + 4 * c4) =
+            *reinterpret_cast<const float4*>((row < k1 ? xb : xb2) + (long)row * HW + p0 + 4 * c4);
+      }
+    }
+#endif
+    __syncthreads();
+    f32x4 acc[RB][4];
+#pragma unroll
+    for (int rb = 0; rb < RB; ++rb)
+#pragma unroll
+      for (int pb = 0; pb < 4; ++pb) acc[rb][pb] = f32x4{0.f, 0.f, 0.f, 0.f};
+#pragma unroll
+    for (int t4 = 0; t4 < KQ / 4; ++t4)
+#pragma unroll
+      for (int c = 0; c < 4; ++c) {
+        const float* xr = xs + (g * KQ + 4 * t4 + c) * XS + l15;
+        float bx[4];
+#pragma unroll
+        for (int pb = 0; pb < 4; ++pb) bx[pb] = xr[16 * pb];
+#pragma unroll
+        for (int rb = 0; rb < RB; ++rb) {
+          const float av = c == 0 ? a[rb][t4].x : c == 1 ? a[rb][t4].y : c == 2 ? a[rb][t4].z : a[rb][t4].w;
+#pragma unroll
+          for (int pb = 0; pb < 4; ++pb) acc[rb][pb] = __builtin_amdgcn_mfma_f32_16x16x4f32(av, bx[pb], acc[rb][pb], 0, 0, 0);
+        }
+      }
+#pragma unroll
+    for (int rb = 0; rb < RB; ++rb)
+#pragma unroll
+      for (int r = 0; r < 4; ++r) {
+        const int row = wid * (M / 4) + rb * 16 + 4 * g + r;
+        float ts = 0.f, tm = -INFINITY;
+#pragma unroll
+        for (int pb = 0; pb < 4; ++pb) {
+          const int p = p0 + pb * 16 + l15;
+          float v = siluf_(acc[rb][pb][r] + bv[rb][r]);
+          if (RES) v += res[(long)b * r_bs + (long)row * HW + p];
+          out[(long)b * o_bs + (long)row * HW + p] = v;
+          if (DUAL && row >= c2lo) out2[(long)b * o2_bs + (long)(row - c2lo) * HW + p] = v;
+          if (STATS) {
+            ts += v;
+            tm = nmax_(tm, v);
+          }
+        }
+        if (STATS) {
+#pragma unroll
+          for (int o = 1; o < 16; o <<= 1) {
+            ts += __shfl_xor(ts, o, 64);
+            tm = nmax_(tm, __shfl_xor(tm, o, 64));
+          }
+          if (l15 == 0) {
+            const long ti = ((long)b * M + row) * ntile + tile;
+            tsum[ti] = ts;
+            tmax[ti] = tm;
+          }
+        }
+      }
+  }
+}
diff --git a/yolo-sod_amd/csrc/conv1x1x2.hip b/yolo-sod_amd/csrc/conv1x1x2.hip
--- a/yolo-sod_amd/csrc/conv1x1x2.hip
+++ b/yolo-sod_amd/csrc/conv1x1x2.hip
@@ -26,10 +26,19 @@
   int up_w;
 };
 
+struct GArgs : Args {
+  const float* gc;
+  const float* gp;
+  int gk0;
+};
+
 #include "conv1x1x2_kernel.h"
 #define YS_C1_STATS_FORMS
 #include "conv1x1x2_kernel.h"
 #undef YS_C1_STATS_FORMS
+#define YS_C1_GATE_FORMS
+#include "conv1x1x2_kernel.h"
+#undef YS_C1_GATE_FORMS
 
 }
 }
@@ -66,6 +75,15 @@
   else hipLaunchKernelGGL((c1::conv1x1_x2_kernel<false, 64, CPW, DB>), dim3(nwg), dim3(c1::NT), 0, st, a);
 }
 
+template <int CPW, bool DB>
+static void c1_launch_gated(bool dual, bool spatial, unsigned nwg, hipStream_t st, const c1::GArgs& a) {
+  const dim3 g(nwg), t(c1::NT);
+  if (dual && spatial) hipLaunchKernelGGL((c1::conv1x1_x2g_kernel<true, CPW, DB, 2>), g, t, 0, st, a);
+  else if (dual) hipLaunchKernelGGL((c1::conv1x1_x2g_kernel<true, CPW, DB, 1>), g, t, 0, st, a);
+  else if (spatial) hipLaunchKernelGGL((c1::conv1x1_x2g_kernel<false, CPW, DB, 2>), g, t, 0, st, a);
+  else hipLaunchKernelGGL((c1::conv1x1_x2g_kernel<false, CPW, DB, 1>), g, t, 0, st, a);
+}
+
 YS_EXPORT size_t yolosod_conv1x1x2_prep_bytes(int cin, int cout) {
   if (cin <= 0 || cin % 32 || cin > 4096 || cout <= 0 || (cout != 64 && cout % 128) || cout > 1024) return 0;
   return split_prep_bytes(c1_halves(cin, cout));
@@ -78,10 +96,10 @@
   return split_prepare<1>("conv1x1x2_prepare", w, cin, c1_pad(cin), cout, prep, prep_bytes, stream);
 }
 
-YS_EXPORT int yolosod_conv1x1x2_silu_cat(const float* x, long x_bstride, const float* x2, long x2_bstride, int k1,
-                                         float* y, long y_bstride, float* y2, long y2_bstride, int c2lo, int B, int cin,
-                                         int cout, int HW, const float* bias, const void* prep, size_t prep_bytes,
-                                         int up_w, void* stream) {
+static int c1_silu_cat(const float* x, long x_bstride, const float* x2, long x2_bstride, int k1, float* y,
+                       long y_bstride, float* y2, long y2_bstride, int c2lo, int B, int cin, int cout, int HW,
+                       const float* bias, const void* prep, size_t prep_bytes, int up_w, const float* gate_c,
+                       const float* gate_p, void* stream) {
   YS_CHECK_ARG(x && y && bias && prep, "conv1x1x2: null pointer");
   if (!x2) k1 = cin;
   YS_CHECK_ARG(up_w == 0 || (x2 && up_w > 0 && up_w % 2 == 0 && HW % up_w == 0 && (HW / up_w) % 2 == 0),
@@ -109,6 +127,18 @@
   const long nwg = (long)B * ntile * (cout == 64 ? 1 : cout / (g256 ? 256 : 128));
   YS_CHECK_ARG(nwg < (1L << 31), "conv1x1x2: too many tiles");
   hipStream_t st = (hipStream_t)stream;
+  if (gate_c) {
+    YS_CHECK_ARG(((uintptr_t)gate_c & 15) == 0, "conv1x1x2: the channel gates must be 16-byte aligned");
+    const c1::GArgs ga{a, gate_c, gate_p, x2 ? k1 : 0};
+    const bool dual = y2 != nullptr, sp2 = gate_p != nullptr;
+    if (cout == 64) c1_launch_gated<1, false>(dual, sp2, (unsigned)nwg, st, ga);
+    else if (g256 && db) c1_launch_gated<4, true>(dual, sp2, (unsigned)nwg, st, ga);
+    else if (g256) c1_launch_gated<4, false>(dual, sp2, (unsigned)nwg, st, ga);
+    else if (db) c1_launch_gated<2, true>(dual, sp2, (unsigned)nwg, st, ga);
+    else c1_launch_gated<2, false>(dual, sp2, (unsigned)nwg, st, ga);
+    YS_CHECK_LAUNCH("conv1x1x2_gated");
+    return 0;
+  }
   if (cout == 64) c1_launch<1, false>(y2 != nullptr, (unsigned)nwg, st, a);
   else if (g256 && db) c1_launch<4, true>(y2 != nullptr, (unsigned)nwg, st, a);
   else if (g256) c1_launch<4, false>(y2 != nullptr, (unsigned)nwg, st, a);
@@ -116,6 +146,24 @@
   else c1_launch<2, false>(y2 != nullptr, (unsigned)nwg, st, a);
   YS_CHECK_LAUNCH("conv1x1x2");
   return 0;
+}
+
+YS_EXPORT int yolosod_conv1x1x2_silu_cat(const float* x, long x_bstride, const float* x2, long x2_bstride, int k1,
+                                         float* y, long y_bstride, float* y2, long y2_bstride, int c2lo, int B, int cin,
+                                         int cout, int HW, const float* bias, const void* prep, size_t prep_bytes,
+                                         int up_w, void* stream) {
+  return c1_silu_cat(x, x_bstride, x2, x2_bstride, k1, y, y_bstride, y2, y2_bstride, c2lo, B, cin, cout, HW, bias, prep,
+                     prep_bytes, up_w, nullptr, nullptr, stream);
+}
+
+YS_EXPORT int yolosod_conv1x1x2_silu_cat_gated(const float* x, long x_bstride, const float* x2, long x2_bstride, int k1,
+                                               const float* gate_c, const float* gate_p, float* y, long y_bstride,
+                                               float* y2, long y2_bstride, int c2lo, int B, int cin, int cout, int HW,
+                                               const float* bias, const void* prep, size_t prep_bytes, int up_w,
+                                               void* stream) {
+  YS_CHECK_ARG(gate_c, "conv1x1x2_gated: null channel gates");
+  return c1_silu_cat(x, x_bstride, x2, x2_bstride, k1, y, y_bstride, y2, y2_bstride, c2lo, B, cin, cout, HW, bias, prep,
+                     prep_bytes, up_w, gate_c, gate_p, stream);
 }
 
 YS_EXPORT int yolosod_conv1x1x2_silu(const float* x, long x_bstride, float* y, long y_bstride, float* y2,
diff --git a/yolo-sod_amd/csrc/conv1x1x2_kernel.h b/yolo-sod_amd/csrc/conv1x1x2_kernel.h
--- a/yolo-sod_amd/csrc/conv1x1x2_kernel.h
+++ b/yolo-sod_amd/csrc/conv1x1x2_kernel.h
@@ -5,6 +5,11 @@
   constexpr bool DUAL = false, DB = false;
   constexpr int NP = 64;
   static_assert(STATS == 1 || STATS == 2, "STATS");
+#elif defined(YS_C1_GATE_FORMS)
+template <bool DUAL, int CPW, bool DB, int GATE>
+__global__ __launch_bounds__(NT, 2) void conv1x1_x2g_kernel(GArgs p) {
+  constexpr int STATS = 0, NP = 64;
+  static_assert(GATE == 1 || GATE == 2, "GATE");
 #else
 template <bool DUAL, int NP, int CPW = 2, bool DB = false>
 __global__ __launch_bounds__(NT, 2) void conv1x1_x2_kernel(Args p) {
@@ -45,6 +50,14 @@
     pc1 = (yy >> 1) * (p.up_w >> 1) + (xx >> 1);
   }
   f32x4 sv[NIT];
+#ifdef YS_C1_GATE_FORMS
+  static_assert(NP == 64, "a wave stages one channel quad per item");
+  f32x4 gq[NIT];
+  bool gst = false;
+  const int gq0 = __builtin_amdgcn_readfirstlane(q0);
+  const float* gcb = p.gc + (long)b * (p.cin - p.gk0);
+  const float gpv = GATE == 2 ? p.gp[(long)b * HW + pc] : 1.f;
+#endif
   auto load_part = [&](int st, int k0, int k1, bool live) __attribute__((always_inline)) {
     const bool second = KS * st >= p.k1;
     const int chs = second ? HW : HW1;
@@ -57,6 +70,18 @@
         sv[k >> 2][k & 3] = __builtin_bit_cast(
             float, __builtin_amdgcn_raw_buffer_load_b32(
                        r, vo + sx + (unsigned)((4 * (NT / NP) * (k >> 2) + (k & 3)) * chs * 4), 0, 0));
+#ifdef YS_C1_GATE_FORMS
+    if (live) {
+      gst = KS * st >= p.gk0;
+#pragma unroll
+      for (int k = 0; k < 4 * NIT; k += 4)
+        if (k >= k0 && k < k1) {
+          const int c = KS * st + 4 * (gq0 + (NT / NP) * (k >> 2));
+          gq[k >> 2] = c >= p.gk0 && c < p.cin ? *reinterpret_cast<const f32x4*>(gcb + (c - p.gk0))
+                                               : f32x4{0.f, 0.f, 0.f, 0.f};
+        }
+    }
+#endif
   };
   const int cb0 = grp * 4 * CPW + CPW * wid;
   auto wfrag = [&](int s, int u, int pl) __attribute__((always_inline)) {
@@ -78,6 +103,12 @@
     for (int i = 0; i < NIT; ++i) {
       const int e = tid + NT * i, quad = e / NP, px = e - quad * NP;
       uint2 hh, ll;
+#ifdef YS_C1_GATE_FORMS
+      if (gst) {
+        sv[i] = sv[i] * gq[i];
+        if (GATE == 2) sv[i] = sv[i] * gpv;
+      }
+#endif
       split4x(sv[i], hh, ll);
       rng = range_acc(rng, sv[i]);
       h16_t* d = pl + px * PS + 4 * quad;
diff --git a/yolo-sod_amd/csrc/conv_epilogue.hip b/yolo-sod_amd/csrc/conv_epilogue.hip
--- a/yolo-sod_amd/csrc/conv_epilogue.hip
+++ b/yolo-sod_amd/csrc/conv_epilogue.hip
@@ -227,118 +227,10 @@
 }
 
 
-template <int M, int K, bool RES, bool DUAL, bool STATS = false, bool UP = false>
-__global__ __launch_bounds__(256, 2) void conv1x1_thin_kernel(const float* __restrict__ x, long x_bs,
-                                                              const float* __restrict__ w,
-                                                              const float* __restrict__ bias, float* __restrict__ out,
-                                                              long o_bs, const float* __restrict__ res, long r_bs,
-                                                              float* __restrict__ out2, long o2_bs, int c2lo, int HW,
-                                                              int ntile, int rev, float* __restrict__ tsum = nullptr,
-                                                              float* __restrict__ tmax = nullptr,
-                                                              const float* __restrict__ x2 = nullptr, long x2_bs = 0,
-                                                              int k1 = K, int up_w = 0) {
-  constexpr int RB = M / 64;
-  constexpr int KQ = K / 4;
-  constexpr int XS = 68;
-  __shared__ __attribute__((aligned(16))) float xs[K * XS];
-  const int tid = threadIdx.x, lane = tid & 63, wid = tid >> 6;
-  const int l15 = lane & 15, g = lane >> 4;
-  const int b = rev ? gridDim.y - 1 - blockIdx.y : blockIdx.y;
-  const float* xb = x + (long)b * x_bs;
-  const float* xb2 = x2 ? x2 + (long)b * x2_bs - (long)k1 * HW : xb;
-  float4 a[RB][KQ / 4];
-#pragma unroll
-  for (int rb = 0; rb < RB; ++rb) {
-    const float* wr = w + (long)(wid * (M / 4) + rb * 16 + l15) * K + g * KQ;
-#pragma unroll
-    for (int t = 0; t < KQ / 4; ++t) a[rb][t] = *reinterpret_cast<const float4*>(wr + 4 * t);
-  }
-  float bv[RB][4];
-#pragma unroll
-  for (int rb = 0; rb < RB; ++rb)
-#pragma unroll
-    for (int r = 0; r < 4; ++r) bv[rb][r] = bias[wid * (M / 4) + rb * 16 + 4 * g + r];
-  for (int tile = blockIdx.x; tile < ntile; tile += gridDim.x) {
-    const int p0 = tile * 64;
-    __syncthreads();
-    if (UP) {
-      const int pp = p0 + 4 * (tid & 15), yy = pp / up_w, xx = pp - yy * up_w;
-      const float* xu = xb + (yy >> 1) * (up_w >> 1) + (xx >> 1);
-      const int hw1 = HW >> 2;
-#pragma unroll 4
-      for (int e = tid; e < k1 * 16; e += 256) {
-        const int row = e >> 4, c4 = e & 15;
-        const float2 s2 = *reinterpret_cast<const float2*>(xu + (long)row * hw1);
-        *reinterpret_cast<float4*>(xs + row * XS + 4 * c4) = make_float4(s2.x, s2.x, s2.y, s2.y);
-      }
-#pragma unroll 4
-      for (int e = k1 * 16 + tid; e < K * 16; e += 256) {
-        const int row = e >> 4, c4 = e & 15;
-        *reinterpret_cast<float4*>(xs + row * XS + 4 * c4) =
-            *reinterpret_cast<const float4*>(xb2 + (long)row * HW + p0 + 4 * c4);
-      }
-    } else {
-#pragma unroll 4
-      for (int e = tid; e < K * 16; e += 256) {
-        const int row = e >> 4, c4 = e & 15;
-        *reinterpret_cast<float4*>(xs + row * XS + 4 * c4) =
-            *reinterpret_cast<const float4*>((row < k1 ? xb : xb2) + (long)row * HW + p0 + 4 * c4);
-      }
-    }
-    __syncthreads();
-    f32x4 acc[RB][4];
-#pragma unroll
-    for (int rb = 0; rb < RB; ++rb)
-#pragma unroll
-      for (int pb = 0; pb < 4; ++pb) acc[rb][pb] = f32x4{0.f, 0.f, 0.f, 0.f};
-#pragma unroll
-    for (int t4 = 0; t4 < KQ / 4; ++t4)
-#pragma unroll
-      for (int c = 0; c < 4; ++c) {
-        const float* xr = xs + (g * KQ + 4 * t4 + c) * XS + l15;
-        float bx[4];
-#pragma unroll
-        for (int pb = 0; pb < 4; ++pb) bx[pb] = xr[16 * pb];
-#pragma unroll
-        for (int rb = 0; rb < RB; ++rb) {
-          const float av = c == 0 ? a[rb][t4].x : c == 1 ? a[rb][t4].y : c == 2 ? a[rb][t4].z : a[rb][t4].w;
-#pragma unroll
-          for (int pb = 0; pb < 4; ++pb) acc[rb][pb] = __builtin_amdgcn_mfma_f32_16x16x4f32(av, bx[pb], acc[rb][pb], 0, 0, 0);
-        }
-      }
-#pragma unroll
-    for (int rb = 0; rb < RB; ++rb)
-#pragma unroll
-      for (int r = 0; r < 4; ++r) {
-        const int row = wid * (M / 4) + rb * 16 + 4 * g + r;
-        float ts = 0.f, tm = -INFINITY;
-#pragma unroll
-        for (int pb = 0; pb < 4; ++pb) {
-          const int p = p0 + pb * 16 + l15;
-          float v = siluf_(acc[rb][pb][r] + bv[rb][r]);
-          if (RES) v += res[(long)b * r_bs + (long)row * HW + p];
-          out[(long)b * o_bs + (long)row * HW + p] = v;
-          if (DUAL && row >= c2lo) out2[(long)b * o2_bs + (long)(row - c2lo) * HW + p] = v;
-          if (STATS) {
-            ts += v;
-            tm = nmax_(tm, v);
-          }
-        }
-        if (STATS) {
-#pragma unroll
-          for (int o = 1; o < 16; o <<= 1) {
-            ts += __shfl_xor(ts, o, 64);
-            tm = nmax_(tm, __shfl_xor(tm, o, 64));
-          }
-          if (l15 == 0) {
-            const long ti = ((long)b * M + row) * ntile + tile;
-            tsum[ti] = ts;
-            tmax[ti] = tm;
-          }
-        }
-      }
-  }
-}
+#include "conv1x1_thin_kernel.h"
+#define YS_THIN_GATE_FORM
+#include "conv1x1_thin_kernel.h"
+#undef YS_THIN_GATE_FORM
 
 __global__ __launch_bounds__(256) void thin_stats_reduce_kernel(const float* __restrict__ tsum,
                                                                 const float* __restrict__ tmax, long planes, int ntile,
@@ -626,6 +518,40 @@
   return 0;
 }
 
+YS_EXPORT int yolosod_conv1x1_thin_gated(const float* x, long x_bs, const float* gate_c, const float* w,
+                                         const float* bias, float* out, long out_bs, float* out2, long out2_bs,
+                                         int c2lo, int B, int Cin, int Cout, long HW, void* stream) {
+  YS_CHECK_ARG(x && gate_c && w && bias && out, "conv1x1_thin_gated: null pointer");
+  YS_CHECK_ARG(HW % 64 == 0 && HW < (1L << 30), "conv1x1_thin_gated: HW=%ld must be a multiple of 64", HW);
+  YS_CHECK_ARG(Cout == 64, "conv1x1_thin_gated: Cout=%d unsupported (64 only)", Cout);
+  YS_CHECK_ARG(x_bs % 4 == 0 && out_bs % 4 == 0 && (!out2 || out2_bs % 4 == 0),
+               "conv1x1_thin_gated: batch strides must be multiples of 4");
+  YS_CHECK_ARG(x_bs >= (long)Cin * HW && out_bs >= (long)Cout * HW, "conv1x1_thin_gated: batch strides too small");
+  YS_CHECK_ARG((((uintptr_t)x | (uintptr_t)w | (uintptr_t)out) & 15) == 0,
+               "conv1x1_thin_gated: pointers must be 16-byte aligned");
+  YS_CHECK_ARG(!out2 || (c2lo >= 0 && c2lo < Cout && out2_bs >= (long)(Cout - c2lo) * HW),
+               "conv1x1_thin_gated: c2lo=%d", c2lo);
+  if (B == 0) return 0;
+  const int ntile = (int)(HW / 64);
+  const int gx = ntile < 4 ? ntile : (ntile + 3) / 4;
+  hipStream_t st = (hipStream_t)stream;
+  const dim3 grid((unsigned)gx, (unsigned)B);
+  bool ok = false;
+#define YS_THING(M_, K_)                                                                                           \
+  if (Cout == M_ && Cin == K_) {                                                                                   \
+    ok = true;                                                                                                     \
+    if (out2) hipLaunchKernelGGL((conv1x1_thin_gate_kernel<M_, K_, true>), grid, dim3(256), 0, st, x, x_bs, w, bias, \
+                                 out, out_bs, out2, out2_bs, c2lo, (int)HW, ntile, mall_reverse(), gate_c);        \
+    else hipLaunchKernelGGL((conv1x1_thin_gate_kernel<M_, K_, false>), grid, dim3(256), 0, st, x, x_bs, w, bias,   \
+                            out, out_bs, nullptr, 0L, 0, (int)HW, ntile, mall_reverse(), gate_c);                  \
+  }
+  YS_THING(64, 64) YS_THING(64, 96) YS_THING(64, 128) YS_THING(64, 192) YS_THING(64, 256)
+#undef YS_THING
+  YS_CHECK_ARG(ok, "conv1x1_thin_gated: Cin=%d unsupported", Cin);
+  YS_CHECK_LAUNCH("conv1x1_thin_gated");
+  return 0;
+}
+
 YS_EXPORT int yolosod_conv1x1_thin_cat(const float* x, long x_bs, const float* x2, long x2_bs, int k1, const float* w,
                                        const float* bias, float* out, long out_bs, float* out2, long out2_bs, int c2lo,
                                        int B, int Cin, int Cout, long HW, int up_w, void* stream) {
diff --git a/yolo-sod_amd/nn/modules.py b/yolo-sod_amd/nn/modules.py
--- a/yolo-sod_amd/nn/modules.py
+++ b/yolo-sod_amd/nn/modules.py
@@ -135,6 +135,8 @@
 BOTTLENECK_FUSE = _onoff_switch("YOLOSOD_BOTTLENECK_FUSE", os.environ.get("YOLOSOD_BOTTLENECK_FUSE", "1"))
 HEAD_FUSE_DEFAULT = "1"
 HEAD_FUSE = _onoff_switch("YOLOSOD_HEAD_FUSE", os.environ.get("YOLOSOD_HEAD_FUSE", HEAD_FUSE_DEFAULT))
+NECK_GATE_FUSE = _onoff_switch("YOLOSOD_NECK_GATE_FUSE", os.environ.get("YOLOSOD_NECK_GATE_FUSE", "1"))
+NECK_GATE_MIN_BYTES = 16 << 20
 
 
 def _s2_on(s2, layer=None):
@@ -169,10 +171,12 @@
     return stats_layer in N1_STATS
 
 
-def _n1_run(conv, x, out, out2, c2lo, n1, stats=None):
+def _n1_run(conv, x, out, out2, c2lo, n1, stats=None, gate=None, key=None):
     prep = _prep(conv, "c1prep", _hip.conv1x1x2_prepare)
     return _hip.conv1x1x2_silu(x, conv.bias, prep, conv.out_channels, out=out, out2=out2, c2lo=c2lo,
-                               op="conv1x1x2_backbone" if n1 == "backbone" else "conv1x1x2", stats=stats)
+                               op="conv1x1x2_backbone" if n1 == "backbone" else "conv1x1x2", stats=stats,
+                               gate_c=None if gate is None else gate.gc, gate_p=None if gate is None else gate.gp,
+                               key=key)
 
 
 def conv_epilogue(conv: nn.Conv2d, act_code, x, out=None, res=None, stats=None, out2=None, c2lo=0, tower=False,
@@ -182,6 +186,12 @@
         return None
     split = _hip.split_convs_enabled()
     if isinstance(x, _hip.CatView):
+        if x.gate is not None:
+            if (NECK_GATE_FUSE and act_code == 1 and res is None and stats is None and conv.kernel_size == (1, 1)
+                    and split and _n1_on(n1, layer) and _hip.conv1x1x2_ok(x, conv)
+                    and (out is None or _hip._imgs_contig(out)) and (out2 is None or _hip._imgs_contig(out2))):
+                return _n1_run(conv, x, out, out2, c2lo, n1, gate=x.gate)
+            x = x.ungated()
         if act_code == 1 and res is None and stats is None and conv.kernel_size == (1, 1):
             if split and _n1_on(n1, layer) and _hip.conv1x1x2_ok(x, conv) and (
                     out is None or _hip._imgs_contig(out)) and (out2 is None or _hip._imgs_contig(out2)):
@@ -281,7 +291,37 @@
         prep = _prep(cv, "c3s2prep", _hip.conv3x3s2_prepare)
         return _hip.conv3x3s2_silu(x, cv.bias, prep, cv.out_channels, gate_c, gate_p, key=key)
 
+    def gate_route(self, x, spatial: bool):
+        cv = self.conv
+        if (not NECK_GATE_FUSE or hasattr(self, "bn") or cv.bias is None or not isinstance(self.act, nn.SiLU)
+                or self.emit_stats is not None or cv.kernel_size != (1, 1) or cv.stride != (1, 1) or cv.groups != 1
+                or cv.padding != (0, 0) or not isinstance(x, torch.Tensor) or x.device.type != "cuda"
+                or x.dtype != torch.float32 or x.dim() != 4 or not _hip.split_convs_enabled()):
+            return None
+        if self.n1 and N1_NECK and _hip.conv1x1x2_ok(x, cv):
+            return "x2"
+        if (not spatial and not self.n1 and THIN1X1 and cv.out_channels == 64 and x.shape[1] == cv.in_channels
+                and _hip.conv1x1_thin_ok(x, 64)):
+            return "thin"
+        return None
+
+    def forward_gatedmap(self, g, out=None, out2=None, c2lo=0):
+        cv = self.conv
+        route = self.gate_route(g.x, g.gp is not None)
+        key = (g.kind + "_conv1x1", tuple(g.shape), (cv.out_channels, g.hid, route))
+        if route == "x2" and (out is None or _hip._imgs_contig(out)) and (out2 is None or _hip._imgs_contig(out2)):
+            return _n1_run(cv, g.x, out, out2, c2lo, True, gate=g, key=key)
+        if route == "thin" and (out is None or out.data_ptr() % 16 == 0):
+            return _hip.conv1x1_thin(g.x, cv.weight.detach().reshape(cv.out_channels, -1), cv.bias.detach(), out=out,
+                                     out2=out2, c2lo=c2lo, gate=g.gc, key=key)
+        return None
+
     def forward_fuse(self, x, out=None, res=None, out2=None, c2lo=0):
+        if isinstance(x, _hip.GatedMap):
+            y = self.forward_gatedmap(x, out, out2, c2lo) if res is None else None
+            if y is not None:
+                return y
+            x = x.materialize()
         if (self.stem and STEM_HIP and self.emit_stats == "sum" and out is None and res is None and out2 is None
                 and isinstance(self.act, nn.SiLU) and _hip.stem_ok(x, self.conv)):
             return _hip.stem_conv(x, self.conv.weight.detach(), self.conv.bias.detach())
diff --git a/yolo-sod_amd/nn/tasks.py b/yolo-sod_amd/nn/tasks.py
--- a/yolo-sod_amd/nn/tasks.py
+++ b/yolo-sod_amd/nn/tasks.py
@@ -209,6 +209,63 @@
         self._gplan = plan
         return plan
 
+    def _neck_gate_plan(self):
+        plan = getattr(self, "_ngplan", None)
+        if plan is not None:
+            return plan
+        plan = {}
+        cprod, taken = self._concat_producers(), self._gate_consumers()
+        det = self.model[-1]
+        levels = set(det.f) if isinstance(det, M.Detect) and isinstance(det.f, (list, tuple)) else set()
+        n = len(self.model)
+
+        def is_1x1(cv):
+            c = cv.conv
+            return (isinstance(cv, M.Conv) and not isinstance(cv, M.DWConv) and c.kernel_size == (1, 1)
+                    and c.stride == (1, 1) and c.groups == 1 and c.padding == (0, 0) and cv.emit_stats is None)
+
+        for k in range(n - 1):
+            m, nxt = self.model[k], self.model[k + 1]
+            if not isinstance(m, (M.SE, M.CBAM_Block)) or k in taken or k in levels or k + 1 in levels or k + 1 in cprod:
+                continue
+            if not (nxt.f == -1 and is_1x1(nxt)
+                    and (nxt.n1 or (isinstance(m, M.SE) and nxt.conv.out_channels == 64))):
+                continue
+            cats, ok = [], True
+            for j in range(k + 2, n):
+                mj = self.model[j]
+                f = list(mj.f) if isinstance(mj.f, (list, tuple)) else [mj.f]
+                if k not in [j - 1 if v == -1 else v % j for v in f]:
+                    continue
+                c2f = self.model[j + 1] if j + 1 < n else None
+                if (isinstance(mj, M.Concat) and mj.d == 1 and len(f) == 2 and f[0] == -1 and f[1] % j == k
+                        and j not in self.save and cprod.get(j - 1) == j and isinstance(c2f, M.C2f) and c2f.f == -1
+                        and is_1x1(c2f.cv1) and c2f.cv1.n1):
+                    cats.append(j)
+                else:
+                    ok = False
+            if ok:
+                plan[k] = (nxt, tuple(cats))
+        self._ngplan = plan
+        return plan
+
+    def _neck_gate_ok(self, m, inp, readers) -> bool:
+        nxt, cats = readers
+        if not (M.NECK_GATE_FUSE and inp.device.type == "cuda" and inp.dtype == torch.float32 and inp.dim() == 4
+                and inp.is_contiguous() and inp.numel() * 4 >= M.NECK_GATE_MIN_BYTES and _hip.split_convs_enabled()):
+            return False
+        spatial = isinstance(m, M.CBAM_Block)
+        if nxt.gate_route(inp, spatial) is None:
+            return False
+        B, C, H, W = inp.shape
+        for j in cats:
+            cv1 = self.model[j + 1].cv1
+            c0 = cv1.conv.in_channels - C
+            if not (CATVIEW and M.N1_NECK and c0 > 0 and c0 % 128 == 0 and cv1.is_fused()
+                    and M.catview_route(cv1, c0, C, H, W, inp.dtype)):
+                return False
+        return True
+
     def _predict_once_planned(self, x):
         plan = self._concat_producers()
         det = self.model[-1]
@@ -238,6 +295,7 @@
         elided = 0
         gplan = self._gate_consumers() if GATE_FUSE else {}
         gated = None
+        ngplan = self._neck_gate_plan() if M.NECK_GATE_FUSE else {}
         for m in self.model:
             if gated is not None:
                 xg, gc, gp, key = gated
@@ -248,6 +306,12 @@
             inp = x
             if m.f != -1:
                 inp = y[m.f] if isinstance(m.f, int) else [x if j == -1 else y[j] for j in m.f]
+            if isinstance(inp, _hip.GatedMap):
+                if not isinstance(m, M.Conv):
+                    inp = inp.materialize()
+            elif isinstance(inp, list):
+                inp = [v.materialize() if isinstance(v, _hip.GatedMap) and not (k == 1 and m.i in cvpend) else v
+                       for k, v in enumerate(inp)]
             cons = gplan.get(m.i)
             if cons is not None and isinstance(inp, torch.Tensor) and cons.gated_ok(inp):
                 if isinstance(m, M.SE):
@@ -310,14 +374,14 @@
                     continue
             cvp = cvpend.pop(m.i, None)
             if cvp is not None:
-                x = _hip.CatView([x if j == -1 else y[j] for j in m.f], up0=cvp[0])
+                x = _hip.CatView(inp, up0=cvp[0])
                 elided += 1
             elif m.i in pend:
                 buf, offs, chans = pend.pop(m.i)
                 elided += 1
                 for j, o, n in zip(m.f, offs, chans):
                     if j != -1:
-                        buf[:, o:o + n].copy_(y[j])
+                        buf[:, o:o + n].copy_(y[j].materialize() if isinstance(y[j], _hip.GatedMap) else y[j])
                 x = buf
             elif m is det and towers is not None and len(towers) == det.nl:
                 feats = [towers[k] for k in range(det.nl)]
@@ -332,6 +396,11 @@
                     else:
                         x = det.forward_towers([f if f is not None else det.tower_features(k, ins[k])
                                                 for k, f in enumerate(feats)])
+            elif (m.i in ngplan and isinstance(inp, torch.Tensor) and self._neck_gate_ok(m, inp, ngplan[m.i])):
+                if isinstance(m, M.SE):
+                    x = _hip.GatedMap(inp, m.gate(inp), None, m.fc1.out_channels)
+                else:
+                    x = _hip.GatedMap(inp, *m.gates(inp), m.channel_attention.fc[0].out_channels)
             else:
                 x = m(inp)
             if towers is not None and m is not det:
@@ -385,6 +454,7 @@
                     m.forward = m.forward_fuse
         self._fused = True
         self._cplan = None
+        self._ngplan = None
         return self
 
 
diff --git a/yolo-sod_amd/perf.py b/yolo-sod_amd/perf.py
--- a/yolo-sod_amd/perf.py
+++ b/yolo-sod_amd/perf.py
@@ -26,7 +26,7 @@
         op = key[0]
         split = ((op == "swin" and key[1][1] in (64, 256) and _on("YOLOSOD_SWIN_X3"))
                  or (op == "a2" and _on("YOLOSOD_A2_X2")) or (op == "head" and _on("YOLOSOD_HEAD_X2"))
-                 or op in FUSED_CONV)
+                 or (op in FUSED_CONV and not (op in FUSED_1X1 and key[2][2] == "thin")))
         if split:
             return PEAK_BF16_MFMA_TFLOPS / 3
     return peak_tflops(key)
@@ -34,6 +34,8 @@
 
 FUSED_CONV = {"se_conv": "se", "cbam_conv": "cbam"}
 GATE_ONLY = {"se_gate": "se_conv", "cbam_gate": "cbam_conv"}
+FUSED_CONV.update({"se_conv1x1": "se", "cbam_conv1x1": "cbam"})
+FUSED_1X1 = frozenset({"se_conv1x1", "cbam_conv1x1"})
 PATH_OPS = frozenset({"se", "cbam", "ca", "a2", "swin", "mamba", "decode", "head", "nms", *FUSED_CONV})
 
 
@@ -51,6 +53,13 @@
 
 def _op_cost(key, E):
     op, shape, extra = key
+    if op in FUSED_1X1:
+        B, C, H, W = shape
+        cout, hid = extra[:2]
+        cb = op == "cbam_conv1x1"
+        act = B * C * H * W * E + B * cout * H * W * E + (B * H * W * F32 if cb else 0)
+        w = (cout * C + cout + 2 * C * hid + C + hid + (98 if cb else 0)) * F32
+        return act + w, 2 * B * H * W * cout * C + B * C * H * W * (2 if cb else 1)
     if op in FUSED_CONV:
         B, C, H, W = shape
         cout, hid = extra
@@ -209,7 +218,7 @@
     gate_ms = {}
     for key, (tot, n) in agg.items():
         if key[0] in GATE_ONLY:
-            k2 = (GATE_ONLY[key[0]], tuple(key[1]))
+            k2 = (FUSED_CONV[GATE_ONLY[key[0]]], tuple(key[1]))
             gate_ms[k2] = gate_ms.get(k2, 0.0) + tot
     ops, backbone = [], []
     for key, (tot, n) in agg.items():
@@ -220,7 +229,7 @@
                              "total_ms_per_step": round(tot / steps, 4)})
             continue
         nbytes, flops = op_cost(key)
-        kern = tot / n + gate_ms.get((key[0], tuple(key[1])), 0.0) / n
+        kern = tot / n + (gate_ms.get((FUSED_CONV[key[0]], tuple(key[1])), 0.0) / n if key[0] in FUSED_CONV else 0.0)
         ext, src = billed.get((FUSED_CONV.get(key[0], key[0]), tuple(key[1])), (0.0, None))
         avg = kern + ext
         bound = bound_of(key)
@@ -256,8 +265,13 @@
 def _split_fused(key):
     op, shape, extra = key[:3]
     B, C, H, W = shape
-    cout, hid = extra
+    cout, hid = extra[:2]
     E = elem_size(key)
+    if op in FUSED_1X1:
+        conv_b = (B * C * H * W + B * cout * H * W) * E + (cout * C + cout) * F32
+        conv_f = 2 * B * H * W * cout * C
+        t_conv = max(conv_b / (PEAK_HBM_GBS * 1e9), conv_f / (method_peak_tflops(key) * 1e12)) * 1e3
+        return (FUSED_CONV[op], tuple(shape), hid) + tuple(key[3:]), t_conv
     Ho, Wo = (H + 1) // 2, (W + 1) // 2
     conv_b = (B * C * H * W + B * cout * Ho * Wo) * E + (cout * C * 9 + cout) * F32
     conv_f = 2 * B * Ho * Wo * cout * C * 9
```

New measurement: 4649 (median of 6 runs). No clear change (+0.6%).
